# thodan/epos

Hardware: AMD Instinct MI355X
Metric: images/sec end-to-end (CNN+PnP-RANSAC), YCB-V 640x480 (higher is better)
Workload: dtype f32

## Files before the change

### epos_amd/_lib.py

```python
import ctypes
import os

from epos_amd import build as _build

c_f32p = ctypes.POINTER(ctypes.c_float)
c_f64p = ctypes.POINTER(ctypes.c_double)
c_i32p = ctypes.POINTER(ctypes.c_int32)
c_i64p = ctypes.POINTER(ctypes.c_int64)
c_u64p = ctypes.POINTER(ctypes.c_uint64)
vp = ctypes.c_void_p


class EposError(RuntimeError):
  pass


class PointwiseArgs(ctypes.Structure):
  _fields_ = [
      ('A', vp), ('lda', ctypes.c_int64),
      ('Wp', vp), ('bias', vp),
      ('R', vp), ('ldr', ctypes.c_int64),
      ('C', vp), ('ldc', ctypes.c_int64),
      ('M', ctypes.c_int32), ('N', ctypes.c_int32), ('K', ctypes.c_int32),
      ('relu', ctypes.c_int32), ('relu_in', ctypes.c_int32),
      ('sub', ctypes.c_int32),
      ('Ho', ctypes.c_int32), ('Wo', ctypes.c_int32),
      ('Hi', ctypes.c_int32), ('Wi', ctypes.c_int32),
      ('Ws', vp),
      ('Wh', vp), ('a_amax', vp), ('a_amax2', vp),
      ('a_gain', ctypes.c_float), ('a_bias', ctypes.c_float),
      ('a_presplit', ctypes.c_int32),
      ('c_amax', vp),
      ('col_sums', vp), ('col_ld', ctypes.c_int64),
      ('c_stream', ctypes.c_int32), ('reserved0', ctypes.c_int32),
  ]


class DepthwiseArgs(ctypes.Structure):
  _fields_ = [
      ('X', vp), ('ldx', ctypes.c_int64),
      ('w9c', vp), ('bias', vp),
      ('Y', vp), ('ldy', ctypes.c_int64),
      ('B', ctypes.c_int32), ('Hi', ctypes.c_int32), ('Wi', ctypes.c_int32),
      ('Ho', ctypes.c_int32), ('Wo', ctypes.c_int32), ('C', ctypes.c_int32),
      ('stride', ctypes.c_int32), ('rate', ctypes.c_int32),
      ('relu_in', ctypes.c_int32), ('relu_out', ctypes.c_int32),
      ('y_h2', ctypes.c_int32), ('x_amax', vp), ('x_amax2', vp),
      ('gain', ctypes.c_float), ('bias0', ctypes.c_float),
  ]


class SepConvArgs(ctypes.Structure):
  _fields_ = [('dw', DepthwiseArgs), ('pw', PointwiseArgs)]


class Conv3x3Args(ctypes.Structure):
  _fields_ = [
      ('X', vp), ('ldx', ctypes.c_int64),
      ('Wp', vp), ('bias', vp),
      ('Y', vp), ('ldy', ctypes.c_int64),
      ('B', ctypes.c_int32), ('H', ctypes.c_int32), ('W', ctypes.c_int32),
      ('Cin', ctypes.c_int32), ('Cout', ctypes.c_int32),
      ('stride', ctypes.c_int32), ('rate', ctypes.c_int32),
      ('relu', ctypes.c_int32),
      ('Ws', vp),
      ('Wh', vp), ('x_amax', vp), ('y_amax', vp),
  ]


class Im2colArgs(ctypes.Structure):
  _fields_ = [
      ('X', vp), ('ldx', ctypes.c_int64),
      ('col', vp), ('ldcol', ctypes.c_int64),
      ('B', ctypes.c_int32), ('Hi', ctypes.c_int32), ('Wi', ctypes.c_int32),
      ('Ho', ctypes.c_int32), ('Wo', ctypes.c_int32), ('C', ctypes.c_int32),
      ('stride', ctypes.c_int32), ('rate', ctypes.c_int32),
      ('pad', ctypes.c_int32), ('preprocess', ctypes.c_int32),
      ('amax_clear', vp), ('amax_words', ctypes.c_int64),
  ]


PREPROCESS_NONE, PREPROCESS_UNIT_RANGE, PREPROCESS_SUB_MEAN = 0, 1, 2


class Im2colKArgs(ctypes.Structure):
  _fields_ = [
      ('X', vp), ('ldx', ctypes.c_int64),
      ('col', vp), ('ldcol', ctypes.c_int64),
      ('B', ctypes.c_int32), ('Hi', ctypes.c_int32), ('Wi', ctypes.c_int32),
      ('Ho', ctypes.c_int32), ('Wo', ctypes.c_int32), ('C', ctypes.c_int32),
      ('k', ctypes.c_int32), ('stride', ctypes.c_int32), ('rate', ctypes.c_int32),
      ('pad', ctypes.c_int32), ('preprocess', ctypes.c_int32),
      ('mean_rgb', ctypes.c_float * 3),
      ('amax_clear', vp), ('amax_words', ctypes.c_int64),
  ]


class PointwiseBf16Args(ctypes.Structure):
  _fields_ = [
      ('A', vp), ('lda', ctypes.c_int64),
      ('Wp', vp), ('bias', vp),
      ('R', vp), ('ldr', ctypes.c_int64),
      ('C', vp), ('ldc', ctypes.c_int64),
      ('M', ctypes.c_int32), ('N', ctypes.c_int32), ('K', ctypes.c_int32),
      ('relu', ctypes.c_int32), ('sub', ctypes.c_int32),
      ('Ho', ctypes.c_int32), ('Wo', ctypes.c_int32),
      ('Hi', ctypes.c_int32), ('Wi', ctypes.c_int32),
      ('c_f32', ctypes.c_int32), ('c_stream', ctypes.c_int32),
  ]


class DepthwiseBf16Args(ctypes.Structure):
  _fields_ = [
      ('X', vp), ('ldx', ctypes.c_int64),
      ('w9c', vp), ('bias', vp),
      ('Y', vp), ('ldy', ctypes.c_int64),
      ('B', ctypes.c_int32), ('Hi', ctypes.c_int32), ('Wi', ctypes.c_int32),
      ('Ho', ctypes.c_int32), ('Wo', ctypes.c_int32), ('C', ctypes.c_int32),
      ('stride', ctypes.c_int32), ('rate', ctypes.c_int32),
      ('relu_in', ctypes.c_int32), ('relu_out', ctypes.c_int32),
  ]


class Im2colBf16Args(ctypes.Structure):
  _fields_ = [
      ('X', vp), ('ldx', ctypes.c_int64),
      ('x_bf16', ctypes.c_int32), ('reserved0', ctypes.c_int32),
      ('col', vp), ('ldcol', ctypes.c_int64),
      ('B', ctypes.c_int32), ('Hi', ctypes.c_int32), ('Wi', ctypes.c_int32),
      ('Ho', ctypes.c_int32), ('Wo', ctypes.c_int32), ('C', ctypes.c_int32),
      ('k', ctypes.c_int32), ('stride', ctypes.c_int32), ('rate', ctypes.c_int32),
      ('pad', ctypes.c_int32), ('preprocess', ctypes.c_int32),
# ... 59 lines not shown
              ('K', ctypes.c_int32), ('N', ctypes.c_int32)]


class PointwiseWgradArgs(ctypes.Structure):
  _fields_ = [('A', vp), ('lda', ctypes.c_int64), ('G', vp), ('ldg', ctypes.c_int64),
              ('M', ctypes.c_int64), ('K', ctypes.c_int32), ('N', ctypes.c_int32),
              ('a_presplit', ctypes.c_int32), ('reserved0', ctypes.c_int32),
              ('a_amax', vp), ('a_amax2', vp),
              ('a_gain', ctypes.c_float), ('a_bias', ctypes.c_float),
              ('S', vp), ('g', vp), ('workspace', vp)]


class PointwiseDgradArgs(ctypes.Structure):
  _fields_ = [('G', vp), ('ldg', ctypes.c_int64), ('W', vp), ('gamma', vp),
              ('moving_variance', vp), ('eps', ctypes.c_double),
              ('mask', vp), ('ldm', ctypes.c_int64),
              ('mask_h2', ctypes.c_int32), ('reserved0', ctypes.c_int32),
              ('M', ctypes.c_int64), ('K', ctypes.c_int32), ('N', ctypes.c_int32),
              ('D', vp), ('ldd', ctypes.c_int64), ('workspace', vp)]


class DepthwiseWgradArgs(ctypes.Structure):
  _fields_ = [('X', vp), ('ldx', ctypes.c_int64), ('D', vp), ('ldd', ctypes.c_int64),
              ('B', ctypes.c_int32), ('H', ctypes.c_int32), ('W', ctypes.c_int32),
              ('C', ctypes.c_int32), ('stride', ctypes.c_int32), ('rate', ctypes.c_int32),
              ('T', vp), ('t', vp), ('workspace', vp)]


class AsppJoinDw(ctypes.Structure):
  _fields_ = [('D', vp), ('ldd', ctypes.c_int64), ('w9c', vp), ('rate', ctypes.c_int32),
              ('reserved0', ctypes.c_int32)]


class AsppJoinPlain(ctypes.Structure):
  _fields_ = [('E', vp), ('lde', ctypes.c_int64)]


class AsppJoinArgs(ctypes.Structure):
  _fields_ = [('B', ctypes.c_int32), ('H', ctypes.c_int32), ('W', ctypes.c_int32),
              ('C', ctypes.c_int32), ('n_dw', ctypes.c_int32), ('n_plain', ctypes.c_int32),
              ('dw', AsppJoinDw * 4), ('plain', AsppJoinPlain * 2),
              ('Pool', vp), ('ldp', ctypes.c_int64), ('pool_div', ctypes.c_int64),
              ('Y', vp), ('ldy', ctypes.c_int64), ('dX', vp), ('ldx', ctypes.c_int64),
              ('partition', ctypes.c_int32), ('reserved0', ctypes.c_int32)]


ASPP_JOIN_PARTITIONS = {'shipped': 0, 'pixel': 1, 'slice32': 2, 'slice64': 3, 'slice32x2': 4,
                        'slice32x4': 5}


class FitParams(ctypes.Structure):
  _fields_ = [
      ('threshold', ctypes.c_double),
      ('neighborhood_ball_radius', ctypes.c_double),
      ('spatial_coherence_weight', ctypes.c_double),
      ('scaling_from_millimeters', ctypes.c_double),
      ('max_tanimoto_similarity', ctypes.c_double),
      ('conf', ctypes.c_double),
      ('proposal_engine_conf', ctypes.c_double),
      ('min_coverage', ctypes.c_double),
      ('min_triangle_area', ctypes.c_double),
      ('max_iters', ctypes.c_int32),
      ('min_point_number', ctypes.c_int32),
      ('max_model_number', ctypes.c_int32),
      ('max_model_number_for_optimization', ctypes.c_int32),
      ('use_prosac', ctypes.c_int32),
      ('lo_iters', ctypes.c_int32),
      ('gc_sweeps', ctypes.c_int32),
      ('pearl_iters', ctypes.c_int32),
  ]


class PnpRansacParams(ctypes.Structure):
  _fields_ = [
      ('iterations_count', ctypes.c_int32),
      ('min_point_number', ctypes.c_int32),
      ('reprojection_error', ctypes.c_double),
      ('confidence', ctypes.c_double),
  ]


SYMBOLS = {
    'epos_abi_version': (ctypes.c_int, []),
    'epos_last_error': (ctypes.c_char_p, []),
    'epos_device_count': (ctypes.c_int, []),
    'epos_clock_probe': (ctypes.c_int, [ctypes.c_void_p, ctypes.c_int, ctypes.c_void_p]),
    'epos_pack_pointwise_weights': (ctypes.c_int64,
                                    [vp, ctypes.c_int, ctypes.c_int, vp]),
    'epos_pack_pointwise_weights_split': (ctypes.c_int64,
                                          [vp, ctypes.c_int, ctypes.c_int, vp]),
    'epos_pack_pointwise_weights_h2': (ctypes.c_int64,
                                       [vp, ctypes.c_int, ctypes.c_int, vp]),
    'epos_absmax_f32': (ctypes.c_int, [vp, ctypes.c_int64, ctypes.c_int64,
                                       ctypes.c_int64, vp, vp]),
    'epos_amax_clear': (ctypes.c_int, [vp, ctypes.c_int64, vp]),
    'epos_pointwise_conv_f32': (ctypes.c_int,
                                [ctypes.POINTER(PointwiseArgs), vp]),
    'epos_pointwise_conv_grouped_f32': (ctypes.c_int, [
        ctypes.POINTER(PointwiseArgs), ctypes.c_int, vp]),
    'epos_heads_gemm_f32': (ctypes.c_int, [
        ctypes.POINTER(PointwiseArgs), ctypes.c_int, vp]),
    'epos_heads_gemm_plan': (ctypes.c_int, [
        ctypes.POINTER(PointwiseArgs), ctypes.c_int, ctypes.c_int, c_i32p]),
    'epos_conv3x3_f32': (ctypes.c_int, [ctypes.POINTER(Conv3x3Args), ctypes.c_void_p]),
    'epos_depthwise3x3_f32': (ctypes.c_int,
                              [ctypes.POINTER(DepthwiseArgs), vp]),
    'epos_separable_conv_f32': (ctypes.c_int, [ctypes.POINTER(SepConvArgs), vp]),
    'epos_set_h2_narrow_tile_limit': (ctypes.c_int, [ctypes.c_int]),
    'epos_im2col3x3_f32': (ctypes.c_int, [ctypes.POINTER(Im2colArgs), vp]),
    'epos_im2col_f32': (ctypes.c_int, [ctypes.POINTER(Im2colKArgs), vp]),
    'epos_global_avg_pool_partial_f32': (ctypes.c_int, [
        vp, ctypes.c_int64, vp, ctypes.c_int, ctypes.c_int, ctypes.c_int, ctypes.c_int, vp]),
    'epos_global_avg_pool_f32': (ctypes.c_int, [
        vp, ctypes.c_int64, vp, ctypes.c_int, ctypes.c_int, ctypes.c_int, vp]),
    'epos_resize_bilinear_f32': (ctypes.c_int, [
        vp, ctypes.c_int64, vp, ctypes.c_int64, ctypes.c_int, ctypes.c_int,
        ctypes.c_int, ctypes.c_int, ctypes.c_int, ctypes.c_int, vp]),
    'epos_maxpool3x3_s2_f32': (ctypes.c_int, [
        vp, ctypes.c_int64, vp, ctypes.c_int64, ctypes.c_int, ctypes.c_int,
        ctypes.c_int, ctypes.c_int, vp]),
    'epos_subsample_f32': (ctypes.c_int, [
        vp, ctypes.c_int64, vp, ctypes.c_int64, ctypes.c_int, ctypes.c_int,
        ctypes.c_int, ctypes.c_int, ctypes.c_int, vp]),
    'epos_add_relu_f32': (ctypes.c_int, [vp, vp, vp, ctypes.c_int64, vp]),
    'epos_softmax_groups_f32': (ctypes.c_int,
                                [vp, ctypes.c_int64, ctypes.c_int, vp]),
    'epos_u8_to_f32': (ctypes.c_int, [vp, vp, ctypes.c_int64, vp]),
    'epos_scatter_blocks_f32': (ctypes.c_int, [vp, vp, vp, ctypes.c_int64, ctypes.c_int, vp]),
    'epos_argmax_i64': (ctypes.c_int, [
        vp, ctypes.c_int64, vp, ctypes.c_int64, ctypes.c_int, vp]),
    'epos_softmax_slots_f32': (ctypes.c_int, [
        vp, vp, ctypes.c_int, ctypes.c_int, ctypes.c_int, ctypes.c_int, vp]),
    'epos_corr_count': (ctypes.c_int, [
        vp, vp, vp, ctypes.c_int, ctypes.c_int, ctypes.c_int, ctypes.c_int,
        ctypes.c_int, ctypes.c_float, ctypes.c_float, vp, vp, vp, vp, vp]),
    'epos_corr_fill': (ctypes.c_int, [
        vp, vp, vp, vp, vp, vp, ctypes.c_int, ctypes.c_int, ctypes.c_int,
        ctypes.c_int, ctypes.c_int, ctypes.c_int, ctypes.c_double, vp, vp, vp,
        vp, ctypes.c_int64, ctypes.POINTER(CorrOut), vp, vp]),
    'epos_corr_slot_bases': (ctypes.c_int, [vp, ctypes.c_int, vp, vp]),
    'epos_corr_order_tile_rows': (ctypes.c_int, []),
    'epos_corr_order_workspace_bytes': (ctypes.c_int64, [ctypes.c_int, ctypes.c_int64]),
    'epos_corr_order_by_conf': (ctypes.c_int, [
        vp, vp, vp, vp, vp, ctypes.c_int, ctypes.c_int64, ctypes.c_int, ctypes.c_int64,
        ctypes.c_int, vp, vp, vp, vp, vp, vp, vp, vp]),
    'epos_project_to_mesh_f64': (ctypes.c_int, [
        ctypes.c_void_p, ctypes.c_int64, ctypes.c_void_p, ctypes.c_int64,
        ctypes.c_void_p, ctypes.c_int64, ctypes.c_void_p, ctypes.c_void_p,
        ctypes.c_void_p]),
    'epos_project_rows_to_mesh_f64': (ctypes.c_int, [
        vp, vp, vp, ctypes.c_int, ctypes.c_int64, vp, ctypes.c_int, vp, vp, vp, vp, vp]),
    'epos_fragmentation_fps': (ctypes.c_int, [
        vp, ctypes.c_int64, ctypes.c_int, vp, vp, vp, vp, vp]),
    'epos_fit_params_default': (None, [ctypes.POINTER(FitParams)]),
    'epos_find6d_poses': (ctypes.c_int, [
        vp, vp, ctypes.c_int64, vp, ctypes.POINTER(FitParams), ctypes.c_uint64,
        vp, vp, vp, ctypes.c_int32]),
    'epos_fit_workspace_bytes': (ctypes.c_int64, [
        ctypes.c_int, ctypes.c_int64, ctypes.POINTER(FitParams),
        ctypes.c_int32]),
    'epos_find6d_poses_device': (ctypes.c_int, [
        vp, vp, vp, ctypes.c_int, ctypes.c_int64, vp, vp, vp,
        ctypes.POINTER(FitParams), ctypes.c_int32, vp, vp, vp, vp, vp, vp]),
    'epos_find6d_poses_device_ordered': (ctypes.c_int, [
        vp, vp, vp, ctypes.c_int, ctypes.c_int64, vp, vp, vp,
        ctypes.POINTER(FitParams), ctypes.c_int32, vp, vp, vp, vp, vp, vp, vp, vp]),
# ... 188 lines not shown
```

### epos_amd/csrc/common.h

```cpp
#pragma once
#include <hip/hip_runtime.h>
#include <stdint.h>
#include <stdio.h>

#include "../../include/epos_hip.h"

namespace epos {

void set_error(const char* fmt, ...);

inline int check_hip(hipError_t e, const char* what) {
  if (e == hipSuccess) return EPOS_OK;
  set_error("%s: %s", what, hipGetErrorString(e));
  return EPOS_E_HIP_BASE - static_cast<int>(e);
}

inline int launch_status(const char* kernel) {
  return check_hip(hipGetLastError(), kernel);
}

inline int64_t round_up(int64_t x, int64_t m) { return (x + m - 1) / m * m; }
inline int64_t ceil_div(int64_t x, int64_t m) { return (x + m - 1) / m; }
inline unsigned blocks_for(int64_t total, int threads) {
  return static_cast<unsigned>(ceil_div(total, threads));
}
inline bool al16(const void* p) { return (reinterpret_cast<uintptr_t>(p) & 15) == 0; }

__device__ __forceinline__ float4 relu4(float4 v) {
  return make_float4(fmaxf(v.x, 0.f), fmaxf(v.y, 0.f), fmaxf(v.z, 0.f),
                     fmaxf(v.w, 0.f));
}

constexpr int DW_PRIO = 3;
#define EPOS_SET_PRIO(p) do { if ((p) > 0) __builtin_amdgcn_s_setprio(p); } while (0)

#define EPOS_REQUIRE(cond, msg)                  \
  do {                                           \
    if (!(cond)) {                               \
      ::epos::set_error("%s: %s", __func__, msg); \
      return EPOS_E_INVALID;                     \
    }                                            \
  } while (0)

#define EPOS_REQUIRE_FN(fn, cond, msg)           \
  do {                                           \
    if (!(cond)) {                               \
      ::epos::set_error("%s: %s", fn, msg);      \
      return EPOS_E_INVALID;                     \
    }                                            \
  } while (0)

}
```

### epos_amd/csrc/glue.hip

```cpp
#include "nhwc.h"

namespace epos {
namespace {

template <class SP, class DP>
__global__ __launch_bounds__(256) void resize_bilinear_kernel(
    const typename SP::elem* X, int64_t ldx, typename DP::elem* Y, int64_t ldy, int Hi, int Wi,
    int Ho, int Wo, int cn, float sy, float sx, int64_t total) {
  static_assert(SP::n == DP::n, "one thread reads the channels it writes");
  const int64_t id = static_cast<int64_t>(blockIdx.x) * blockDim.x + threadIdx.x;
  if (id >= total) return;
  const Pixel p = decode_pixel<DP::n>(id, cn, Ho, Wo);
  const BilinearSrc<typename SP::elem> src = {X, ldx, Hi, Wi, sy, sx};
  float o[DP::n];
  bilinear_sample<SP>(src, p.b, p.yo, p.xo, p.c, o);
  DP::store(Y + pixel_offset(p, Ho, Wo, ldy), o);
}

template <class P>
__global__ __launch_bounds__(256) void maxpool3x3_s2_kernel(
    const typename P::elem* X, int64_t ldx, typename P::elem* Y, int64_t ldy, int Hi, int Wi,
    int Ho, int Wo, int cn, int pad_y, int pad_x, int64_t total) {
  const int64_t id = static_cast<int64_t>(blockIdx.x) * blockDim.x + threadIdx.x;
  if (id >= total) return;
  const Pixel p = decode_pixel<P::n>(id, cn, Ho, Wo);
  const typename P::elem* xb = X + static_cast<int64_t>(p.b) * Hi * Wi * ldx + p.c;
  float m[P::n];
#pragma unroll
  for (int e = 0; e < P::n; ++e) m[e] = -INFINITY;
#pragma unroll
  for (int ky = 0; ky < 3; ++ky) {
    const int yi = p.yo * 2 - pad_y + ky;
    if (yi < 0 || yi >= Hi) continue;
#pragma unroll
    for (int kx = 0; kx < 3; ++kx) {
      const int xi = p.xo * 2 - pad_x + kx;
      if (xi < 0 || xi >= Wi) continue;
      float v[P::n];
      P::load(xb + (static_cast<int64_t>(yi) * Wi + xi) * ldx, v);
#pragma unroll
      for (int e = 0; e < P::n; ++e) m[e] = fmaxf(m[e], v[e]);
    }
  }
  P::store(Y + pixel_offset(p, Ho, Wo, ldy), m);
}

template <class P>
__global__ __launch_bounds__(256) void subsample_kernel(
    const typename P::elem* X, int64_t ldx, typename P::elem* Y, int64_t ldy, int Hi, int Wi,
    int Ho, int Wo, int cn, int factor, int64_t total) {
  const int64_t id = static_cast<int64_t>(blockIdx.x) * blockDim.x + threadIdx.x;
  if (id >= total) return;
  const Pixel p = decode_pixel<P::n>(id, cn, Ho, Wo);
  using vec = typename P::vec;
  *reinterpret_cast<vec*>(Y + pixel_offset(p, Ho, Wo, ldy)) = *reinterpret_cast<const vec*>(
      X + ((static_cast<int64_t>(p.b) * Hi + p.yo * factor) * Wi + p.xo * factor) * ldx + p.c);
}

template <class P>
__global__ __launch_bounds__(256) void add_relu_kernel(const typename P::elem* A,
                                                       const typename P::elem* B,
                                                       typename P::elem* Y, int64_t packs) {
  const int64_t i = static_cast<int64_t>(blockIdx.x) * blockDim.x + threadIdx.x;
  if (i >= packs) return;
  float a[P::n], b[P::n];
  P::load(A + P::n * i, a);
  P::load(B + P::n * i, b);
#pragma unroll
  for (int e = 0; e < P::n; ++e) a[e] = fmaxf(a[e] + b[e], 0.f);
  P::store(Y + P::n * i, a);
}

int check_maps(const char* fn, const void* X, int64_t ldx, const void* Y, int64_t ldy, int B,
               int Hi, int Wi, int C, int N, const void* need_al0 = nullptr,
               const void* need_al1 = nullptr) {
  const char* msg = nullptr;
  if (!X || !Y) msg = "null pointer";
  else if (C % N || ldx % N || ldy % N) msg = "C, ldx, ldy must be multiples of 4 (bf16: 8)";
  else if (!al16(need_al0) || !al16(need_al1)) msg = "bf16 tensors must be 16-byte aligned";
  else if (B < 1 || Hi < 1 || Wi < 1 || C < 1) msg = "empty map";
  else if (ldx < C || ldy < C) msg = "ldx, ldy >= C";
  if (!msg) return EPOS_OK;
  set_error("%s: %s", fn, msg);
  return EPOS_E_INVALID;
}

struct Same { int out, pad; };
Same same_3x3_s2(int in) {
  const int out = (in + 1) / 2, t = (out - 1) * 2 + 3 - in;
  return {out, t > 0 ? t / 2 : 0};
}

template <class SP, class DP>
int resize(const typename SP::elem* X, int64_t ldx, typename DP::elem* Y, int64_t ldy, int B,
           int Hi, int Wi, int Ho, int Wo, int C, void* stream) {
  const int cn = C / DP::n;
  const int64_t total = static_cast<int64_t>(B) * Ho * Wo * cn;
  hipLaunchKernelGGL((resize_bilinear_kernel<SP, DP>), dim3(blocks_for(total, 256)), dim3(256),
                     0, static_cast<hipStream_t>(stream), X, ldx, Y, ldy, Hi, Wi, Ho, Wo, cn,
                     align_corners_scale(Hi, Ho), align_corners_scale(Wi, Wo), total);
  return launch_status("resize_bilinear_kernel");
}

template <class P>
int maxpool(const typename P::elem* X, int64_t ldx, typename P::elem* Y, int64_t ldy, int B,
            int Hi, int Wi, int C, void* stream) {
  const Same y = same_3x3_s2(Hi), x = same_3x3_s2(Wi);
  const int cn = C / P::n;
  const int64_t total = static_cast<int64_t>(B) * y.out * x.out * cn;
  hipLaunchKernelGGL(maxpool3x3_s2_kernel<P>, dim3(blocks_for(total, 256)), dim3(256), 0,
                     static_cast<hipStream_t>(stream), X, ldx, Y, ldy, Hi, Wi, y.out, x.out, cn,
                     y.pad, x.pad, total);
  return launch_status("maxpool3x3_s2_kernel");
}

template <class P>
int subsample(const typename P::elem* X, int64_t ldx, typename P::elem* Y, int64_t ldy, int B,
              int Hi, int Wi, int C, int factor, void* stream) {
  const int Ho = (Hi - 1) / factor + 1, Wo = (Wi - 1) / factor + 1;
  const int cn = C / P::n;
  const int64_t total = static_cast<int64_t>(B) * Ho * Wo * cn;
  hipLaunchKernelGGL(subsample_kernel<P>, dim3(blocks_for(total, 256)), dim3(256), 0,
                     static_cast<hipStream_t>(stream), X, ldx, Y, ldy, Hi, Wi, Ho, Wo, cn,
                     factor, total);
  return launch_status("subsample_kernel");
}

template <class P>
int add_relu(const char* fn, const typename P::elem* A, const typename P::elem* B,
             typename P::elem* Y, int64_t n, bool need_al, void* stream) {
  const char* msg = nullptr;
  if (!A || !B || !Y) msg = "null pointer";
  else if (n < 0 || n % P::n) msg = "n must be a multiple of 4 (bf16: 8)";
  else if (need_al && !(al16(A) && al16(B) && al16(Y))) msg = "16-byte aligned";
  if (msg) {
    set_error("%s: %s", fn, msg);
    return EPOS_E_INVALID;
  }
  if (n == 0) return EPOS_OK;
  hipLaunchKernelGGL(add_relu_kernel<P>, dim3(blocks_for(n / P::n, 256)), dim3(256), 0,
                     static_cast<hipStream_t>(stream), A, B, Y, n / P::n);
  return launch_status("add_relu_kernel");
}

using F32 = F32Pack<4>;

}
}

using namespace epos;

extern "C" int epos_resize_bilinear_f32(const float* X, int64_t ldx, float* Y, int64_t ldy, int B,
                                        int Hi, int Wi, int Ho, int Wo, int C, void* stream) {
  EPOS_REQUIRE(Ho >= 1 && Wo >= 1, "empty map");
  if (int rc = check_maps(__func__, X, ldx, Y, ldy, B, Hi, Wi, C, 4)) return rc;
  return resize<F32, F32>(X, ldx, Y, ldy, B, Hi, Wi, Ho, Wo, C, stream);
}

extern "C" int epos_resize_bilinear_bf16(const void* X, int64_t ldx, int x_f32, uint16_t* Y,
                                         int64_t ldy, int B, int Hi, int Wi, int Ho, int Wo,
                                         int C, void* stream) {
  EPOS_REQUIRE(Ho >= 1 && Wo >= 1, "empty map");
  if (int rc = check_maps(__func__, X, ldx, Y, ldy, B, Hi, Wi, C, 8, Y, x_f32 ? nullptr : X))
    return rc;
  if (x_f32)
    return resize<F32ScalarPack, Bf16Pack>(static_cast<const float*>(X), ldx, Y, ldy, B, Hi, Wi,
                                           Ho, Wo, C, stream);
  return resize<Bf16Pack, Bf16Pack>(static_cast<const uint16_t*>(X), ldx, Y, ldy, B, Hi, Wi, Ho,
                                    Wo, C, stream);
}

extern "C" int epos_maxpool3x3_s2_f32(const float* X, int64_t ldx, float* Y, int64_t ldy, int B,
                                      int Hi, int Wi, int C, void* stream) {
  if (int rc = check_maps(__func__, X, ldx, Y, ldy, B, Hi, Wi, C, 4)) return rc;
  return maxpool<F32>(X, ldx, Y, ldy, B, Hi, Wi, C, stream);
}

extern "C" int epos_maxpool3x3_s2_bf16(const uint16_t* X, int64_t ldx, uint16_t* Y,
                                       int64_t ldy, int B, int Hi, int Wi, int C, void* stream) {
  if (int rc = check_maps(__func__, X, ldx, Y, ldy, B, Hi, Wi, C, 8, X, Y)) return rc;
  return maxpool<Bf16Pack>(X, ldx, Y, ldy, B, Hi, Wi, C, stream);
}

extern "C" int epos_subsample_f32(const float* X, int64_t ldx, float* Y, int64_t ldy, int B,
                                  int Hi, int Wi, int C, int factor, void* stream) {
  EPOS_REQUIRE(factor >= 1, "factor >= 1");
  if (int rc = check_maps(__func__, X, ldx, Y, ldy, B, Hi, Wi, C, 4)) return rc;
  return subsample<F32>(X, ldx, Y, ldy, B, Hi, Wi, C, factor, stream);
}

extern "C" int epos_subsample_bf16(const uint16_t* X, int64_t ldx, uint16_t* Y, int64_t ldy,
                                   int B, int Hi, int Wi, int C, int factor, void* stream) {
  EPOS_REQUIRE(factor >= 1, "factor >= 1");
  if (int rc = check_maps(__func__, X, ldx, Y, ldy, B, Hi, Wi, C, 8, X, Y)) return rc;
  return subsample<Bf16Pack>(X, ldx, Y, ldy, B, Hi, Wi, C, factor, stream);
}

extern "C" int epos_add_relu_f32(const float* A, const float* B, float* Y, int64_t n,
                                 void* stream) {
  return add_relu<F32>(__func__, A, B, Y, n, false, stream);
}

extern "C" int epos_add_relu_bf16(const uint16_t* A, const uint16_t* B, uint16_t* Y, int64_t n,
                                  void* stream) {
  return add_relu<Bf16Pack>(__func__, A, B, Y, n, true, stream);
}
```

### epos_amd/csrc/heads_gemm_h2.hip

```cpp
#include "h2_scale.h"
#include "pointwise_gemm.h"

namespace epos {
namespace {

typedef _Float16 hd_f16x8 __attribute__((ext_vector_type(8)));
typedef unsigned hd_u32x4 __attribute__((ext_vector_type(4)));

constexpr int HD_BM = 128, HD_BN = 64, HD_BK = 16;
constexpr int HD_K = 256;
constexpr int HD_NKS = HD_K / HD_BK;
constexpr int HD_NS = 8;
constexpr int HD_LA = HD_NS - 1;
constexpr int HD_STAGE = 4 * 1024;
constexpr int HD_RING = HD_NS * HD_STAGE;
constexpr int HD_OPS = 2 * 4 * 1024;
constexpr int HD_EPR = HD_BN + 4;
constexpr int HD_EPI = 4 * 32 * HD_EPR * 4;
constexpr int HD_LDS = HD_RING + HD_OPS + HD_EPI;
constexpr int HD_S_MIN = 8;
constexpr unsigned HD_OOB = 0x80000000u;
static_assert(HD_NKS % HD_NS == 0, "stage of a K step = its index mod HD_NS");
static_assert(HD_LA - 2 + 2 + HD_S_MIN <= 63, "vmcnt is a 6-bit counter");

// ... 151 lines not shown
    const int par = (tt - t0) & 1;
    f32x16 acc[2], corr[2];
#pragma unroll
    for (int j = 0; j < 2; ++j)
#pragma unroll
      for (int r = 0; r < 16; ++r) { acc[j][r] = 0.f; corr[j][r] = 0.f; }

    auto step = [&](auto ks_tag) {
      constexpr int ks = decltype(ks_tag)::value;
      constexpr int younger = (HD_LA - 2) + (ks >= 10 ? 2 : 0);
      static_assert(HD_LA == 7, "the counts above are written for 7 steps ahead");
      if constexpr (ks <= 5) {
        if (first) hd_wait_vm_lgkm0<younger>();
        else hd_wait_vm_lgkm0<younger + HD_S_MIN>();
      } else {
        hd_wait_vm_lgkm0<younger>();
      }
      __builtin_amdgcn_s_barrier();
      constexpr int s1 = (ks + 1) % HD_NS;
      hd_u32x4 nb[2][2];
#pragma unroll
      for (int cb = 0; cb < 2; ++cb)
#pragma unroll
        for (int pc = 0; pc < 2; ++pc)
          nb[cb][pc] = *reinterpret_cast<const hd_u32x4*>(smem + s1 * (HD_STAGE / 4) + b_off +
                                                          (cb * 2 + pc) * 256);
      __builtin_amdgcn_sched_barrier(0);
      hd_mfma(ah[ks], bp[0][1], corr[0]);
      __builtin_amdgcn_sched_barrier(0);
      {
        constexpr int q = ks + HD_LA;
        constexpr int slot = q % HD_NS;
        if constexpr (q < HD_NKS) issue_w(cur, q, slot);
        else issue_w(nxt, q - HD_NKS, slot);
      }
      __builtin_amdgcn_sched_barrier(0);
      hd_mfma(ah[ks], bp[1][1], corr[1]);
      if constexpr (ks + HD_LA == HD_NKS) {
        __builtin_amdgcn_sched_barrier(0);
        issue_ops(nxt, par ^ 1);
        __builtin_amdgcn_sched_barrier(0);
      }
      hd_mfma(am[ks], bp[0][0], corr[0]);
      hd_mfma(am[ks], bp[1][0], corr[1]);
      hd_mfma(ah[ks], bp[0][0], acc[0]);
      hd_mfma(ah[ks], bp[1][0], acc[1]);
#pragma unroll
      for (int cb = 0; cb < 2; ++cb) { bp[cb][0] = nb[cb][0]; bp[cb][1] = nb[cb][1]; }
    };
    hd_static_for(std::make_integer_sequence<int, HD_NKS>{}, step);

#pragma unroll
    for (int j = 0; j < 2; ++j)
#pragma unroll
      for (int r = 0; r < 16; ++r)
        ws[((r & 3) + 8 * (r >> 2) + 4 * h) * HD_EPR + j * 32 + l31] =
            __builtin_fmaf(corr[j][r], 0x1p-11f, acc[j][r]);
    __builtin_amdgcn_fence(__ATOMIC_RELEASE, "wavefront");
    const float* ops = smem + (HD_RING + par * 4096) / 4 + wave * 256;
    const float4 cn4 = *reinterpret_cast<const float4*>(ops + c4 * 4);
    const float4 b4 = *reinterpret_cast<const float4*>(ops + 64 + c4 * 4);
    float4 v[8];
#pragma unroll
    for (int i = 0; i < 8; ++i) {
      v[i] = *reinterpret_cast<const float4*>(ws + (r0 + 4 * i) * HD_EPR + c4 * 4);
      v[i].x = v[i].x * cn4.x * inv_a + b4.x;
      v[i].y = v[i].y * cn4.y * inv_a + b4.y;
      v[i].z = v[i].z * cn4.z * inv_a + b4.z;
      v[i].w = v[i].w * cn4.w * inv_a + b4.w;
    }
    const EposPointwiseArgs& q = gp->p[cur.pi];
    const int rows = M - m0 < HD_BM ? M - m0 : HD_BM;
    const int64_t ldc = q.ldc;
    const __amdgpu_buffer_rsrc_t rsrc = __builtin_amdgcn_make_buffer_rsrc(
        q.C + static_cast<int64_t>(m0) * ldc, 0, static_cast<int>(rows * ldc * 4), 0x00020000);
    const int n = cur.n0 + c4 * 4;
    const unsigned row0 = static_cast<unsigned>(wave * 32 + r0);
    const bool vec = (ldc & 3) == 0 && (cur.N & 3) == 0 &&
                     (reinterpret_cast<uintptr_t>(q.C) & 15) == 0;
    auto opaque = [](unsigned x) { asm volatile("" : "+v"(x)); return x; };
    if (vec) {
      const unsigned oob = n < cur.N ? 0u : HD_OOB;
      const unsigned nb4 = static_cast<unsigned>(n) * 4u;
#pragma unroll
      for (int i = 0; i < 8; ++i) {
        const int off = static_cast<int>(
            opaque(((row0 + 4 * i) * static_cast<unsigned>(ldc) * 4u + nb4) | oob));
        if (q.c_stream)
          __builtin_amdgcn_raw_buffer_store_b128(__builtin_bit_cast(hd_u32x4, v[i]), rsrc, off, 0, 2);
        else
          __builtin_amdgcn_raw_buffer_store_b128(__builtin_bit_cast(hd_u32x4, v[i]), rsrc, off, 0, 0);
      }
    } else {
#pragma unroll
      for (int i = 0; i < 8; ++i) {
        const float e4[4] = {v[i].x, v[i].y, v[i].z, v[i].w};
#pragma unroll
        for (int e = 0; e < 4; ++e) {
          const unsigned oob = n + e < cur.N ? 0u : HD_OOB;
          const int off = static_cast<int>(opaque(
              (((row0 + 4 * i) * static_cast<unsigned>(ldc) + static_cast<unsigned>(n + e)) * 4u) |
              oob));
          __builtin_amdgcn_raw_buffer_store_b32(__float_as_uint(e4[e]), rsrc, off, 0, 0);
        }
      }
    }
    cur = nxt;
    nxt = hd_tile(gp, tt + 2 < t1 ? tt + 2 : t1 - 1);
  }
  asm volatile("s_waitcnt vmcnt(0)" ::: "memory");
}

int choose_range(int nt, int panels, int cus) {
  const int slots = cus > 8 ? cus * 2 / 8 : 1;
  const int pmax = (panels + 7) / 8;
  int best = nt < 4 ? nt : 4;
  int64_t best_cost = -1;
  for (int r = 4; r <= 32; ++r) {
    const int rr = r < nt ? r : nt;
    const int64_t nr = (nt + rr - 1) / rr;
    const int64_t rounds = (pmax * nr + slots - 1) / slots;
    const int64_t cost = rounds * (rr + 1);
    if (best_cost < 0 || cost < best_cost) { best_cost = cost; best = rr; }
    if (rr == nt) break;
  }
  return best;
}

int device_cus() {
  static int cus[16] = {};
  int dev = 0;
  if (hipGetDevice(&dev) != hipSuccess || dev < 0 || dev >= 16) return 256;
  int n = __atomic_load_n(&cus[dev], __ATOMIC_RELAXED);
  if (n > 0) return n;
  if (hipDeviceGetAttribute(&n, hipDeviceAttributeMultiprocessorCount, dev) != hipSuccess || n <= 0)
    n = 256;
  __atomic_store_n(&cus[dev], n, __ATOMIC_RELAXED);
  return n;
}

}

bool heads_eligible(const EposPointwiseArgs* args, int count) {
  if (count < 1 || count > MAX_GROUP) return false;
  const EposPointwiseArgs& a0 = args[0];
  if (!a0.a_amax) return false;
  for (int i = 0; i < count; ++i) {
    const EposPointwiseArgs& a = args[i];
    if (a.A != a0.A || a.lda != a0.lda || a.M != a0.M || a.K != HD_K || a.sub != 1 ||
        a.R || a.relu || a.relu_in || a.a_presplit || a.c_amax || a.col_sums || !a.Wh ||
        a.a_amax != a0.a_amax || a.a_amax2 != a0.a_amax2 || a.a_gain != a0.a_gain ||
        a.a_bias != a0.a_bias || a.N < 1 || a.M < 1 || a.ldc < a.N ||
        a.ldc > (1LL << 20) ||
        (reinterpret_cast<uintptr_t>(a.Wh) & 15) != 0 ||
        (reinterpret_cast<uintptr_t>(a.bias) & 3) != 0)
      return false;
  }
  return true;
}

namespace {

bool heads_fill(const EposPointwiseArgs* args, int count, int cus, HeadsArgs& g, int& blocks) {
  if (!h2_eligible(args, count) || !heads_eligible(args, count)) return false;
  g.count = count;
  int nt = 0;
  for (int i = 0; i < count; ++i) {
    g.p[i] = args[i];
    g.tile0[i] = nt;
    nt += static_cast<int>(ceil_div(args[i].N, HD_BN));
  }
  for (int i = count; i <= MAX_GROUP; ++i) g.tile0[i] = nt;
  g.nt = nt;
  g.panels = static_cast<int>(ceil_div(args[0].M, HD_BM));
// ... 47 lines not shown
```

### epos_amd/csrc/layers.hip

```cpp
#include <stdlib.h>

#include "h2_scale.h"
#include "nhwc.h"

namespace epos {
namespace {

typedef unsigned dw_u32x4 __attribute__((ext_vector_type(4)));
__device__ __forceinline__ void st4_h2(float* p, float4 v, float s) {
  dw_u32x4 o;
  unsigned h0, h1, m0, m1;
  h2_split_pair(v.x, v.y, s, h0, m0);
  h2_split_pair(v.z, v.w, s, h1, m1);
  o[0] = h0; o[1] = h1; o[2] = m0; o[3] = m1;
  *reinterpret_cast<dw_u32x4*>(p) = o;
}
__device__ __forceinline__ void st4_any(float* p, float4 v, bool h2, float s) {
  if (h2) st4_h2(p, v, s); else st4(p, v);
}
__device__ __forceinline__ float4 fma4(float4 a, float4 b, float4 c) {
  return make_float4(fmaf(a.x, b.x, c.x), fmaf(a.y, b.y, c.y),
                     fmaf(a.z, b.z, c.z), fmaf(a.w, b.w, c.w));
}

__global__ __launch_bounds__(256) void depthwise3x3_kernel(EposDepthwiseArgs p,
                                                           int c4n,
                                                           int64_t total) {
  EPOS_SET_PRIO(DW_PRIO);
  int64_t id = static_cast<int64_t>(blockIdx.x) * blockDim.x + threadIdx.x;
  const bool h2 = p.y_h2 != 0;
  float hs = 1.f;
  unsigned am_raw, am_raw2;
  {
    const unsigned* s1 = h2 ? p.x_amax : reinterpret_cast<const unsigned*>(p.bias);
    const unsigned* s2 = (h2 && p.x_amax2) ? p.x_amax2 : s1;
    const int li = h2 ? static_cast<int>(threadIdx.x & 63) : 0;
    am_raw = s1[li];
    am_raw2 = s2[li];
  }
  const bool live = id < total;
  if (__builtin_amdgcn_ballot_w64(live) == 0) return;
  id = live ? id : total - 1;
  const Pixel o = decode_pixel<4>(id, c4n, p.Ho, p.Wo);
  const int pad = p.rate;
  float4 acc = ld4(p.bias + o.c);
  const float* xb = p.X + static_cast<int64_t>(o.b) * p.Hi * p.Wi * p.ldx + o.c;
#pragma unroll
  for (int ky = 0; ky < 3; ++ky) {
    const int yi = o.yo * p.stride - pad + ky * p.rate;
    if (yi < 0 || yi >= p.Hi) continue;
#pragma unroll
    for (int kx = 0; kx < 3; ++kx) {
      const int xi = o.xo * p.stride - pad + kx * p.rate;
      if (xi < 0 || xi >= p.Wi) continue;
      float4 v = ld4(xb + (static_cast<int64_t>(yi) * p.Wi + xi) * p.ldx);
      if (p.relu_in) v = relu4(v);
      acc = fma4(v, ld4(p.w9c + (ky * 3 + kx) * p.C + o.c), acc);
    }
  }
  if (p.relu_out) acc = relu4(acc);
  if (h2) {
    float hinv;
    h2_scale_finish(am_raw, am_raw2, p.gain, p.bias0, hs, hinv);
  }
  if (live) st4_any(p.Y + pixel_offset(o, p.Ho, p.Wo, p.ldy), acc, h2, hs);
}

constexpr int DW_REP = 1;
constexpr int DW_MIN_BLOCKS = 4;
constexpr int DW_MIN_BLOCKS2 = 3;
struct FastDiv {
  unsigned mul, sh1, sh2, d;
};
struct DwPartition {
  int mode;
  int runs;
  int rows;
  int unit;
  int nu;
  FastDiv dwc[3];
  FastDiv dc4n, dchunk, dres, dho;
  FastDiv drate;
};
__device__ __forceinline__ unsigned fdiv(unsigned n, const FastDiv& f) {
  const unsigned t = __umulhi(f.mul, n);
  return (t + ((n - t) >> f.sh1)) >> f.sh2;
}
__device__ __forceinline__ float relu_1op(float x) {
  float r;
  asm("v_max_f32 %0, 0, %1" : "=v"(r) : "v"(x));
  return r;
}
__device__ __forceinline__ float4 relu4_1op(float4 v) {
  return make_float4(relu_1op(v.x), relu_1op(v.y), relu_1op(v.z), relu_1op(v.w));
}

template <int L, bool RELU_IN, bool RELU_OUT, int ROWS>
__global__ __launch_bounds__(256, (ROWS == 2 ? DW_MIN_BLOCKS2 : DW_MIN_BLOCKS)) void depthwise3x3_s1_kernel(
    EposDepthwiseArgs p, int c4n, int nres, int nchunk, int nrows, DwPartition part) {
  constexpr int NR = ROWS + 2;
  EPOS_SET_PRIO(DW_PRIO);
  {
    uint64_t a0 = reinterpret_cast<uint64_t>(p.X), a1 = reinterpret_cast<uint64_t>(p.w9c),
             a2 = reinterpret_cast<uint64_t>(p.bias), a3 = reinterpret_cast<uint64_t>(p.Y),
             a4 = reinterpret_cast<uint64_t>(p.x_amax), a5 = reinterpret_cast<uint64_t>(p.x_amax2),
             l0 = static_cast<uint64_t>(p.ldx), l1 = static_cast<uint64_t>(p.ldy);
    int i0 = p.B, i1 = p.Hi, i2 = p.Wi, i3 = p.Ho, i4 = p.Wo, i5 = p.C, i6 = p.rate, i7 = p.y_h2;
    float f0 = p.gain, f1 = p.bias0;
    const unsigned bd = blockDim.x;
    asm volatile("" : : "s"(bd));
    asm volatile("" : : "s"(a0), "s"(a1), "s"(a2), "s"(a3), "s"(a4), "s"(a5), "s"(l0), "s"(l1),
                 "s"(i0), "s"(i1), "s"(i2), "s"(i3), "s"(i4), "s"(i5), "s"(i6), "s"(i7), "s"(f0),
                 "s"(f1), "s"(c4n), "s"(nres), "s"(nchunk), "s"(nrows));
    asm volatile("" : : "s"(part.mode), "s"(part.runs), "s"(part.rows), "s"(part.dwc[0].mul),
                 "s"(part.dwc[0].sh1), "s"(part.dwc[0].sh2), "s"(part.dwc[0].d),
                 "s"(part.dwc[1].mul), "s"(part.dwc[1].sh1), "s"(part.dwc[1].sh2), "s"(part.dwc[1].d),
                 "s"(part.dwc[2].mul), "s"(part.dwc[2].sh1), "s"(part.dwc[2].sh2), "s"(part.unit), "s"(part.nu),
                 "s"(part.dc4n.mul), "s"(part.dc4n.sh1), "s"(part.dc4n.sh2), "s"(part.dchunk.mul),
                 "s"(part.dchunk.sh1), "s"(part.dchunk.sh2), "s"(part.dres.mul), "s"(part.dres.sh1),
                 "s"(part.dres.sh2), "s"(part.dho.mul), "s"(part.dho.sh1), "s"(part.dho.sh2),
                 "s"(part.drate.mul), "s"(part.drate.sh1), "s"(part.drate.sh2));
  }
  const bool h2 = p.y_h2 != 0;
  float hs = 1.f;
  unsigned am_raw, am_raw2;
  {
    const unsigned* s1 = h2 ? p.x_amax : reinterpret_cast<const unsigned*>(p.bias);
    const unsigned* s2 = (h2 && p.x_amax2) ? p.x_amax2 : s1;
    const int li = h2 ? static_cast<int>(threadIdx.x & 63) : 0;
    am_raw = s1[li];
    am_raw2 = s2[li];
  }
  static_assert(DW_REP == 1, "the scale reduction sits inside the (one) run of a thread");
  auto dw_scale_finish = [&] {
    if (h2) {
      float hinv;
      unsigned r1 = am_raw, r2 = am_raw2;
      asm volatile("" : "+v"(r1), "+v"(r2));
      h2_scale_finish(r1, r2, p.gain, p.bias0, hs, hinv);
    }
  };
  const int xcd = blockIdx.x & 7;
  const unsigned local = (blockIdx.x >> 3) * blockDim.x + threadIdx.x;
  int c, chunk, res, ys, b;
  bool live = true;
  if (part.mode == 0) {
    const int c_lo = (xcd * part.nu / 8) * part.unit;
    int c_hi = ((xcd + 1) * part.nu / 8) * part.unit;
    c_hi = c_hi < c4n ? c_hi : c4n;
    const int wc = c_hi - c_lo;
    live = wc > 0 && local < static_cast<unsigned>(part.runs) * wc;
    const FastDiv& dw = wc == static_cast<int>(part.dwc[0].d) ? part.dwc[0]
                      : wc == static_cast<int>(part.dwc[1].d) ? part.dwc[1] : part.dwc[2];
    unsigned rest = fdiv(local, dw);
    c = (c_lo + static_cast<int>(local - rest * wc)) * 4;
    unsigned q = fdiv(rest, part.dchunk);
    chunk = static_cast<int>(rest - q * nchunk); rest = q;
    q = fdiv(rest, part.dres);
    res = static_cast<int>(rest - q * nres); rest = q;
    q = fdiv(rest, part.dho);
    ys = static_cast<int>(rest - q * nrows);
    b = static_cast<int>(q);
  } else {
    const int r_lo = static_cast<int>(static_cast<int64_t>(xcd) * part.rows / 8);
    const int nrow = static_cast<int>(static_cast<int64_t>(xcd + 1) * part.rows / 8) - r_lo;
    live = local < static_cast<unsigned>(nrow) * nres * nchunk * c4n;
    unsigned rest = fdiv(local, part.dc4n);
    c = static_cast<int>(local - rest * c4n) * 4;
    unsigned q = fdiv(rest, part.dchunk);
    chunk = static_cast<int>(rest - q * nchunk); rest = q;
    q = fdiv(rest, part.dres);
    res = static_cast<int>(rest - q * nres); rest = q;
    const unsigned row = r_lo + rest;
    q = fdiv(row, part.dho);
    ys = static_cast<int>(row - q * nrows);
    b = static_cast<int>(q);
  }
  const int r = p.rate;
  int y = ys;
  if (ROWS == 2) {
    const unsigned g = fdiv(static_cast<unsigned>(ys), part.drate);
    y = static_cast<int>(2 * r * g + (ys - g * r));
  }
  live = live && res + chunk * (DW_REP * L) * r < p.Wo && y < p.Ho;
  if (__builtin_amdgcn_ballot_w64(live) == 0) return;
  if (!live) {
    c = part.mode == 0 ? (xcd * part.nu / 8) * part.unit * 4 : 0;
    chunk = 0; res = 0; y = 0; b = 0;
  }
  const bool row1 = ROWS == 2 && y + r < p.Ho;
  float4 w[9];
#pragma unroll
  for (int i = 0; i < 9; ++i) w[i] = ld4(p.w9c + i * p.C + c);
  const float4 bias = ld4(p.bias + c);
  const float* xb = p.X + static_cast<int64_t>(b) * p.Hi * p.Wi * p.ldx + c;
  float* yb = p.Y + ((static_cast<int64_t>(b) * p.Ho + y) * p.Wo) * p.ldy + c;
  const int ldx = static_cast<int>(p.ldx), ldy = static_cast<int>(p.ldy);
  const int rowpitch = p.Wi * ldx;
  const unsigned yrow1 = static_cast<unsigned>(r * p.Wo * ldy);
#pragma unroll 1
  for (int rep = 0; rep < DW_REP; ++rep) {
  const int x0 = res + (chunk * DW_REP + rep) * L * r;
  if (x0 >= p.Wo) break;
  const bool interior = y - r >= 0 && y + (ROWS == 2 ? 2 : 1) * r < p.Hi && x0 - r >= 0 &&
                        x0 + L * r < p.Wi && (ROWS == 1 || row1);
  float4 col[L + 2][NR];
  if (__builtin_amdgcn_ballot_w64(!interior) == 0) {
    const unsigned o00 = (y - r) * rowpitch + (x0 - r) * ldx;
    const unsigned rstep = r * rowpitch, cstep = r * ldx;
#pragma unroll
    for (int i = 0; i < L + 2; ++i)
#pragma unroll
      for (int ky = 0; ky < NR; ++ky) col[i][ky] = ld4(xb + (o00 + ky * rstep + i * cstep));
    __builtin_amdgcn_sched_barrier(0);
    dw_scale_finish();
    __builtin_amdgcn_sched_barrier(0);
    if (RELU_IN) {
#pragma unroll
      for (int i = 0; i < L + 2; ++i)
#pragma unroll
        for (int ky = 0; ky < NR; ++ky) col[i][ky] = relu4_1op(col[i][ky]);
    }
#pragma unroll
    for (int rr = 0; rr < ROWS; ++rr) {
#pragma unroll
      for (int j = 0; j < L; ++j) {
        float4 acc = bias;
#pragma unroll
        for (int ky = 0; ky < 3; ++ky) {
          acc = fma4(col[j][ky + rr], w[ky * 3 + 0], acc);
          acc = fma4(col[j + 1][ky + rr], w[ky * 3 + 1], acc);
          acc = fma4(col[j + 2][ky + rr], w[ky * 3 + 2], acc);
        }
        if (RELU_OUT) acc = relu4_1op(acc);
        st4_any(yb + (static_cast<unsigned>((x0 + j * r) * ldy) + (rr ? yrow1 : 0u)), acc, h2, hs);
      }
    }
    continue;
  }
  unsigned rowoff[NR];
  bool rowok[NR];
#pragma unroll
  for (int ky = 0; ky < NR; ++ky) {
    const int yi = y + (ky - 1) * r;
    rowok[ky] = yi >= 0 && yi < p.Hi;
    rowoff[ky] = (rowok[ky] ? yi : 0) * rowpitch;
  }
#pragma unroll
  for (int i = 0; i < L + 2; ++i) {
    const int xi = x0 + (i - 1) * r;
    const bool xok = xi >= 0 && xi < p.Wi;
    const unsigned off = (xok ? xi : 0) * ldx;
#pragma unroll
    for (int ky = 0; ky < NR; ++ky) col[i][ky] = ld4(xb + (rowoff[ky] + off));
  }
  __builtin_amdgcn_sched_barrier(0);
  dw_scale_finish();
  __builtin_amdgcn_sched_barrier(0);
#pragma unroll
  for (int i = 0; i < L + 2; ++i) {
    const int xi = x0 + (i - 1) * r;
    const bool xok = xi >= 0 && xi < p.Wi;
#pragma unroll
    for (int ky = 0; ky < NR; ++ky) {
      float4 v = col[i][ky];
      if (!(xok && rowok[ky])) v = make_float4(0.f, 0.f, 0.f, 0.f);
      col[i][ky] = RELU_IN ? relu4_1op(v) : v;
    }
  }
#pragma unroll
  for (int rr = 0; rr < ROWS; ++rr) {
    if (rr == 1 && !row1) break;
#pragma unroll
    for (int j = 0; j < L; ++j) {
      const int x = x0 + j * r;
      float4 acc = bias;
#pragma unroll
      for (int ky = 0; ky < 3; ++ky) {
        acc = fma4(col[j][ky + rr], w[ky * 3 + 0], acc);
        acc = fma4(col[j + 1][ky + rr], w[ky * 3 + 1], acc);
        acc = fma4(col[j + 2][ky + rr], w[ky * 3 + 2], acc);
      }
      if (RELU_OUT) acc = relu4_1op(acc);
      if (x < p.Wo && live) st4_any(yb + (static_cast<unsigned>(x * ldy) + (rr ? yrow1 : 0u)), acc, h2, hs);
    }
  }
  }
}

__global__ __launch_bounds__(256) void im2col3x3_kernel(EposIm2colArgs p,
                                                        int64_t total) {
  const int64_t id = static_cast<int64_t>(blockIdx.x) * blockDim.x + threadIdx.x;
  if (p.amax_clear && id < p.amax_words) p.amax_clear[id] = 0u;
  if (id >= total) return;
  const int col = static_cast<int>(id % p.ldcol);
  int64_t pix = id / p.ldcol;
  float v = 0.f;
  if (col < 9 * p.C) {
    const int tap = col / p.C, c = col - tap * p.C;
    const int ky = tap / 3, kx = tap - ky * 3;
    const int xo = static_cast<int>(pix % p.Wo);
    const int64_t t = pix / p.Wo;
    const int yo = static_cast<int>(t % p.Ho);
    const int b = static_cast<int>(t / p.Ho);
    const int yi = yo * p.stride - p.pad + ky * p.rate;
    const int xi = xo * p.stride - p.pad + kx * p.rate;
    if (yi >= 0 && yi < p.Hi && xi >= 0 && xi < p.Wi) {
      v = p.X[((static_cast<int64_t>(b) * p.Hi + yi) * p.Wi + xi) * p.ldx + c];
      if (p.preprocess) v = (2.0f / 255.0f) * v - 1.0f;
    }
  }
  p.col[pix * p.ldcol + col] = v;
}

__global__ __launch_bounds__(256) void im2col_k_kernel(EposIm2colKArgs p, int q) {
  const int r = blockIdx.x * blockDim.x + threadIdx.x;
  if (p.amax_clear) {
    const int64_t lin = (static_cast<int64_t>(blockIdx.y) * gridDim.x + blockIdx.x) *
                        blockDim.x + threadIdx.x;
    if (lin < p.amax_words) p.amax_clear[lin] = 0u;
  }
  if (r >= p.Wo * q) return;
  const int xo = r / q;
  const int col0 = (r - xo * q) * 4;
  const int kkc = p.k * p.k * p.C;
  const int tap0 = col0 / p.C;
  const int c0 = col0 - tap0 * p.C;
  const int ky0 = tap0 / p.k;
  const int kx0 = tap0 - ky0 * p.k;
  const int x0 = xo * p.stride - p.pad;
  const float m0 = p.mean_rgb[0], m1 = p.mean_rgb[1], m2 = p.mean_rgb[2];
  const int rows = p.B * p.Ho;
  for (int row = blockIdx.y; row < rows; row += gridDim.y) {
    const int b = row / p.Ho, yo = row - b * p.Ho;
    const int y0 = yo * p.stride - p.pad;
    const float* xb = p.X + static_cast<int64_t>(b) * p.Hi * p.Wi * p.ldx;
    int c = c0, ky = ky0, kx = kx0;
    float v[4];
#pragma unroll
    for (int j = 0; j < 4; ++j) {
      float e = 0.f;
      const int yi = y0 + ky * p.rate, xi = x0 + kx * p.rate;
      if (col0 + j < kkc && yi >= 0 && yi < p.Hi && xi >= 0 && xi < p.Wi) {
        e = xb[(static_cast<int64_t>(yi) * p.Wi + xi) * p.ldx + c];
        if (p.preprocess == EPOS_PREPROCESS_UNIT_RANGE) {
          e = (2.0f / 255.0f) * e - 1.0f;
        } else if (p.preprocess == EPOS_PREPROCESS_SUB_MEAN) {
          e = e - (c == 0 ? m0 : c == 1 ? m1 : c == 2 ? m2 : 0.f);
        }
      }
      v[j] = e;
      if (++c == p.C) {
        c = 0;
        if (++kx == p.k) { kx = 0; ++ky; }
      }
    }
    const int64_t m = static_cast<int64_t>(row) * p.Wo + xo;
    st4(p.col + m * p.ldcol + col0, make_float4(v[0], v[1], v[2], v[3]));
  }
}

__global__ __launch_bounds__(1024) void global_avg_pool_kernel(
    const float* X, int64_t ldx, float* Y, int HW, int C) {
  __shared__ float4 part[64][16];
  const int b = blockIdx.y;
  const int c = blockIdx.x * 64 + (threadIdx.x & 15) * 4;
  const int phase = threadIdx.x >> 4;
  float4 s = make_float4(0.f, 0.f, 0.f, 0.f);
  if (c < C) {
    const float* xb = X + static_cast<int64_t>(b) * HW * ldx + c;
    int r = phase;
    for (; r + 7 * 64 < HW; r += 8 * 64) {
      float4 v[8];
#pragma unroll
      for (int u = 0; u < 8; ++u) v[u] = ld4(xb + static_cast<int64_t>(r + u * 64) * ldx);
#pragma unroll
      for (int u = 0; u < 8; ++u) { s.x += v[u].x; s.y += v[u].y; s.z += v[u].z; s.w += v[u].w; }
    }
    for (; r < HW; r += 64) {
      const float4 v = ld4(xb + static_cast<int64_t>(r) * ldx);
      s.x += v.x; s.y += v.y; s.z += v.z; s.w += v.w;
    }
  }
  part[phase][threadIdx.x & 15] = s;
  __syncthreads();
  if (phase == 0 && c < C) {
    float4 t = part[0][threadIdx.x];
    for (int i = 1; i < 64; ++i) {
      const float4 v = part[i][threadIdx.x];
      t.x += v.x; t.y += v.y; t.z += v.z; t.w += v.w;
    }
    const float n = static_cast<float>(HW);
    st4(Y + static_cast<int64_t>(b) * C + c,
        make_float4(t.x / n, t.y / n, t.z / n, t.w / n));
  }
}

__global__ __launch_bounds__(256) void argmax_kernel(const float* X, int64_t ldx,
                                                     int64_t* labels, int64_t P,
                                                     int C) {
  const int64_t i = static_cast<int64_t>(blockIdx.x) * blockDim.x + threadIdx.x;
  if (i >= P) return;
  const float* x = X + i * ldx;
  float best = x[0];
  int arg = 0;
  for (int c = 1; c < C; ++c) {
    const float v = x[c];
    if (v > best) { best = v; arg = c; }
  }
  labels[i] = arg;
}

__global__ __launch_bounds__(256) void scatter_blocks_kernel(float* __restrict__ dst,
                                                             const int64_t* __restrict__ offsets,
                                                             const float* __restrict__ src,
                                                             int64_t total, int width) {
  const int64_t i = static_cast<int64_t>(blockIdx.x) * blockDim.x + threadIdx.x;
  if (i >= total) return;
  const int64_t b = i / width;
  dst[offsets[b] + (i - b * width)] = src[i];
}

__global__ __launch_bounds__(256) void u8_to_f32_kernel(const uint8_t* __restrict__ X,
                                                        float* __restrict__ Y, int64_t n) {
  const int64_t i = (static_cast<int64_t>(blockIdx.x) * blockDim.x + threadIdx.x) * 16;
  if (i >= n) return;
  if (i + 16 <= n) {
    const uint4 v = *reinterpret_cast<const uint4*>(X + i);
    const unsigned w[4] = {v.x, v.y, v.z, v.w};
#pragma unroll
    for (int q = 0; q < 4; ++q)
      reinterpret_cast<float4*>(Y + i)[q] = make_float4(
          static_cast<float>(w[q] & 0xffu), static_cast<float>((w[q] >> 8) & 0xffu),
          static_cast<float>((w[q] >> 16) & 0xffu), static_cast<float>(w[q] >> 24));
  } else {
    for (int64_t j = i; j < n; ++j) Y[j] = static_cast<float>(X[j]);
  }
}

}
}

using namespace epos;


extern "C" int epos_depthwise3x3_f32(const EposDepthwiseArgs* a, void* stream) {
  EPOS_REQUIRE(a && a->X && a->w9c && a->bias && a->Y, "null pointer");
  EPOS_REQUIRE(a->C % 4 == 0 && a->ldx % 4 == 0 && a->ldy % 4 == 0,
               "C, ldx, ldy must be multiples of 4");
  EPOS_REQUIRE(a->stride == 1 || (a->stride == 2 && a->rate == 1),
               "stride 2 requires rate 1");
  EPOS_REQUIRE(!a->y_h2 || a->x_amax, "y_h2 needs the absmax slot of X (x_amax)");
  const int c4n = a->C / 4;
  hipStream_t st = static_cast<hipStream_t>(stream);
  if (a->stride == 1 && a->Hi == a->Ho && a->Wi == a->Wo) {
    constexpr int L = 4;
    static const int threads = [] {
      const char* e = getenv("EPOS_DW_THREADS");
      return e ? atoi(e) : 256;
    }();
    const int nres = a->rate < a->Wo ? a->rate : a->Wo;
    const int per_res = static_cast<int>(ceil_div(a->Wo, a->rate));
    const int nchunk = static_cast<int>(ceil_div(per_res, L * DW_REP));
    static const int rows_env = [] {
      const char* e = getenv("EPOS_DW_ROWS");
      return e ? atoi(e) : 2;
    }();
    const int64_t threads2 = static_cast<int64_t>(a->B) * ceil_div(a->Ho, 2) *
                             ceil_div(a->Wo, L) * c4n;
    const int ROWS = (rows_env == 1 || (rows_env != 22 && threads2 < 256 * 256)) ? 1 : 2;
    const int nrows = ROWS == 2 ? static_cast<int>(ceil_div(a->Ho, 2 * a->rate)) * a->rate : a->Ho;
    const int64_t runs = static_cast<int64_t>(a->B) * nrows * nres * nchunk;
    if (runs == 0) return EPOS_OK;
    EPOS_REQUIRE(runs * c4n < (1LL << 31) &&
                 static_cast<int64_t>(a->Hi) * a->Wi * a->ldx < (1LL << 29) &&
                 static_cast<int64_t>(a->Ho) * a->Wo * a->ldy < (1LL << 29),
                 "tensor too large for 32-bit offsets within one image");
    static const int force_mode = [] {
      const char* e = getenv("EPOS_DW_MODE");
      return e ? atoi(e) : -1;
    }();
    auto fast_div = [](unsigned d) {
      FastDiv f; f.d = d;
      unsigned l = 0;
      while ((1ull << l) < d) ++l;
      f.mul = static_cast<unsigned>(((1ull << 32) * ((1ull << l) - d)) / d + 1);
      f.sh1 = l > 0 ? 1 : 0;
      f.sh2 = l > 0 ? l - 1 : 0;
      return f;
    };
    DwPartition part;
    part.mode = (c4n >= 128 || (c4n >= 64 && c4n % 8 == 0)) ? 0 : 1;
    if (force_mode >= 0) part.mode = force_mode;
    if (c4n < 8) part.mode = 1;
    part.runs = static_cast<int>(runs);
    part.rows = a->B * nrows;
    const bool lines = a->ldx % 32 == 0 && a->ldy % 32 == 0 &&
                       (reinterpret_cast<uintptr_t>(a->X) & 127) == 0 &&
                       (reinterpret_cast<uintptr_t>(a->Y) & 127) == 0 && c4n >= 64;
    part.unit = lines ? 8 : 1;
    part.nu = static_cast<int>(ceil_div(c4n, part.unit));
    int widths[3] = {0, 0, 0}, nwid = 0, wmax = 0;
    for (int x = 0; x < 8; ++x) {
      const int lo = (x * part.nu / 8) * part.unit;
      int hi = ((x + 1) * part.nu / 8) * part.unit;
      hi = hi < c4n ? hi : c4n;
      const int wdt = hi - lo;
      if (wdt <= 0) continue;
      wmax = wdt > wmax ? wdt : wmax;
      bool seen = false;
      for (int i = 0; i < nwid; ++i) seen = seen || widths[i] == wdt;
      if (!seen && nwid < 3) widths[nwid++] = wdt;
    }
    for (int i = 0; i < 3; ++i) part.dwc[i] = fast_div(widths[i] > 0 ? widths[i] : 1);
    part.dc4n = fast_div(c4n);
    part.dchunk = fast_div(nchunk);
    part.dres = fast_div(nres);
    part.dho = fast_div(nrows);
    part.drate = fast_div(a->rate);
    int64_t per_xcd;
    if (part.mode == 0) per_xcd = runs * (wmax > 0 ? wmax : 1);
    else per_xcd = ceil_div(part.rows, 8) * nres * nchunk * c4n;
    const unsigned grid = 8 * blocks_for(per_xcd, threads);
    const int v = (a->relu_in ? 2 : 0) | (a->relu_out ? 1 : 0);
    static const unsigned lds_pad = [] {
      const char* e = getenv("EPOS_DW_LDS_KB");
      return e ? static_cast<unsigned>(atoi(e)) * 1024u : 0u;
    }();
#define EPOS_DW_LAUNCH(RI, RO, RW)                                                          \
    hipLaunchKernelGGL((depthwise3x3_s1_kernel<L, RI, RO, RW>), dim3(grid), dim3(threads),   \
                       lds_pad, st, *a, c4n, nres, nchunk, nrows, part)
    if (ROWS == 2) {
      if (v == 0) EPOS_DW_LAUNCH(false, false, 2);
      else if (v == 1) EPOS_DW_LAUNCH(false, true, 2);
      else if (v == 2) EPOS_DW_LAUNCH(true, false, 2);
      else EPOS_DW_LAUNCH(true, true, 2);
    } else {
      if (v == 0) EPOS_DW_LAUNCH(false, false, 1);
      else if (v == 1) EPOS_DW_LAUNCH(false, true, 1);
      else if (v == 2) EPOS_DW_LAUNCH(true, false, 1);
      else EPOS_DW_LAUNCH(true, true, 1);
    }
#undef EPOS_DW_LAUNCH
    return launch_status("depthwise3x3_s1_kernel");
  }
  const int64_t total = static_cast<int64_t>(a->B) * a->Ho * a->Wo * c4n;
  if (total == 0) return EPOS_OK;
  hipLaunchKernelGGL(depthwise3x3_kernel, dim3(blocks_for(total, 256)), dim3(256),
                     0, st, *a, c4n, total);
  return launch_status("depthwise3x3_kernel");
}

extern "C" int epos_im2col3x3_f32(const EposIm2colArgs* a, void* stream) {
  EPOS_REQUIRE(a && a->X && a->col, "null pointer");
  EPOS_REQUIRE(a->ldcol >= 9 * a->C, "ldcol too small");
  const int64_t total = static_cast<int64_t>(a->B) * a->Ho * a->Wo * a->ldcol;
  EPOS_REQUIRE(!a->amax_clear || (a->amax_words >= 0 && a->amax_words <= total),
               "amax_words exceeds the launch's thread count");
  if (total == 0) return EPOS_OK;
  hipLaunchKernelGGL(im2col3x3_kernel, dim3(blocks_for(total, 256)), dim3(256), 0,
                     static_cast<hipStream_t>(stream), *a, total);
  return launch_status("im2col3x3_kernel");
}

extern "C" int epos_im2col_f32(const EposIm2colKArgs* a, void* stream) {
  EPOS_REQUIRE(a && a->X && a->col, "null pointer");
  EPOS_REQUIRE(a->k >= 1 && a->stride >= 1 && a->rate >= 1 && a->pad >= 0 && a->C >= 1,
               "bad k / stride / rate / pad / C");
  EPOS_REQUIRE(a->preprocess >= EPOS_PREPROCESS_NONE &&
               a->preprocess <= EPOS_PREPROCESS_SUB_MEAN, "bad preprocess mode");
  EPOS_REQUIRE(a->ldx >= a->C, "ldx < C");
  EPOS_REQUIRE(a->ldcol >= static_cast<int64_t>(a->k) * a->k * a->C, "ldcol too small");
  EPOS_REQUIRE(a->ldcol % 4 == 0 && reinterpret_cast<uintptr_t>(a->col) % 16 == 0,
               "col needs ldcol % 4 == 0 and 16-byte alignment");
  EPOS_REQUIRE(a->B >= 0 && a->Ho >= 0 && a->Wo >= 0 && a->Hi >= 1 && a->Wi >= 1,
               "bad shape");
  EPOS_REQUIRE(static_cast<int64_t>(a->Wo) * (a->ldcol / 4) < (1ll << 31) &&
               static_cast<int64_t>(a->B) * a->Ho < (1ll << 31), "shape too large");
  const int q = static_cast<int>(a->ldcol / 4);
  const int rows = a->B * a->Ho;
  const int64_t per_row = static_cast<int64_t>(a->Wo) * q;
  if (rows == 0 || per_row == 0) {
    EPOS_REQUIRE(!a->amax_clear || a->amax_words == 0,
                 "amax_words exceeds the launch's thread count");
    return EPOS_OK;
  }
  const dim3 grid(static_cast<unsigned>(blocks_for(per_row, 256)),
                  static_cast<unsigned>(rows < 65535 ? rows : 65535));
  EPOS_REQUIRE(!a->amax_clear || (a->amax_words >= 0 && a->amax_words <= per_row * grid.y),
               "amax_words exceeds the launch's thread count");
  hipLaunchKernelGGL(im2col_k_kernel, grid, dim3(256), 0, static_cast<hipStream_t>(stream), *a,
                     q);
  return launch_status("im2col_k_kernel");
}

extern "C" int epos_global_avg_pool_f32(const float* X, int64_t ldx, float* Y,
                                        int B, int HW, int C, void* stream) {
  EPOS_REQUIRE(X && Y, "null pointer");
  EPOS_REQUIRE(C % 4 == 0 && ldx % 4 == 0 && HW > 0, "C, ldx multiples of 4");
  EPOS_REQUIRE(B > 0 && C > 0 && ldx >= C, "B, C > 0; ldx >= C");
  hipLaunchKernelGGL(global_avg_pool_kernel,
                     dim3(static_cast<unsigned>(ceil_div(C, 64)), B), dim3(1024),
                     0, static_cast<hipStream_t>(stream), X, ldx, Y, HW, C);
  return launch_status("global_avg_pool_kernel");
}

namespace epos { namespace {
__global__ __launch_bounds__(256) void pool_partial_kernel(const float* P, int64_t ldp,
                                                           float* Y, int blocks, int C, int hw) {
  __shared__ float4 red[16][16];
  const int b = blockIdx.y;
  const int q = threadIdx.x & 15, r = threadIdx.x >> 4;
  const int c = (blockIdx.x * 16 + q) * 4;
  float4 t = make_float4(0.f, 0.f, 0.f, 0.f);
  if (c < C) {
    const float* pb = P + static_cast<int64_t>(b) * blocks * ldp + c;
#pragma unroll 4
    for (int i = r; i < blocks; i += 16) {
      const float4 v = ld4(pb + static_cast<int64_t>(i) * ldp);
      t.x += v.x; t.y += v.y; t.z += v.z; t.w += v.w;
    }
  }
  red[r][q] = t;
  __syncthreads();
  if (r != 0 || c >= C) return;
  for (int i = 1; i < 16; ++i) {
    const float4 v = red[i][q];
    t.x += v.x; t.y += v.y; t.z += v.z; t.w += v.w;
  }
  const float n = static_cast<float>(hw);
  st4(Y + static_cast<int64_t>(b) * C + c, make_float4(t.x / n, t.y / n, t.z / n, t.w / n));
}
} }

extern "C" int epos_global_avg_pool_partial_f32(const float* P, int64_t ldp, float* Y,
                                                int32_t B, int32_t blocks, int32_t C,
                                                int32_t hw, void* stream) {
  EPOS_REQUIRE(P && Y, "null pointer");
  EPOS_REQUIRE(C % 4 == 0 && ldp % 4 == 0 && ldp >= C && blocks > 0 && hw > 0 && B > 0,
               "C, ldp multiples of 4; blocks, hw, B > 0");
  hipLaunchKernelGGL(epos::pool_partial_kernel,
                     dim3(static_cast<unsigned>(epos::ceil_div(C, 64)), B), dim3(256), 0,
                     static_cast<hipStream_t>(stream), P, ldp, Y, blocks, C, hw);
  return epos::launch_status("pool_partial_kernel");
}

extern "C" int epos_argmax_i64(const float* X, int64_t ldx, int64_t* labels,
                               int64_t P, int C, void* stream) {
  EPOS_REQUIRE(X && labels, "null pointer");
  EPOS_REQUIRE(P >= 0 && C >= 1 && ldx >= C, "P >= 0; C >= 1; ldx >= C");
  if (P == 0) return EPOS_OK;
  hipLaunchKernelGGL(argmax_kernel, dim3(blocks_for(P, 256)), dim3(256), 0,
                     static_cast<hipStream_t>(stream), X, ldx, labels, P, C);
  return launch_status("argmax_kernel");
}

extern "C" int epos_scatter_blocks_f32(float* dst, const int64_t* offsets, const float* src,
                                       int64_t n_blocks, int width, void* stream) {
  EPOS_REQUIRE(n_blocks >= 0 && width > 0, "bad sizes");
  if (n_blocks == 0) return EPOS_OK;
  EPOS_REQUIRE(dst && offsets && src, "null pointer");
  const int64_t total = n_blocks * width;
  hipLaunchKernelGGL(scatter_blocks_kernel, dim3(blocks_for(total, 256)), dim3(256), 0,
                     static_cast<hipStream_t>(stream), dst, offsets, src, total, width);
  return launch_status("scatter_blocks_kernel");
}

extern "C" int epos_u8_to_f32(const uint8_t* X, float* Y, int64_t n, void* stream) {
  EPOS_REQUIRE(X && Y, "null pointer");
  EPOS_REQUIRE(reinterpret_cast<uintptr_t>(X) % 16 == 0 &&
               reinterpret_cast<uintptr_t>(Y) % 16 == 0, "16-byte aligned buffers");
  if (n == 0) return EPOS_OK;
  hipLaunchKernelGGL(u8_to_f32_kernel, dim3(blocks_for((n + 15) / 16, 256)), dim3(256), 0,
                     static_cast<hipStream_t>(stream), X, Y, n);
  return launch_status("u8_to_f32_kernel");
}
```

### epos_amd/csrc/pointwise_gemm.h

```cpp
#pragma once
#include <stdlib.h>

#include <mutex>
#include <type_traits>

#include "common.h"

namespace epos {

struct Fp32MfmaRef {
  int (*dma)(const EposPointwiseArgs* args, int count, hipStream_t s, const int* conv_cin,
             const int* conv_rate);
  int (*staged)(const EposPointwiseArgs* args, int count, hipStream_t s);
};
Fp32MfmaRef& fp32_mfma_ref();
int launch_grouped_split(const EposPointwiseArgs* args, int count, hipStream_t s,
                         const int* conv_cin = nullptr, const int* conv_rate = nullptr);
bool split_eligible(const EposPointwiseArgs* args, int count);
int launch_grouped_h2(const EposPointwiseArgs* args, int count, hipStream_t s,
                      const int* conv_cin = nullptr, const int* conv_rate = nullptr);
bool h2_eligible(const EposPointwiseArgs* args, int count);
bool heads_eligible(const EposPointwiseArgs* args, int count);
bool heads_takes(const EposPointwiseArgs* args, int count);
int heads_plan(const EposPointwiseArgs* args, int count, int cus, int32_t* plan);
// ... 55 lines not shown
  const uint32_t hi = __builtin_amdgcn_readfirstlane(static_cast<uint32_t>(b >> 32));
  return reinterpret_cast<const float*>((static_cast<uint64_t>(hi) << 32) | lo);
}
__device__ __forceinline__ void glds16_s(unsigned voff, const float* sbase,
                                         unsigned lds_dst) {
  unsigned keep;
  asm volatile(
      "s_mov_b32 %0, m0\n\ts_mov_b32 m0, %2\n\ts_nop 0\n\t"
      "global_load_lds_dwordx4 %1, %3\n\ts_mov_b32 m0, %0"
      : "=&s"(keep) : "v"(voff), "s"(lds_dst), "s"(sbase) : "memory");
}

__device__ __forceinline__ void glds16_v_m0(const float* gsrc, unsigned lds_dst) {
  asm volatile("s_mov_b32 m0, %1\n\ts_nop 0\n\tglobal_load_lds_dwordx4 %0, off"
               : : "v"(gsrc), "s"(lds_dst) : "memory", "m0");
}
__device__ __forceinline__ void glds16_s_m0(unsigned voff, const float* sbase,
                                            unsigned lds_dst) {
  asm volatile("s_mov_b32 m0, %1\n\ts_nop 0\n\tglobal_load_lds_dwordx4 %0, %2"
               : : "v"(voff), "s"(lds_dst), "s"(sbase) : "memory", "m0");
}
template <int OFF>
__device__ __forceinline__ void glds16_v_off(const float* gsrc) {
  asm volatile("global_load_lds_dwordx4 %0, off offset:%1" : : "v"(gsrc), "n"(OFF) : "memory");
}
template <int OFF>
__device__ __forceinline__ void glds16_s_off(unsigned voff, const float* sbase) {
  asm volatile("global_load_lds_dwordx4 %0, %1 offset:%2"
               : : "v"(voff), "s"(sbase), "n"(OFF) : "memory");
}
__device__ __forceinline__ void amax_publish(unsigned* slot, float m, int lane, int salt) {
#pragma unroll
  for (int o = 32; o > 0; o >>= 1) m = fmaxf(m, __shfl_xor(m, o, 64));
  if (lane == 0)
    __hip_atomic_fetch_max(slot + (salt & (EPOS_AMAX_WORDS - 1)), __float_as_uint(m),
                           __ATOMIC_RELAXED, __HIP_MEMORY_SCOPE_AGENT);
}

constexpr int EP_ROW = 68;

__device__ __forceinline__ bool vec_epilogue_ok(const EposPointwiseArgs& p, bool has_res) {
  bool ok = (p.ldc & 3) == 0 && (p.N & 3) == 0 &&
            (reinterpret_cast<uintptr_t>(p.C) & 15) == 0;
  if (has_res)
    ok = ok && (p.ldr & 3) == 0 && (reinterpret_cast<uintptr_t>(p.R) & 15) == 0;
  return ok;
}

template <int TM, int TN, bool HAS_RES, int EPR = EP_ROW>
__device__ __forceinline__ void vec_epilogue(float* ws, const f32x16* acc,
                                             const EposPointwiseArgs& p, int m0w,
                                             int n0w, int lane) {
  const int l31 = lane & 31, h = lane >> 5;
  const int M = p.M, N = p.N;
  constexpr int C4 = TN * 8;
  constexpr int RPI = 64 / C4;
  constexpr int NI = TM * 32 / RPI;
  const int c4 = lane % C4, r0 = lane / C4;
  const int n = n0w + c4 * 4;
  float4 rv[HAS_RES ? NI : 1];
  if (HAS_RES) {
    const int ncl = n < N ? n : 0;
#pragma unroll
    for (int i = 0; i < NI; ++i) {
      int m = m0w + r0 + i * RPI;
      m = m < M ? m : M - 1;
      rv[i] = *reinterpret_cast<const float4*>(p.R + static_cast<int64_t>(m) * p.ldr + ncl);
    }
  }
#pragma unroll
  for (int j = 0; j < TN; ++j) {
    const int nb = n0w + j * 32 + l31;
    const float bias = p.bias ? p.bias[nb < N ? nb : N - 1] : 0.f;
#pragma unroll
    for (int i = 0; i < TM; ++i)
#pragma unroll
      for (int r = 0; r < 16; ++r)
        ws[(i * 32 + (r & 3) + 8 * (r >> 2) + 4 * h) * EPR + j * 32 + l31] =
            acc[i * TN + j][r] + bias;
  }
  __builtin_amdgcn_fence(__ATOMIC_RELEASE, "wavefront");
  const bool relu = p.relu != 0;
  float amax = 0.f;
#pragma unroll
  for (int i = 0; i < NI; ++i) {
    const int row = r0 + i * RPI;
    const int m = m0w + row;
    float4 v = *reinterpret_cast<const float4*>(ws + row * EPR + c4 * 4);
    if (HAS_RES) {
      v.x += rv[i].x; v.y += rv[i].y; v.z += rv[i].z; v.w += rv[i].w;
    }
    if (relu) v = relu4(v);
    if (m < M && n < N) {
      *reinterpret_cast<float4*>(p.C + static_cast<int64_t>(m) * p.ldc + n) = v;
      amax = fmaxf(fmaxf(amax, fmaxf(fabsf(v.x), fabsf(v.y))), fmaxf(fabsf(v.z), fabsf(v.w)));
    }
  }
  if (p.c_amax) amax_publish(p.c_amax, amax, lane, static_cast<int>(blockIdx.x) * 4 + (m0w >> 5));
}

}
}
```

### epos_amd/csrc/pointwise_gemm.hip

```cpp
#include "pointwise_gemm.h"

namespace epos {

Fp32MfmaRef& fp32_mfma_ref() {
  static Fp32MfmaRef hooks = {nullptr, nullptr};
  return hooks;
}

namespace {

int no_fp32_mfma(const char* what) {
  set_error("%s: this problem brings neither fp16-pair (Wh + a bound for A) nor bf16 x 6 (Ws) "
            "weights, and this build of libepos_hip.so carries no fp32-MFMA kernel (they are "
            "test-only since round 6: libepos_hip_ref.so, `python -m epos_amd.build --ref`, "
            "EPOS_HIP_LIB=<that file>)", what);
  return EPOS_E_INVALID;
}

constexpr int GEMV_SLICES = 16;

__global__ __launch_bounds__(64 * GEMV_SLICES) void pointwise_gemv_f32(EposPointwiseArgs p,
                                                                       int npad) {
  __shared__ float part[GEMV_SLICES][64];
  const int t = threadIdx.x;
// ... 12 lines not shown
      wv[u] = *reinterpret_cast<const float4*>(
          p.Wp + (static_cast<int64_t>(q + u * GEMV_SLICES) * npad + n) * 4);
    }
#pragma unroll
    for (int u = 0; u < 8; ++u) {
      if (p.relu_in) av[u] = relu4(av[u]);
      acc = fmaf(av[u].x, wv[u].x, acc);
      acc = fmaf(av[u].y, wv[u].y, acc);
      acc = fmaf(av[u].z, wv[u].z, acc);
      acc = fmaf(av[u].w, wv[u].w, acc);
    }
  }
  for (; q < kq; q += GEMV_SLICES) {
    float4 av = *reinterpret_cast<const float4*>(a + q * 4);
    if (p.relu_in) av = relu4(av);
    const float4 wv = *reinterpret_cast<const float4*>(
        p.Wp + (static_cast<int64_t>(q) * npad + n) * 4);
    acc = fmaf(av.x, wv.x, acc);
    acc = fmaf(av.y, wv.y, acc);
    acc = fmaf(av.z, wv.z, acc);
    acc = fmaf(av.w, wv.w, acc);
  }
  part[ks][t & 63] = acc;
  __syncthreads();
  if (ks == 0 && n < p.N) {
    float v = part[0][t];
#pragma unroll
    for (int i = 1; i < GEMV_SLICES; ++i) v += part[i][t];
    if (p.bias) v += p.bias[n];
    if (p.R) v += p.R[static_cast<int64_t>(m) * p.ldr + n];
    if (p.relu) v = fmaxf(v, 0.f);
    p.C[static_cast<int64_t>(m) * p.ldc + n] = v;
  }
}

int validate(const EposPointwiseArgs* a) {
  EPOS_REQUIRE(a->A && a->Wp && a->C, "null pointer");
  EPOS_REQUIRE(a->M > 0 && a->N > 0 && a->K > 0, "empty problem");
  EPOS_REQUIRE(a->K % 4 == 0 && a->lda % 4 == 0, "K and lda must be multiples of 4");
  EPOS_REQUIRE((reinterpret_cast<uintptr_t>(a->A) & 15) == 0, "A must be 16-byte aligned");
  EPOS_REQUIRE(a->sub >= 1, "sub must be >= 1");
  EPOS_REQUIRE(!a->a_presplit || (a->Wh && a->a_amax && a->relu_in == 0 && a->M > 8 &&
                                  a->sub == 1),
               "a_presplit needs Wh, a_amax, relu_in == 0, sub == 1 and M > 8");
  if (a->c_amax) {
    bool ok = a->relu_in == 0 && a->M > 8 && (a->N & 3) == 0 && (a->ldc & 3) == 0 &&
              (reinterpret_cast<uintptr_t>(a->C) & 15) == 0;
    if (a->R) ok = ok && (a->ldr & 3) == 0 && (reinterpret_cast<uintptr_t>(a->R) & 15) == 0;
    EPOS_REQUIRE(ok, "c_amax needs N, ldc (ldr) multiples of 4, 16-byte aligned C (R), "
                     "relu_in == 0 and M > 8");
  }
  return EPOS_OK;
}

}
}

extern "C" int64_t epos_pack_pointwise_weights(const float* w_kn, int K, int N,
                                               float* dst) {
  using namespace epos;
  const int64_t kg = ceil_div(K, BK) * (BK / 4);
  const int64_t npad = round_up(N, BN);
  const int64_t total = kg * npad * 4;
  if (!dst) return total;
  for (int64_t q = 0; q < kg; ++q)
    for (int64_t n = 0; n < npad; ++n)
      for (int e = 0; e < 4; ++e) {
        const int64_t k = q * 4 + e;
        dst[(q * npad + n) * 4 + e] =
            (k < K && n < N) ? w_kn[k * static_cast<int64_t>(N) + n] : 0.f;
      }
  return total;
}

static int grouped_impl(const EposPointwiseArgs* args, int count, void* stream);

extern "C" int epos_pointwise_conv_grouped_f32(const EposPointwiseArgs* args,
                                               int count, void* stream) {
  using namespace epos;
  EPOS_REQUIRE(args && count >= 1 && count <= MAX_GROUP, "1..8 problems per group");
  for (int i = 0; i < count; ++i) {
    const EposPointwiseArgs& a = args[i];
    EPOS_REQUIRE(a.reserved0 == 0, "EposPointwiseArgs.reserved0 must be 0 (ABI 7)");
    if (a.col_sums)
      EPOS_REQUIRE(!a.R && a.N % 4 == 0 && a.col_ld % 4 == 0 && a.col_ld >= a.N &&
                       (reinterpret_cast<uintptr_t>(a.col_sums) & 15) == 0 &&
                       (a.ldc & 3) == 0 && (reinterpret_cast<uintptr_t>(a.C) & 15) == 0 &&
                       h2_eligible(args, count),
                   "col_sums needs the fp16-pair kernel (Wh, a bound for A), no residual, "
                   "N, ldc, col_ld multiples of 4 and 16-byte aligned C / col_sums");
  }
  return grouped_impl(args, count, stream);
}

extern "C" int epos_heads_gemm_f32(const EposPointwiseArgs* args, int count, void* stream) {
  using namespace epos;
  EPOS_REQUIRE(args && count >= 1 && count <= MAX_GROUP, "1..8 problems per group");
  if (!heads_takes(args, count))
    return epos_pointwise_conv_grouped_f32(args, count, stream);
  for (int i = 0; i < count; ++i) {
    EPOS_REQUIRE(args[i].reserved0 == 0, "EposPointwiseArgs.reserved0 must be 0 (ABI 7)");
    const int rc = validate(&args[i]);
    if (rc) return rc;
  }
  hipStream_t s = static_cast<hipStream_t>(stream);
  const float* z = h2_zero_chunk(s);
  EPOS_REQUIRE(z, "cannot allocate the zero chunk (first fp16-pair launch on this device "
                  "during a stream capture? launch once before capturing)");
  return launch_heads_h2(args, count, z, s);
}

extern "C" int epos_heads_gemm_plan(const EposPointwiseArgs* args, int count, int cus,
                                    int32_t* plan) {
  using namespace epos;
  EPOS_REQUIRE(args && count >= 1 && count <= MAX_GROUP, "1..8 problems per group");
  EPOS_REQUIRE(cus >= 0, "cus: 0 (the current device) or a positive count");
  return heads_plan(args, count, cus, plan);
}

static int grouped_impl(const EposPointwiseArgs* args, int count, void* stream) {
  using namespace epos;
  hipStream_t s = static_cast<hipStream_t>(stream);
  for (int i = 0; i < count; ++i) {
    const int rc = validate(&args[i]);
    if (rc) return rc;
    EPOS_REQUIRE((args[i].relu_in != 0) == (args[0].relu_in != 0) &&
                 (args[i].R != nullptr) == (args[0].R != nullptr),
                 "problems of one group must agree on relu_in / residual");
  }
  if (count == 1 && args[0].M <= 8 && args[0].sub == 1) {
    const int npad = static_cast<int>(round_up(args[0].N, BN));
    hipLaunchKernelGGL(pointwise_gemv_f32, dim3(npad / 64, args[0].M),
                       dim3(64 * GEMV_SLICES), 0, s, args[0], npad);
    return launch_status("pointwise_gemv_f32");
  }
  if (h2_eligible(args, count)) return launch_grouped_h2(args, count, s);
  for (int i = 0; i < count; ++i)
    EPOS_REQUIRE(!args[i].a_presplit,
                 "a pre-split A operand needs the fp16-pair kernel (every problem of the "
                 "group with Wh; EPOS_GEMM_H2 / EPOS_GEMM_SPLIT not 0)");
  if (split_eligible(args, count)) return launch_grouped_split(args, count, s);
  const Fp32MfmaRef& ref = fp32_mfma_ref();
  static const int use_dma = [] {
    const char* e = getenv("EPOS_GEMM_DMA");
    return e ? atoi(e) : -1;
  }();
  if (args[0].relu_in == 0 && use_dma != 0 && ref.dma)
    return ref.dma(args, count, s, nullptr, nullptr);
  if (ref.staged) return ref.staged(args, count, s);
  for (int i = 0; i < count; ++i)
    if (args[i].M <= 8) {
      set_error("epos_pointwise_conv_grouped_f32: problem %d of %d has M <= 8 rows (M = %d, "
                "sub = %d): such a problem is served by the GEMV only, as a single problem "
                "with sub == 1 -- not inside a group and not with a stride-2 gather, whatever "
                "weights it brings", i, count, args[i].M, args[i].sub);
      return EPOS_E_INVALID;
    }
  if (args[0].relu_in != 0) {
    set_error("epos_pointwise_conv_grouped_f32: relu_in != 0 with M > 8 (M = %d): the "
              "pre-activation ReLU is served by the GEMV only (one problem, M <= 8, sub == 1), "
              "whatever weights the problem brings", args[0].M);
    return EPOS_E_INVALID;
  }
  return no_fp32_mfma("epos_pointwise_conv_grouped_f32");
}

extern "C" int epos_conv3x3_f32(const EposConv3x3Args* a, void* stream) {
  using namespace epos;
  EPOS_REQUIRE(a && a->X && a->Wp && a->Y, "null pointer");
  EPOS_REQUIRE(a->Cin > 0 && a->Cin % BK == 0, "Cin must be a multiple of 32");
  EPOS_REQUIRE(a->ldx % 4 == 0 && a->ldx >= a->Cin, "ldx: multiple of 4, >= Cin");
  EPOS_REQUIRE((reinterpret_cast<uintptr_t>(a->X) & 15) == 0, "X must be 16-byte aligned");
  EPOS_REQUIRE(a->B > 0 && a->H > 0 && a->W > 0 && a->Cout > 0, "empty problem");
  EPOS_REQUIRE((a->stride == 1 || a->stride == 2) && a->rate >= 1, "stride 1|2, rate >= 1");
  const int ho = (a->H - 1) / a->stride + 1, wo = (a->W - 1) / a->stride + 1;
  EPOS_REQUIRE(static_cast<int64_t>(a->B) * a->H * a->W < (1LL << 31), "too many pixels");
  EposPointwiseArgs p = {};
  p.A = a->X; p.lda = a->ldx;
  p.Wp = a->Wp; p.bias = a->bias;
  p.R = nullptr; p.ldr = 0;
  p.C = a->Y; p.ldc = a->ldy;
  p.M = a->B * ho * wo; p.N = a->Cout; p.K = 9 * a->Cin;
  p.relu = a->relu; p.relu_in = 0; p.sub = a->stride;
  p.Ho = ho; p.Wo = wo; p.Hi = a->H; p.Wi = a->W;
  p.Ws = a->Ws;
  p.Wh = a->Wh; p.a_amax = a->x_amax; p.c_amax = a->y_amax;
  {
    const int rc = validate(&p);
    if (rc) return rc;
  }
  const int cin = a->Cin, rate = a->rate;
  if (a->Wh && h2_eligible(&p, 1))
    return launch_grouped_h2(&p, 1, static_cast<hipStream_t>(stream), &cin, &rate);
  if (a->Ws && split_eligible(&p, 1))
    return launch_grouped_split(&p, 1, static_cast<hipStream_t>(stream), &cin, &rate);
  if (fp32_mfma_ref().dma)
    return fp32_mfma_ref().dma(&p, 1, static_cast<hipStream_t>(stream), &cin, &rate);
  return no_fp32_mfma("epos_conv3x3_f32");
}

extern "C" int epos_separable_conv_f32(const EposSepConvArgs* a, void* stream) {
  using namespace epos;
  EPOS_REQUIRE(a && a->dw.X && a->dw.w9c && a->dw.bias && a->dw.Y, "null pointer");
  const EposDepthwiseArgs& d = a->dw;
  const EposPointwiseArgs& p = a->pw;
  EPOS_REQUIRE(p.A == d.Y && p.lda == d.ldy && p.K == d.C,
               "the pointwise conv must read the depthwise output");
  EPOS_REQUIRE(static_cast<int64_t>(p.M) == static_cast<int64_t>(d.B) * d.Ho * d.Wo,
               "pw.M must be the number of depthwise output pixels");
  EPOS_REQUIRE((d.y_h2 != 0) == (p.a_presplit != 0),
               "dw.y_h2 and pw.a_presplit describe the same intermediate");
  const int rc = validate(&p);
  if (rc) return rc;
  const int rd = epos_depthwise3x3_f32(&d, stream);
  if (rd) return rd;
  return epos_pointwise_conv_f32(&p, stream);
}

extern "C" int epos_pointwise_conv_f32(const EposPointwiseArgs* a, void* stream) {
  return epos_pointwise_conv_grouped_f32(a, 1, stream);
}
```

### epos_amd/csrc/pointwise_gemm_h2.hip

```cpp
#include <string.h>

#include <mutex>
#include <utility>

#include "h2_scale.h"
#include "pointwise_gemm.h"

namespace epos {
namespace {

typedef _Float16 f16x8 __attribute__((ext_vector_type(8)));
typedef unsigned u32x4 __attribute__((ext_vector_type(4)));
typedef float h2_f32x4 __attribute__((ext_vector_type(4)));

#ifdef EPOS_GEMM_TRACE
__device__ uint64_t* g_h2_trace = nullptr;
#define H2_STAMP(i) do { if (g_h2_trace && t == 0) g_h2_trace[8 * static_cast<uint64_t>(blockIdx.x) + (i)] = wall_clock64(); } while (0)
#else
#define H2_STAMP(i) do { } while (0)
#endif
constexpr int RING_DEVICES = 16;
constexpr int H2_BM = 128, H2_BN = 128, H2_BK = 16;
constexpr int H2_W_BYTES = H2_BK * H2_BN * 4;
constexpr int H2_A_BYTES = H2_BM * H2_BK * 4;
// ... 51 lines not shown
                                                 const EposPointwiseArgs& p, int m0w, int n0w,
                                                 int lane) {
  const int l31 = lane & 31, h = lane >> 5;
  const int M = p.M, N = p.N;
  constexpr int EPR = H2Geo<NB>::EP_ROW;
  constexpr int C4 = NB * 8;
  constexpr int RPI = 64 / C4;
  constexpr int NI = 32 / RPI;
  const int c4 = lane & (C4 - 1);
  int r0 = lane / C4;
  asm volatile("" : "+v"(r0));
  const int n = n0w + c4 * 4;
  float4 rv[HAS_RES ? NI : 1];
  const int ncl = n < N ? n : 0;
  auto request_res = [&](int i_lo, int i_hi) {
#pragma unroll
    for (int i = i_lo; i < i_hi; ++i) {
      int m = m0w + r0 + i * RPI;
      m = m < M ? m : M - 1;
      rv[i] = *reinterpret_cast<const float4*>(p.R + static_cast<int64_t>(m) * p.ldr + ncl);
    }
  };
  if (HAS_RES) request_res(0, NI / 2);
#pragma unroll
  for (int j = 0; j < NB; ++j) {
    if (HAS_RES && j == NB / 2) request_res(NI / 2, NI);
    const float bias = bias4 ? bias4[j] : 0.f;
    const float c = cn[j];
#pragma unroll
    for (int r = 0; r < 16; r += 2) {
      const h2_f32x2 a2 = {acc[j][r], acc[j][r + 1]}, c2 = {corr[j][r], corr[j][r + 1]};
      const h2_f32x2 k2 = {0x1p-11f, 0x1p-11f}, cc = {c, c}, ia = {inv_a, inv_a}, b2 = {bias, bias};
      const h2_f32x2 sum = __builtin_elementwise_fma(c2, k2, a2);
      h2_f32x2 sv = (sum * cc) * ia;
      if (bias4) sv = sv + b2;
      ws[((r & 3) + 8 * (r >> 2) + 4 * h) * EPR + j * 32 + l31] = sv[0];
      ws[(((r + 1) & 3) + 8 * ((r + 1) >> 2) + 4 * h) * EPR + j * 32 + l31] = sv[1];
    }
  }
  __builtin_amdgcn_fence(__ATOMIC_RELEASE, "wavefront");
#ifdef EPOS_GEMM_TRACE
  if (g_h2_trace && threadIdx.x == 0) g_h2_trace[8 * static_cast<uint64_t>(blockIdx.x) + 6] = wall_clock64();
#endif
  const bool relu = p.relu != 0;
  float amax = 0.f;
  float4 bv = make_float4(0.f, 0.f, 0.f, 0.f);
  if (!bias4 && p.bias) {
    const float* bsrc = p.bias + (n < N ? n : 0);
    bv = *reinterpret_cast<const float4*>(bsrc);
  }
  float4 v[NI];
#pragma unroll
  for (int i = 0; i < NI; ++i)
    v[i] = *reinterpret_cast<const float4*>(ws + (r0 + i * RPI) * EPR + c4 * 4);
#pragma unroll
  for (int i = 0; i < NI; ++i) {
    if (!bias4) { v[i].x += bv.x; v[i].y += bv.y; v[i].z += bv.z; v[i].w += bv.w; }
    if (HAS_RES) {
      v[i].x += rv[i].x; v[i].y += rv[i].y; v[i].z += rv[i].z; v[i].w += rv[i].w;
    }
  }
  if (relu) {
#pragma unroll
    for (int i = 0; i < NI; ++i) v[i] = relu4(v[i]);
  }
  if (!HAS_RES && p.col_sums) {
    float4 cs = make_float4(0.f, 0.f, 0.f, 0.f);
#pragma unroll
    for (int i = 0; i < NI; ++i) {
      if (m0w + r0 + i * RPI < M) { cs.x += v[i].x; cs.y += v[i].y; cs.z += v[i].z; cs.w += v[i].w; }
    }
    if constexpr (NB == 2) {
      cs.x += __shfl_xor(cs.x, 16, 64); cs.y += __shfl_xor(cs.y, 16, 64);
      cs.z += __shfl_xor(cs.z, 16, 64); cs.w += __shfl_xor(cs.w, 16, 64);
    }
    cs.x += __shfl_xor(cs.x, 32, 64); cs.y += __shfl_xor(cs.y, 32, 64);
    cs.z += __shfl_xor(cs.z, 32, 64); cs.w += __shfl_xor(cs.w, 32, 64);
    if (lane < C4 && n < N && m0w < M)
      *reinterpret_cast<float4*>(p.col_sums + static_cast<int64_t>(m0w >> 5) * p.col_ld + n) = cs;
  }
  float* crow = p.C + (static_cast<int64_t>(m0w + r0) * p.ldc + n);
  const int64_t cstep = static_cast<int64_t>(RPI) * p.ldc;
  const bool nok = n < N;
  const bool nt = p.c_stream != 0;
#pragma unroll
  for (int i = 0; i < NI; ++i) {
    const int m = m0w + r0 + i * RPI;
    if (m < M && nok) {
      if (nt) {
        const h2_f32x4 nv = {v[i].x, v[i].y, v[i].z, v[i].w};
        __builtin_nontemporal_store(nv, reinterpret_cast<h2_f32x4*>(crow));
      }
      else *reinterpret_cast<float4*>(crow) = v[i];
      amax = fmaxf(fmaxf(amax, fmaxf(fabsf(v[i].x), fabsf(v[i].y))),
                   fmaxf(fabsf(v[i].z), fabsf(v[i].w)));
    }
    crow += cstep;
  }
#ifdef EPOS_GEMM_TRACE
  if (g_h2_trace && threadIdx.x == 0) g_h2_trace[8 * static_cast<uint64_t>(blockIdx.x) + 7] = wall_clock64();
#endif
  return amax;
}

template <bool HAS_RES, bool SINGLE, bool CONV, bool PRESPLIT, int NB = 4>
__global__ __launch_bounds__(256, 2)
void pointwise_gemm_h2_f32(GroupedArgs ga_) {
  static_assert(NB == 4 || NB == 2, "tile = 128 x 128 or 128 x 64");
  using Geo = H2Geo<NB>;
  constexpr int NW = 4;
  constexpr int NST = H2_NST;
  constexpr int BM = H2_BM;
  constexpr int NP = Geo::NP;
  constexpr int NA = Geo::NA;
  constexpr int LA = NST - 1;
  static_assert((LA - 1) * NP <= 63, "vmcnt is a 6-bit counter");
  extern __shared__ __attribute__((aligned(16))) float smem[];
  const int t = threadIdx.x;
  const int lane = t & 63;
  const int wave = t >> 6;
  const int wave_u = __builtin_amdgcn_readfirstlane(wave);
  const int wrow = wave;
  const int l31 = lane & 31, h = lane >> 5;

  (void)ga_;
  H2_STAMP(0);
  const GroupedArgs* __restrict__ gp =
      (const GroupedArgs*)__builtin_amdgcn_kernarg_segment_ptr();
  if constexpr (SINGLE) {
    const EposPointwiseArgs& q = gp->p[0];
    uint64_t a0 = reinterpret_cast<uint64_t>(q.A), a1 = reinterpret_cast<uint64_t>(q.Wh),
             a2 = reinterpret_cast<uint64_t>(q.C), a3 = reinterpret_cast<uint64_t>(q.R),
             a4 = reinterpret_cast<uint64_t>(q.bias), a5 = reinterpret_cast<uint64_t>(q.a_amax),
             a6 = reinterpret_cast<uint64_t>(q.a_amax2), a7 = reinterpret_cast<uint64_t>(q.c_amax),
             a8 = reinterpret_cast<uint64_t>(gp->zero_chunk), l0 = static_cast<uint64_t>(q.lda),
             l1 = static_cast<uint64_t>(q.ldc), l2 = static_cast<uint64_t>(q.ldr);
    int i0 = q.M, i1 = q.N, i2 = q.K, i3 = q.relu, i4 = q.sub, i5 = gp->tiles_n[0],
        i6 = gp->tile_start[MAX_GROUP], i7 = q.Ho, i8 = q.Wo, i9 = q.Hi, i10 = q.Wi,
        i11 = q.c_stream;
    uint64_t a9 = reinterpret_cast<uint64_t>(q.col_sums), l3 = static_cast<uint64_t>(q.col_ld);
    unsigned u0 = gp->tn_mul[0], u1 = gp->tn_sh1[0], u2 = gp->tn_sh2[0];
    float f0 = q.a_gain, f1 = q.a_bias;
    asm volatile("" : : "s"(a0), "s"(a1), "s"(a2), "s"(a3), "s"(a4), "s"(a5), "s"(a6), "s"(a7),
                 "s"(a8), "s"(l0), "s"(l1), "s"(l2));
    asm volatile("" : : "s"(i0), "s"(i1), "s"(i2), "s"(i3), "s"(i4), "s"(i5), "s"(i6), "s"(u0),
                 "s"(u1), "s"(u2), "s"(f0), "s"(f1));
    asm volatile("" : : "s"(i7), "s"(i8), "s"(i9), "s"(i10), "s"(i11), "s"(a9), "s"(l3));
  }
  int bid;
  {
    const int total = gp->tile_start[MAX_GROUP];
    const int raw = blockIdx.x, x = raw & 7, idx = raw >> 3;
    const int q = total >> 3, r = total & 7;
    bid = (x < r ? x * (q + 1) : r * (q + 1) + (x - r) * q) + idx;
  }
  int pi = 0;
  if (!SINGLE) {
#pragma unroll
    for (int i = 1; i < MAX_GROUP; ++i)
      if (i < gp->count && bid >= gp->tile_start[i]) pi = i;
    bid -= gp->tile_start[pi];
  }
  const EposPointwiseArgs p = gp->p[pi];
  const int tiles_n = gp->tiles_n[pi];
  const float* zero_chunk = uniform_ptr(gp->zero_chunk);
  const int M = p.M, N = p.N, K = p.K;
  int tile_m, tile_n;
  if (tiles_n <= 8) {
    const H2Div dv = {gp->tn_mul[pi], gp->tn_sh1[pi], gp->tn_sh2[pi]};
    tile_m = static_cast<int>(h2_div(static_cast<unsigned>(bid), dv));
    tile_n = bid - tile_m * tiles_n;
  } else {
    const int tiles_m = (M + BM - 1) / BM;
    const int per_band = tiles_m * 8;
    const int band = bid / per_band;
    const int rem = bid - band * per_band;
    const int left = tiles_n - band * 8;
    const int bw = left < 8 ? left : 8;
    tile_m = rem / bw;
    tile_n = band * 8 + (rem - tile_m * bw);
  }
// ... 819 lines not shown
```

### epos_amd/csrc/runtime.hip

```cpp
#include <stdarg.h>
#include <string.h>

#include "common.h"

namespace epos {
namespace {
thread_local char g_error[512] = "";
}

void set_error(const char* fmt, ...) {
  va_list ap;
  va_start(ap, fmt);
  vsnprintf(g_error, sizeof(g_error), fmt, ap);
  va_end(ap);
}

namespace {
__global__ void clock_probe_kernel(int64_t* out, int ticks) {
  const unsigned long long w0 = wall_clock64(), c0 = clock64();
  unsigned long long w = w0;
  while (w - w0 < static_cast<unsigned long long>(ticks)) {
    __builtin_amdgcn_s_sleep(8);
    w = wall_clock64();
  }
  const unsigned long long c1 = clock64();
  out[0] = static_cast<int64_t>(c1 - c0);
  out[1] = static_cast<int64_t>(w - w0);
}
}
}

extern "C" int epos_clock_probe(int64_t* out2, int microseconds, void* stream) {
  EPOS_REQUIRE(out2 && microseconds > 0 && microseconds <= 100000, "bad arguments");
  hipLaunchKernelGGL(epos::clock_probe_kernel, dim3(1), dim3(64), 0,
                     static_cast<hipStream_t>(stream), out2, microseconds * 100);
  return epos::launch_status("clock_probe_kernel");
}

extern "C" int epos_abi_version(void) { return EPOS_ABI_VERSION; }

extern "C" const char* epos_last_error(void) { return epos::g_error; }

extern "C" int epos_device_count(void) {
  int n = 0;
  hipError_t e = hipGetDeviceCount(&n);
  if (e != hipSuccess) {
    epos::set_error("hipGetDeviceCount: %s", hipGetErrorString(e));
    (void)hipGetLastError();
    return 0;
  }
  return n;
}
```

### epos_amd/csrc/softmax.hip

```cpp
#include "common.h"
#include "wave.h"

namespace epos {
namespace {

typedef float sm_f32x4 __attribute__((ext_vector_type(4)));
template <bool STREAM>
__device__ __forceinline__ float4 ld4(const float* p) {
  const sm_f32x4* q = reinterpret_cast<const sm_f32x4*>(p);
  const sm_f32x4 v = STREAM ? __builtin_nontemporal_load(q) : *q;
  return make_float4(v[0], v[1], v[2], v[3]);
}
template <bool STREAM>
__device__ __forceinline__ void st4(float* p, float4 v) {
  const sm_f32x4 o = {v.x, v.y, v.z, v.w};
  if (STREAM) __builtin_nontemporal_store(o, reinterpret_cast<sm_f32x4*>(p));
  else *reinterpret_cast<sm_f32x4*>(p) = o;
}

template <int LANES>
__device__ __forceinline__ float4 softmax_vec4(float4 v) {
  const float m = wave_max<LANES>(fmaxf(fmaxf(v.x, v.y), fmaxf(v.z, v.w)));
  v.x = expf(v.x - m); v.y = expf(v.y - m); v.z = expf(v.z - m); v.w = expf(v.w - m);
  const float s = wave_sum<LANES>((v.x + v.y) + (v.z + v.w));
  return make_float4(v.x / s, v.y / s, v.z / s, v.w / s);
}

template <int N, typename Op>
__device__ __forceinline__ float in_lane(const float* v, Op op) {
  if constexpr (N == 1) return v[0];
  else return op(in_lane<N / 2>(v, op), in_lane<N / 2>(v + N / 2, op));
}

template <int NV>
__device__ __forceinline__ void softmax_strided(float* x, int G, int lane) {
  float v[NV];
#pragma unroll
  for (int k = 0; k < NV; ++k) v[k] = lane + 64 * k < G ? x[lane + 64 * k] : -INFINITY;
  const float m = wave_max(in_lane<NV>(v, [](float a, float b) { return fmaxf(a, b); }));
#pragma unroll
  for (int k = 0; k < NV; ++k) v[k] = lane + 64 * k < G ? expf(v[k] - m) : 0.f;
  const float s = wave_sum(in_lane<NV>(v, [](float a, float b) { return a + b; }));
#pragma unroll
  for (int k = 0; k < NV; ++k)
    if (lane + 64 * k < G) x[lane + 64 * k] = v[k] / s;
}

struct DenseRows {
  static constexpr bool STREAM = true;
  typedef int64_t Index;
  Index n;
  __device__ __forceinline__ float* at(float* X, int64_t r, int G) const { return X + r * G; }
};
struct SlotRows {
  static constexpr bool STREAM = false;
  typedef int Index;
  Index n;
  const EposCorrSlot* __restrict__ slots;
  int O;
  __device__ __forceinline__ float* at(float* X, int p, int F) const {
    const int img = slots[blockIdx.y].image, obj = slots[blockIdx.y].obj_id;
    return X + ((static_cast<int64_t>(img) * n + p) * O + (obj - 1)) * F;
  }
};

template <int VEC, int NV, typename Rows>
__global__ __launch_bounds__(256) void softmax_kernel(float* X, Rows rows, int G) {
  constexpr int ROWS_PER_WAVE = VEC ? 64 / VEC : 1;
  const int lane = threadIdx.x & 63;
  typedef typename Rows::Index Index;
  const Index r = (static_cast<Index>(blockIdx.x) * 4 + (threadIdx.x >> 6)) * ROWS_PER_WAVE +
                  (VEC ? lane / VEC : 0);
  const bool on = r < rows.n;
  if (ROWS_PER_WAVE == 1 && !on) return;
  if constexpr (VEC != 0) {
    float* x = rows.at(X, on ? r : 0, 4 * VEC) + (lane & (VEC - 1)) * 4;
    const float4 y = softmax_vec4<VEC>(ld4<Rows::STREAM>(x));
    if (on) st4<Rows::STREAM>(x, y);
  } else {
    softmax_strided<NV>(rows.at(X, r, G), G, lane);
  }
}

template <int VEC, int NV, typename Rows>
int launch_form(float* X, const Rows& rows, unsigned grid_y, int G, void* stream,
                const char* name) {
  const unsigned grid_x = static_cast<unsigned>(ceil_div(rows.n, VEC == 16 ? 16 : 4));
  hipLaunchKernelGGL((softmax_kernel<VEC, NV, Rows>), dim3(grid_x, grid_y), dim3(256), 0,
                     static_cast<hipStream_t>(stream), X, rows, G);
  return launch_status(name);
}

template <typename Rows>
int softmax_launch(float* X, const Rows& rows, unsigned grid_y, int G, void* stream) {
#define EPOS_SM_LAUNCH(VEC, NV)                                                          \
  launch_form<VEC, NV>(X, rows, grid_y, G, stream,                                       \
                       std::is_same<Rows, DenseRows>::value                              \
                           ? "softmax_kernel<" #VEC ", " #NV ", DenseRows>"              \
                           : "softmax_kernel<" #VEC ", " #NV ", SlotRows>")
  const bool aligned = (reinterpret_cast<uintptr_t>(X) & 15) == 0;
  if (G > 64) return G == 256 && aligned ? EPOS_SM_LAUNCH(64, 0) : EPOS_SM_LAUNCH(0, 4);
  return G == 64 && aligned ? EPOS_SM_LAUNCH(16, 0) : EPOS_SM_LAUNCH(0, 1);
#undef EPOS_SM_LAUNCH
}

}
}

using namespace epos;

extern "C" int epos_softmax_groups_f32(float* X, int64_t n_groups, int G,
                                       void* stream) {
  EPOS_REQUIRE(X, "null pointer");
  EPOS_REQUIRE(G >= 1 && G <= 256, "G must be in [1, 256]");
  if (n_groups == 0) return EPOS_OK;
  return softmax_launch(X, DenseRows{n_groups}, 1, G, stream);
}

extern "C" int epos_softmax_slots_f32(float* X, const EposCorrSlot* slots, int S,
                                      int P, int O, int F, void* stream) {
  EPOS_REQUIRE(X && slots, "null pointer");
  EPOS_REQUIRE(F >= 1 && F <= 256, "F must be in [1, 256]");
  if (S == 0 || P == 0) return EPOS_OK;
  return softmax_launch(X, SlotRows{P, slots, O}, S, F, stream);
}
```

### epos_amd/net.py

```python
import ctypes
import os

import numpy as np
import torch

from epos_amd import _call as C
from epos_amd import _lib
from epos_amd import weights as W
from epos_amd._call import ptr as _ptr
from epos_amd.net_modes import Bf16Mode, Fp32Mode

XCEPTION_BN_EPS = 1e-3
HEAD_BN_EPS = 1e-5
RESNET_BN_EPS = 1e-5
MODES = {'fp32': Fp32Mode, 'bf16': Bf16Mode}
PRECISIONS = tuple(MODES)
PREPROCESS = {None: _lib.PREPROCESS_NONE, 'unit_range': _lib.PREPROCESS_UNIT_RANGE,
              'sub_mean': _lib.PREPROCESS_SUB_MEAN}
PREPROCESS_EXPR = {'unit_range': 'preprocess(input)', 'sub_mean': 'submean(input)'}


def scale_dimension(dim, scale):
  return int((float(dim) - 1.0) * scale + 1.0)


_CAPTURE_STREAMS = {}


def _capture_stream(dev):
  side = torch.cuda.current_stream(dev)
  if side != torch.cuda.default_stream(dev):
    return side
  key = str(dev)
  if key not in _CAPTURE_STREAMS:
    _CAPTURE_STREAMS[key] = torch.cuda.Stream(dev)
  return _CAPTURE_STREAMS[key]


class EposNet(object):

  def __init__(self, checkpoint, batch, height, width, num_objs, num_frags=64,
               model_variant='xception_65', encoder_output_stride=8,
               decoder_output_stride=4, atrous_rates=(12, 24, 36),
               multi_grid=None, device='cuda:0', dry_run=False, precision='fp32',
               decoder_hw=None):
    if precision not in PRECISIONS:
      raise ValueError('precision must be one of %s (got %r).' % (PRECISIONS, precision))
    self.precision = precision
    self.variant = W.variant(model_variant)
    self.model_variant = model_variant
    if encoder_output_stride != 8 or decoder_output_stride != 4:
      raise ValueError('Only encoder OS 8 / decoder OS 4 (common.py:127-135).')
    if not 1 <= num_frags <= 256:
      raise ValueError('num_frags must be in [1, 256] (got %d).' % num_frags)
    self.dry_run = bool(dry_run)
    if not self.dry_run and not torch.cuda.is_available():
      raise _lib.EposError('EposNet needs a HIP device (no CPU fallback).')
    self.lib = None if self.dry_run else _lib.load()
    self.dev = torch.device('meta' if self.dry_run else device)
    self.B, self.H, self.W = batch, height, width
    self.num_objs, self.num_frags = num_objs, num_frags
    self.atrous_rates = tuple(atrous_rates)
    self.multi_grid = list(multi_grid) if multi_grid else [1, 1, 1]
    self.decoder_hw = tuple(decoder_hw) if decoder_hw is not None else None
    self.ckpt = checkpoint
    self._keep = []
    self.ops = []
    self.post_ops = []
    self.flops = 0
    self.op_flops = {}
    self.op_kind = {}
    self.op_bytes = {}
    self.op_io = {}
    self._dw_reads = {}
    self._glue_bytes = 0
    self._graph = None
    self._graph_sparse = None
    self._graph_logits = None
    self._graph_alt, self.alt_skip = None, None
    self.trace_layers, self.trace_outputs = [], {}
    self._exprs = {}
    self.pad_rows = os.environ.get('EPOS_PAD_ROWS', '1') != '0'
    self._lds = {}
    self._col_ids = set()
    self._images_u8 = None
    self.pool_folded = False
    self._n_trunk_ops = 0
    self._obj_head_op, self._obj_head_flops = None, 0
    self._sparse_packs = None
    self._layer_consts = {}
# ... 5 lines not shown
    self._aspp_pw, self._aspp_dw = W.aspp_layers(self.atrous_rates)
    self._aspp = {}
    self.mode = MODES[precision](self)
    self.act_dtype = self.mode.dtype
    self._build_plan()

  use_h2 = property(lambda self: self.mode.use_h2)
  h2_layers = property(lambda self: self.mode.h2_layers)
  h2_refused = property(lambda self: self.mode.h2_refused)
  presplit_layers = property(lambda self: self.mode.presplit_layers)
  _n_slots = property(lambda self: self.mode._n_slots)
  _amax_table = property(lambda self: self.mode._amax_table)

  def _empty(self, *shape, dtype=torch.float32):
    t = torch.empty(*shape, dtype=dtype, device=self.dev)
    self._keep.append(t)
    return t

  def _act(self, b, h, w, c):
    line = self.mode.line
    ld = (c + line - 1) // line * line if (self.pad_rows and c >= 256) else c
    t = self._empty(b, h, w, ld, dtype=self.act_dtype)
    self._lds[id(t)] = ld
    return t

  def _abuf(self, *shape):
    return self._empty(*shape, dtype=self.act_dtype)

  def _ld(self, buf):
    return self._lds.get(id(buf), buf.shape[-1])

  def _dev(self, arr):
    t = torch.from_numpy(np.ascontiguousarray(arr)).to(self.dev)
    self._keep.append(t)
    return t

  def _set_expr(self, buf, expr, off=0, width=None):
    width = buf.shape[-1] if width is None else width
    ent = [e for e in self._exprs.get(id(buf), []) if e[0] != off]
    ent.append((off, width, expr))
    self._exprs[id(buf)] = sorted(ent)

  def _expr_of(self, buf, off=0, width=None):
    width = buf.shape[-1] if width is None else width
    ent = self._exprs[id(buf)]
    for o, w, e in ent:
      if o == off and w == width:
        return e
    parts, at = [], off
    for o, w, e in ent:
      if o == at and at < off + width:
        parts.append(e)
        at += w
    assert at == off + width and parts, ('no expression for the slice', off, width, ent)
    return 'concat(%s)' % ','.join(parts)

  @staticmethod
  def _relu_expr(e):
    return e if e.startswith('relu(') else 'relu(%s)' % e

  def _trace_layer(self, scope, op, kernel, stride, rate, padding, cin, cout, bn_eps,
                   bias, expr_in, out_hw):
    self.trace_layers.append({
        'scope': scope, 'op': op, 'kernel': [kernel, kernel], 'stride': stride,
        'rate': rate, 'padding': padding, 'cin': cin, 'cout': cout, 'bn_eps': bn_eps,
        'bias': bias, 'input': expr_in, 'out_hw': [int(out_hw[0]), int(out_hw[1])]})

  def _conv_params(self, scope, eps):
    w = self.ckpt[scope + '/weights']
    w = w.reshape(-1, w.shape[3])
    if eps is None:
      return w, np.ones(w.shape[1], np.float32), self.ckpt[scope + '/biases']
    scale, bias = W.fold_bn(self.ckpt, scope, eps, 'conv')
    return w, scale, bias

  def _dw_params(self, scope, eps):
    w = self.ckpt[scope + '/depthwise_weights']
    scale, bias = W.fold_bn(self.ckpt, scope, eps, 'dw')
    w9c = (w[:, :, :, 0].reshape(9, -1) * scale[None, :]).astype(np.float32)
    gain = float(np.abs(w9c.astype(np.float64)).sum(0).max())
    bias0 = float(np.abs(np.asarray(bias, np.float64)).max())
    return self._dev(w9c), self._dev(bias), gain, bias0

  def _fn(self, name):
    return None if self.lib is None else getattr(self.lib, name)

  @staticmethod
  def _call(name, fn, args):
    args = tuple(ctypes.byref(a) if isinstance(a, ctypes.Structure) else a for a in args)

    def run(stream):
      _lib.check(fn(*args, stream), name)
    return run

  def _launch(self, name, fn, args, kind='other', flops=0, nbytes=0):
    self.ops.append((name, self._call(name, fn, args)))
    self.op_bytes[name] = nbytes
    self.flops += flops
    self.op_flops[name] = flops
    self.op_kind[name] = kind

  def _conv1x1(self, name, eps, a, a_off, lda, m, k, c, c_off, ldc, relu, res=None,
               res_off=0, ldr=0, sub=1, ho=0, wo=0, hi=0, wi=0, group=None, track_out=True):
    conv = self._conv_params(name, eps)
    n = conv[0].shape[1]
    hw = (ho, wo) if sub > 1 else (c.shape[1:3] if c.dim() == 4 else (1, 1))
    self._trace_layer(name, 'conv2d', 1, sub, 1, 'SAME', k, n, eps, eps is None,
                      self._expr_of(a, a_off, k), hw)
    eout = 'L:' + name
    if res is not None:
      eout = 'add(%s)' % ','.join(sorted([eout, self._expr_of(res, res_off, n)]))
    self._set_expr(c, self._relu_expr(eout) if relu else eout, c_off, n)
    self.mode.pointwise(name, a, a_off, lda, m, k, conv, c, c_off, ldc, relu, res, res_off,
                        ldr, sub, ho, wo, hi, wi, group, track_out)

  def _depthwise(self, name, x, ldx, hi, wi, c, stride, rate, eps, relu_in, relu_out):
    B = self.B
    ho, wo = (hi - 1) // stride + 1, (wi - 1) // stride + 1
    w9c, bias, gain, bias0 = self._dw_params(name, eps)
    y = self._act(B, ho, wo, c)
    if name in W.DEPTHWISE_BACKWARD_LAYERS or name in W.DEPTHWISE_CHAIN_LAYERS or \
        name in self._aspp_dw:
      assert stride == 1 and not relu_in and relu_out, name
      self._dw_operands[name] = {'x': x, 'ldx': ldx, 'b': B, 'h': hi, 'w': wi, 'c': c,
                                 'rate': rate, 'w9c': w9c, 'bias': bias, 'eps': eps}
    ein = self._expr_of(x, 0, c)
    if relu_in:
      ein = self._relu_expr(ein)
    if stride > 1:
      ein = 'pad(%s,%d,%d)' % (ein, rate, rate)
    self._trace_layer(name, 'depthwise_conv2d', 3, stride, rate,
                      'SAME' if stride == 1 else 'VALID', c, c, eps, False, ein, (ho, wo))
    self._set_expr(y, self._relu_expr('L:' + name) if relu_out else 'L:' + name, 0, c)
    e = y.element_size()
    self._dw_reads[id(y)] = e * B * hi * wi * c + 40 * c
    self.mode.depthwise(name, x, y, gain, bias0, 2 * 9 * B * ho * wo * c,
                        e * (B * hi * wi * c + B * ho * wo * c) + 40 * c,
                        X=_ptr(x), ldx=ldx, w9c=_ptr(w9c), bias=_ptr(bias), Y=_ptr(y),
                        ldy=self._ld(y), B=B, Hi=hi, Wi=wi, Ho=ho, Wo=wo, C=c, stride=stride,
                        rate=rate, relu_in=int(relu_in), relu_out=int(relu_out))
    return y, ho, wo

  def _dense_conv(self, name, x, hi, wi, cin, stride, eps, rate=1, preprocess=None):
    conv = self._conv_params(name, eps)
    kk = self.ckpt[name + '/weights'].shape[0]
    cout = conv[0].shape[1]
    ho, wo = (hi - 1) // stride + 1, (wi - 1) // stride + 1
    pad = rate * (kk - 1) // 2
    ein = self._expr_of(x, 0, cin)
    if preprocess:
      assert ein == 'input'
      ein = PREPROCESS_EXPR[preprocess]
    if stride > 1:
      ein = 'pad(%s,%d,%d)' % (ein, pad, rate * (kk - 1) - pad)
    self._trace_layer(name, 'conv2d', kk, stride, rate, 'SAME' if stride == 1 else 'VALID',
                      cin, cout, eps, False, ein, (ho, wo))
    y = self._abuf(self.B, ho, wo, cout)
    self.mode.dense_conv(name, x, y, hi, wi, cin, ho, wo, kk, stride, rate, pad,
                         PREPROCESS[preprocess], conv)
    self._set_expr(y, 'relu(L:%s)' % name)
    return y, ho, wo, cout

  def _bottleneck(self, scope, x, hi, wi, cin, depth, db, stride, rate,
                  keep_conv3=False):
    eps = RESNET_BN_EPS
    B = self.B
# ... 150 lines not shown
      x, h, w, c, low_level = self._backbone_resnet()
    self.encoder = x
    eh, ew, ec = h, w, c

    nb = 2 + len(self.atrous_rates)
    cat = self._abuf(B, eh, ew, 256 * nb)
    ldcat = 256 * nb
    m_enc = B * eh * ew
    pooled = self._empty(B, ec)
    self.pool_folded = mode.mean('image_pooling/mean', x, pooled, eh * ew, ec)
    self._set_expr(pooled, 'mean(%s)' % self._expr_of(x, 0, ec))
    pool_feat = self._empty(B, 256)
    self._conv1x1('image_pooling', HEAD_BN_EPS, pooled, 0, ec, B, ec, pool_feat, 0, 256,
                  relu=True)
    mode.resize('image_pooling/resize', pool_feat, 256, cat, ldcat, 1, 1, eh, ew, 256)
    self._set_expr(cat, 'resize(%s,%dx%d)' % (self._expr_of(pool_feat), eh, ew), 0, 256)
    grp = []
    self._conv1x1('aspp0', HEAD_BN_EPS, x, 0, ec, m_enc, ec, cat, 256, ldcat, relu=True,
                  group=grp)
    for i, r in enumerate(self.atrous_rates, 1):
      d, _, _ = self._depthwise('aspp%d_depthwise' % i, x, ec, eh, ew, ec, 1, r,
                                HEAD_BN_EPS, False, True)
      self._conv1x1('aspp%d_pointwise' % i, HEAD_BN_EPS, d, 0, self._ld(d), m_enc, ec, cat,
                    256 * (i + 1), ldcat, relu=True, group=grp)
    mode.flush(grp)
    mode.join_absmax('image_pooling/absmax', pool_feat, 256, B, 256, cat)
    proj = self._abuf(B, eh, ew, 256)
    self._conv1x1('concat_projection', HEAD_BN_EPS, cat, 0, ldcat, m_enc, ldcat, proj, 0,
                  256, relu=True)
    self.aspp_concat, self.concat_projection = cat, proj
    self._aspp = {'encoder': x, 'eh': eh, 'ew': ew, 'ec': ec, 'pooled': pooled,
                  'pool_feat': pool_feat, 'aspp_concat': cat,
                  'encoder_relu': self._expr_of(x, 0, ec).startswith('relu(')}

    ll, lh, lw, lc = low_level
    dh = scale_dimension(H, 1.0 / 4)
    dw_ = scale_dimension(Wd, 1.0 / 4)
    assert (lh, lw) == (dh, dw_), ((lh, lw), (dh, dw_))
    if self.decoder_hw is not None:
      dh, dw_ = self.decoder_hw
    dcat = self._abuf(B, dh, dw_, 304)
    ldd = self._ld(dcat)
    mode.resize('decoder/resize', proj, 256, dcat, ldd, eh, ew, dh, dw_, 256)
    self._set_expr(dcat, self._expr_of(proj) if (eh, ew) == (dh, dw_) else
                   'resize(%s,%dx%d)' % (self._expr_of(proj), dh, dw_), 0, 256)
    m_dec = B * dh * dw_
    if (lh, lw) == (dh, dw_):
      self._conv1x1('decoder/feature_projection0', HEAD_BN_EPS, ll, 0, lc, m_dec, lc, dcat,
                    256, ldd, relu=True)
    else:
      low = self._abuf(B, lh, lw, 48)
      self._conv1x1('decoder/feature_projection0', HEAD_BN_EPS, ll, 0, lc, B * lh * lw, lc,
                    low, 0, 48, relu=True)
      mode.resize('decoder/resize_low_level', low, 48, dcat[..., 256:], ldd, lh, lw, dh, dw_,
                  48)
      self._set_expr(dcat, 'resize(%s,%dx%d)' % (self._expr_of(low), dh, dw_), 256, 48)
      mode.same_bound(dcat, low)
    mode.concat_bound(dcat, proj)
    self.decoder_concat = dcat[..., :304]
    self._chain = {'decoder_concat': dcat, 'ld_concat': ldd, 'concat_projection': proj,
                   'aspp_concat': cat, 'ld_aspp': ldcat, 'low_level': ll, 'low_level_c': lc,
                   'low_level_hw': (lh, lw), 'encoder_hw': (eh, ew), 'decoder_hw': (dh, dw_)}
    x, c = dcat, 304
    for j in range(2):
      scope = 'decoder/decoder_conv%d' % j
      d, _, _ = self._depthwise(scope + '_depthwise', x, self._ld(x), dh, dw_, c, 1, 1,
                                HEAD_BN_EPS, False, True)
      y = self._abuf(B, dh, dw_, 256)
      self._conv1x1(scope + '_pointwise', HEAD_BN_EPS, d, 0, self._ld(d), m_dec, c, y, 0,
                    256, relu=True)
      x, c = y, 256
    self.decoder_out = x
    self.out_h, self.out_w = dh, dw_

    self.logits = {}
    grp = []
    self._n_trunk_ops = len(self.ops)
    for name, ch in sorted(W.outputs_to_num_channels(
        self.num_objs, self.num_frags).items()):
      buf = self._empty(B, dh, dw_, ch)
      self._conv1x1('logits/' + name, None, x, 0, 256, m_dec, 256, buf, 0, ch, relu=False,
                    group=grp, track_out=False)
      self.logits[name] = buf
    if os.environ.get('EPOS_HEAD_NT_STORES', '1') == '1':
      for g in grp:
        g[1].c_stream = 1
    oname, oargs, oflops = [g for g in grp if g[0].endswith(W.PRED_OBJ_CONF)][0][:3]
    self.heads_group = None
    mode.flush(grp, heads=os.environ.get('EPOS_HEADS_KERNEL', '1') == '1')
    self._obj_head_op = (oname, mode.obj_head(oname, oargs))
    self._obj_head_flops = oflops
    self._decoder_x = x

    obj = self.logits[W.PRED_OBJ_CONF]
    frag = self.logits[W.PRED_FRAG_CONF]
    self.obj_label = self._empty(B, dh, dw_, dtype=torch.int64)
    O, F = self.num_objs, self.num_frags
    softmax = self._fn('epos_softmax_groups_f32')
    self.post_ops = [
        ('softmax_obj', self._call('softmax_obj', softmax, (_ptr(obj), m_dec, O + 1))),
        ('softmax_frag', self._call('softmax_frag', softmax, (_ptr(frag), m_dec * O, F))),
        ('argmax', self._call('argmax', self._fn('epos_argmax_i64'),
                              (_ptr(obj), O + 1, _ptr(self.obj_label), m_dec, O + 1)))]
    eo = self._expr_of(self.logits[W.PRED_OBJ_CONF])
    ef = self._expr_of(self.logits[W.PRED_FRAG_CONF])
    el = self._expr_of(self.logits[W.PRED_FRAG_LOC])
    self.trace_outputs = {
        W.PRED_OBJ_CONF: {'expr': 'softmax(%s)' % eo, 'shape': [B, dh, dw_, O + 1]},
        W.PRED_OBJ_LABEL: {'expr': 'argmax(softmax(%s))' % eo, 'shape': [B, dh, dw_]},
        W.PRED_FRAG_CONF: {'expr': 'softmax(reshape(%s,%s))' % (ef, [O, F]),
                           'shape': [B, dh, dw_, O, F]},
        W.PRED_FRAG_LOC: {'expr': 'reshape(%s,%s)' % (el, [O, F, 3]),
                          'shape': [B, dh, dw_, O, F, 3]}}
    mode.finish()

  def algorithmic_bytes(self, dense_heads=True):
    total = self._glue_bytes
    for a_bytes, rest, a_id in self.op_io.values():
      total += self._dw_reads.get(a_id, a_bytes) + rest
    if not dense_heads:
      total -= 4 * self.B * self.out_h * self.out_w * (4 * self.num_objs * self.num_frags)
    return total

  def _stream(self):
    return C.stream_handle(self.dev)[1]

  def sync_current(self):
    torch.cuda.current_stream(self.dev).synchronize()

  def run_plan(self, with_post=True, sparse=False, skip_kinds=()):
    s = self._stream()
    if not sparse:
      for name, fn in self.ops:
        if self.op_kind.get(name) not in skip_kinds:
          fn(s)
      if with_post and 'post' not in skip_kinds:
        for name, fn in self.post_ops:
          fn(s)
      return
    for name, fn in self.ops[:self._n_trunk_ops]:
      fn(s)
    self._obj_head_op[1](s)
    for name, fn in self.post_ops:
      if name != 'softmax_frag':
        fn(s)

  def _build_sparse_packs(self):
    O, F = self.num_objs, self.num_frags
    wc, bc = self._conv_params('logits/' + W.PRED_FRAG_CONF, None)[::2]
    wl, bl = self._conv_params('logits/' + W.PRED_FRAG_LOC, None)[::2]
    self._sparse_packs = [
        (self.mode.sparse_weights(wc[:, o * F:(o + 1) * F], bc[o * F:(o + 1) * F]),
         self.mode.sparse_weights(wl[:, o * 3 * F:(o + 1) * 3 * F],
                                  bl[o * 3 * F:(o + 1) * 3 * F]))
        for o in range(O)]

  def run_sparse_heads(self, slots, slots_dev):
    if self._sparse_packs is None:
      self._build_sparse_packs()
    O, F = self.num_objs, self.num_frags
    P = self.out_h * self.out_w
    x = self._decoder_x
    s = self._stream()
    flops = 0
    for kind, buf in enumerate((self.logits[W.PRED_FRAG_CONF], self.logits[W.PRED_FRAG_LOC])):
      n = F if kind == 0 else 3 * F
      ldc = O * n
      probs = [self.mode.sparse_problem(self._sparse_packs[obj_id - 1][kind], x, im * P * 256,
                                        buf, im * P * ldc + (obj_id - 1) * n, ldc, P, n)
               for im, obj_id in slots]
      flops += 2 * P * n * 256 * len(slots)
      for i in range(0, len(probs), 8):
        self.mode.sparse_launch(probs[i:i + 8], s)
    if slots:
      _lib.check(self.lib.epos_softmax_slots_f32(_ptr(self.logits[W.PRED_FRAG_CONF]),
                                                 _ptr(slots_dev), len(slots), P, O, F, s),
                 'softmax_slots')
    return flops

  def _need_fp32_plan(self, what, device=True):
    if self.precision != 'fp32':
      raise NotImplementedError('%s: precision=%r nets are not supported' % (
          what, self.precision))
    if device and self.lib is None:
# ... 129 lines not shown
            'encoder_relu': r['encoder_relu'], 'pooled': r['pooled'],
            'pool_feat': r['pool_feat'], 'aspp_concat': r['aspp_concat'],
            'rates': self.atrous_rates,
            'pointwise': {s: self._pointwise_record(s, None, eps)
                          for s, eps in self._aspp_pw.items()},
            'depthwise': {s: dict(self._dw_operands[s]) for s in self._aspp_dw}}

  def aspp_constants(self, scope):
    if scope not in self._aspp_pw and scope not in self._aspp_dw:
      raise ValueError('%r is not an ASPP layer (%s)' % (
          scope, ', '.join(list(self._aspp_pw) + list(self._aspp_dw))))
    kept = self._pw_consts if scope in self._aspp_pw else self._dw_consts
    if scope not in kept:
      first = 'weights' if scope in self._aspp_pw else 'depthwise_weights'
      kept[scope] = tuple(
          torch.from_numpy(np.ascontiguousarray(self.ckpt[scope + '/' + v], np.float32)).to(self.dev)
          for v in (first, 'BatchNorm/gamma', 'BatchNorm/moving_mean',
                    'BatchNorm/moving_variance'))
    return kept[scope]

  def chain_operands(self):
    self._need_fp32_plan('chain_operands', device=False)
    r = self._chain
    ll, (lh, lw) = r['low_level'], r['low_level_hw']
    return {'decoder_concat': r['decoder_concat'][..., :304],
            'concat_projection': r['concat_projection'], 'aspp_concat': r['aspp_concat'],
            'low_level': ll.view(self.B, lh, lw, -1)[..., :r['low_level_c']],
            'low_level_hw': (lh, lw), 'encoder_hw': r['encoder_hw'],
            'decoder_hw': r['decoder_hw']}

  def depthwise_operand(self, name=W.DECODER_CONV1_DEPTHWISE):
    return self._depthwise_record('depthwise_operand', name, W.DEPTHWISE_BACKWARD_LAYERS)

  def crossed_depthwise_operand(self, name=W.DECODER_CONV0_DEPTHWISE):
    return self._depthwise_record('crossed_depthwise_operand', name, W.DEPTHWISE_CHAIN_LAYERS)

  def _depthwise_record(self, what, name, table):
    self._need_fp32_plan(what, device=False)
    if name not in table or name not in self._dw_operands:
      raise ValueError('%r is not a depthwise layer the backward pass crosses (%s)' % (
          name, ', '.join(table)))
    return dict(self._dw_operands[name])

  def depthwise_constants(self, name=W.DECODER_CONV1_DEPTHWISE):
    return self._depthwise_consts(name, W.DEPTHWISE_BACKWARD_LAYERS)

  def crossed_depthwise_constants(self, name=W.DECODER_CONV0_DEPTHWISE):
    return self._depthwise_consts(name, W.DEPTHWISE_CHAIN_LAYERS)

  def _depthwise_consts(self, name, table):
    if name not in table:
      raise ValueError('%r is not a depthwise layer the backward pass crosses (%s)' % (
          name, ', '.join(table)))
    if name not in self._dw_consts:
      self._dw_consts[name] = tuple(
          torch.from_numpy(np.ascontiguousarray(self.ckpt[name + '/' + v], np.float32)).to(self.dev)
          for v in ('depthwise_weights', 'BatchNorm/gamma', 'BatchNorm/moving_mean',
                    'BatchNorm/moving_variance'))
    return self._dw_consts[name]

  def layer_constants(self, name=W.DECODER_CONV1_POINTWISE):
    if name not in self._layer_consts:
      self._layer_consts[name] = tuple(
          torch.from_numpy(np.ascontiguousarray(self.ckpt[name + '/BatchNorm/' + v],
                                                np.float32)).to(self.dev)
          for v in ('moving_mean', 'moving_variance'))
    return self._layer_consts[name]

  def set_images(self, images):
    t = torch.as_tensor(images)
    if t.dtype == torch.uint8:
      n = self.B * self.H * self.W * 3
      t = t.reshape(-1)
      if t.numel() != n:
        raise ValueError('images: expected %d values, got %d' % (n, t.numel()))
      if not t.is_cuda and t.is_pinned() and t.is_contiguous() and t.data_ptr() % 16 == 0 and \
          os.environ.get('EPOS_UPLOAD', 'zerocopy') == 'zerocopy':
        src = t
      else:
        if self._images_u8 is None:
          self._images_u8 = torch.empty(n, dtype=torch.uint8, device=self.dev)
        self._images_u8.copy_(t, non_blocking=True)
        src = self._images_u8
      _lib.check(self.lib.epos_u8_to_f32(_ptr(src), _ptr(self.images), n, self._stream()),
                 'u8_to_f32')
      return
    if t.dtype != torch.float32:
      if t.is_cuda:
        raise TypeError('device images must be float32 or uint8, got %s' % t.dtype)
      t = t.float()
    self.images.copy_(t.reshape(self.B, self.H, self.W, 3), non_blocking=True)

  def capture_graph(self, sparse=False):
    torch.cuda.synchronize(self.dev)
    side = _capture_stream(self.dev)
    with torch.cuda.stream(side):
      self.run_plan(sparse=sparse)
    torch.cuda.synchronize(self.dev)
    g = torch.cuda.CUDAGraph()
    with torch.cuda.graph(g, stream=side):
      self.run_plan(sparse=sparse)
    if sparse:
      self._graph_sparse = g
    else:
      self._graph = g
    return g

  def capture_alt(self, skip_kinds):
    if skip_kinds is None:
      self._graph_alt, self.alt_skip = None, None
      return
    torch.cuda.synchronize(self.dev)
    g = torch.cuda.CUDAGraph()
    with torch.cuda.graph(g, stream=_capture_stream(self.dev)):
      self.run_plan(skip_kinds=tuple(skip_kinds))
    self._graph_alt, self.alt_skip = g, tuple(skip_kinds)

  def forward(self, images=None, use_graph=False, sparse=False):
    if images is not None:
      self.set_images(images)
    if use_graph:
      if sparse:
        if self._graph_sparse is None:
          self.capture_graph(sparse=True)
        self._graph_sparse.replay()
      elif self._graph_alt is not None:
        self._graph_alt.replay()
      else:
        if self._graph is None:
          self.capture_graph()
        self._graph.replay()
    else:
      self.run_plan(sparse=sparse)
    return self.outputs()

  def forward_logits(self, images=None, use_graph=False):
    if images is not None:
      self.set_images(images)
    if use_graph:
      if self._graph_logits is None:
        torch.cuda.synchronize(self.dev)
        side = _capture_stream(self.dev)
        with torch.cuda.stream(side):
          self.run_plan(with_post=False)
        torch.cuda.synchronize(self.dev)
        g = torch.cuda.CUDAGraph()
        with torch.cuda.graph(g, stream=side):
          self.run_plan(with_post=False)
        self._graph_logits = g
      self._graph_logits.replay()
    else:
      self.run_plan(with_post=False)
    out = self.outputs()
    del out[W.PRED_OBJ_LABEL]
    return out

  def outputs(self):
    B, h, w = self.B, self.out_h, self.out_w
    O, F = self.num_objs, self.num_frags
    return {
        W.PRED_OBJ_CONF: self.logits[W.PRED_OBJ_CONF],
        W.PRED_OBJ_LABEL: self.obj_label,
        W.PRED_FRAG_CONF: self.logits[W.PRED_FRAG_CONF].view(B, h, w, O, F),
        W.PRED_FRAG_LOC: self.logits[W.PRED_FRAG_LOC].view(B, h, w, O, F, 3),
    }

  def time_ops(self, iters=3, warm=0):
    out = []
# ... 15 lines not shown
```

### epos_amd/net_modes.py

```python
import ctypes
import os

import numpy as np
import torch

from epos_amd import _lib
from epos_amd._call import ptr as _ptr
from epos_amd import weights as W


def _fold(w_kn, scale, kmult):
  k, n = w_kn.shape
  w = w_kn.astype(np.float32) * scale[None, :].astype(np.float32)
  kpad = -(-k // kmult) * kmult
  if kpad != k:
    w = np.concatenate([w, np.zeros((kpad - k, n), np.float32)], 0)
  return np.ascontiguousarray(w)


def _pack(fn, w, dtype):
  src = w.ctypes.data_as(ctypes.c_void_p)
  total = fn(src, w.shape[0], w.shape[1], None)
  if total <= 0:
    return None
  dst = np.empty(total, dtype)
  fn(src, w.shape[0], w.shape[1], dst.ctypes.data_as(ctypes.c_void_p))
  return dst


def _bias(bias, n, mult):
  b = np.zeros(-(-n // mult) * mult, np.float32)
  b[:n] = bias
  return b


class Fp32Mode(object):

  dtype, line = torch.float32, 32
  MAX_SLOTS = 512

  def __init__(self, net):
    self.net = net
    fn = net._fn
    self.gemm = fn('epos_pointwise_conv_grouped_f32')
    self.gemm1 = fn('epos_pointwise_conv_f32')
    self.heads = fn('epos_heads_gemm_f32')
    self.dw = fn('epos_depthwise3x3_f32')
    self.conv3x3 = fn('epos_conv3x3_f32')
    self.im2col3x3 = fn('epos_im2col3x3_f32')
    self.im2col_k = fn('epos_im2col_f32')
    self.absmax = fn('epos_absmax_f32')
    self.amax_clear = fn('epos_amax_clear')
    self.avg_pool = fn('epos_global_avg_pool_f32')
    self.avg_pool_partial = fn('epos_global_avg_pool_partial_f32')
    self.resize_fn = fn('epos_resize_bilinear_f32')
    self.subsample = fn('epos_subsample_f32')
    self.add_relu = fn('epos_add_relu_f32')
    self.maxpool = fn('epos_maxpool3x3_s2_f32')
    self.pack_plain = fn('epos_pack_pointwise_weights')
    self.pack_split = fn('epos_pack_pointwise_weights_split')
    self.pack_h2 = fn('epos_pack_pointwise_weights_h2')
    self._amax_table = torch.zeros(self.MAX_SLOTS * _lib.AMAX_WORDS, dtype=torch.int32,
                                   device=net.dev)
    self._slot_count = ctypes.c_int64(0)
    self._bounds = {}
    self.use_h2 = (os.environ.get('EPOS_GEMM_H2', '1') != '0' and
                   os.environ.get('EPOS_GEMM_SPLIT', '1') != '0')
    self.use_presplit = self.use_h2 and os.environ.get('EPOS_H2_PRESPLIT', '1') == '1'
    self._dw_h2 = {}
    self.h2_layers, self.h2_refused, self.presplit_layers = [], [], []
    self.packs = {}
    self.layer_operands = {}
    self.pack_device = fn('epos_pack_weights_device_f32')
    self._last_pw = None
    self._first_im2col = None

  @property
  def _n_slots(self):
    return self._slot_count.value

  def _new_slot(self):
    i = self._slot_count.value
    if i >= self.MAX_SLOTS:
      raise _lib.EposError('absmax slot table exhausted')
    self._slot_count.value = i + 1
    return i

  def _slot_ptr(self, i):
    return _ptr(self._amax_table, i * _lib.AMAX_WORDS) if i is not None else None

  def _set_bound(self, buf, slot, slot2=None, gain=0.0, bias=0.0):
    self._bounds[id(buf)] = (slot, slot2, float(gain), float(bias))

  def _out_slot(self, buf, n, ldc, off=0):
    if n % 4 or ldc % 4 or off % 4:
      return None
    b = self._bounds.get(id(buf))
    if b is not None and b[1] is None and b[2] == 0.0:
      return b[0]
    slot = self._new_slot()
    self._set_bound(buf, slot)
    return slot

  def same_bound(self, dst, src):
    b = self._bounds.get(id(src))
    if b is not None:
      self._bounds[id(dst)] = b

  def concat_bound(self, cat, left):
    lb, cb = self._bounds.get(id(left)), self._bounds.get(id(cat))
    if lb is not None and cb is not None:
      self._set_bound(cat, cb[0], lb[0])
    else:
      self._bounds.pop(id(cat), None)

  def track_absmax(self, name, y, ld, rows, n):
    slot = self._new_slot()
    self._set_bound(y, slot)
    self.net._launch(name, self.absmax, (_ptr(y), ld, rows, n, self._slot_ptr(slot)))

  def join_absmax(self, name, x, ld, rows, n, into):
    b = self._bounds.get(id(into))
    if b is not None:
      self.net._launch(name, self.absmax, (_ptr(x), ld, rows, n, self._slot_ptr(b[0])))

  def _weights(self, name, conv, h2):
    w_kn, scale, bias = conv
    k, n = w_kn.shape
    kpad = -(-k // 4) * 4
    net = self.net
    if net.dry_run:
      wp, bp, ws, wh = net._empty(1), net._empty(1), net._empty(1), None
      if h2:
        wh = net._empty(1)
    else:
      w = _fold(w_kn, scale, 4)
      wh = _pack(self.pack_h2, w, np.uint8) if h2 else None
      wh = net._dev(wh) if wh is not None else None
      wp, bp = net._dev(_pack(self.pack_plain, w, np.float32)), net._dev(_bias(bias, n, 128))
      ws = net._dev(_pack(self.pack_split, w, np.uint8))
    if h2 and name is not None:
      (self.h2_layers if wh is not None else self.h2_refused).append(name)
    return wp, bp, ws, wh, kpad

  def begin(self):
    self.net._launch('amax_clear', self.amax_clear, (_ptr(self._amax_table), self._slot_count))

  def pointwise(self, name, a, a_off, lda, m, k, conv, c, c_off, ldc, relu, res=None, res_off=0,
                ldr=0, sub=1, ho=0, wo=0, hi=0, wi=0, group=None, track_out=True):
    net = self.net
    ab = self._bounds.get(id(a)) if self.use_h2 else None
    wp, bp, ws, wh, kpad = self._weights(name, conv, ab is not None and m > 8)
    n = conv[0].shape[1]
    assert kpad == k or (kpad > k and lda >= kpad), (name, k, kpad, lda)
    if name in W.TRAINABLE_LAYERS:
      assert kpad == k, name
      self.packs[name] = (k, n, (wp, bp, ws, wh))
    dwa = self._dw_h2.pop(id(a), None)
    presplit = False
    if dwa is not None:
      presplit = wh is not None and sub == 1 and a_off == 0
      dwa.y_h2 = int(presplit)
      if presplit:
        self.presplit_layers.append(name)
    track = track_out and m > 8 and (res is None or ldr % 4 == 0)
    cslot = self._out_slot(c, n, ldc, c_off) if track else None
    h = wh is not None
    args = _lib.PointwiseArgs(
        A=_ptr(a, a_off), lda=lda, Wp=_ptr(wp), bias=_ptr(bp),
        R=_ptr(res, res_off) if res is not None else None, ldr=ldr,
        C=_ptr(c, c_off), ldc=ldc, M=m, N=n, K=kpad, relu=int(relu), sub=sub,
        Ho=ho, Wo=wo, Hi=hi, Wi=wi, Ws=_ptr(ws), Wh=_ptr(wh) if h else None,
        a_amax=self._slot_ptr(ab[0]) if h else None,
        a_amax2=self._slot_ptr(ab[1]) if h else None,
        a_gain=ab[2] if h else 0.0, a_bias=ab[3] if h else 0.0,
        a_presplit=int(presplit), c_amax=self._slot_ptr(cslot))
    if (name in W.TRAINABLE_LAYERS and name not in W.LOGITS_LAYERS) or \
        name in W.POINTWISE_CHAIN_LAYERS or name in net._aspp_pw:
      assert a_off == 0 and sub == 1 and res is None, name
      self.layer_operands[name] = (a, lda, m, k, n, args, ab if h else None)
    nbytes = 4 * (m * k + k * n + m * n + (m * n if res is not None else 0))
    net.op_io[name] = (4 * m * k, nbytes - 4 * m * k, id(a))
    if group is not None:
      group.append((name, args, 2 * m * n * k, nbytes))
      return
    net._launch(name, self.gemm, (args, 1), 'gemm', 2 * m * n * k, nbytes)
    self._last_pw = (c, args, h and res is None and c_off == 0 and n % 4 == 0)

  def flush(self, group, heads=False):
    for kind in sorted({g[1].a_presplit for g in group}):
      part = [g for g in group if g[1].a_presplit == kind]
      arr = (_lib.PointwiseArgs * len(part))(*[g[1] for g in part])
      fn = self.heads if heads and not kind else self.gemm
      if fn is self.heads:
        self.net.heads_group = (arr, len(part))
      self.net._launch('+'.join(g[0] for g in part), fn, (arr, len(part)), 'gemm',
                       sum(g[2] for g in part), sum(g[3] for g in part))
    del group[:]

  def depthwise(self, name, x, y, gain, bias0, flops, nbytes, **fields):
    xb = self._bounds.get(id(x))
    if xb is not None:
      self._set_bound(y, xb[0], xb[1], gain * (xb[2] if xb[2] else 1.0), gain * xb[3] + bias0)
    args = _lib.DepthwiseArgs(**fields)
    yb = self._bounds.get(id(y))
    if yb is not None and self.use_presplit:
      args.y_h2 = 1
      args.x_amax, args.x_amax2 = self._slot_ptr(yb[0]), self._slot_ptr(yb[1])
      args.gain, args.bias0 = yb[2], yb[3]
      self._dw_h2[id(y)] = args
    self.net._launch(name, self.dw, (args,), 'dw', flops, nbytes)

  def dense_conv(self, name, x, y, hi, wi, cin, ho, wo, kk, stride, rate, pad, preprocess,
                 conv):
    net, B = self.net, self.net.B
    cout = y.shape[3]
    k = kk * kk * cin
    if kk == 3 and cin % 32 == 0 and preprocess == _lib.PREPROCESS_NONE:
      xb = self._bounds.get(id(x))
      wp, bp, ws, wh, _ = self._weights(name, conv, xb is not None and xb[1] is None and
                                        xb[2] == 0.0)
      yslot = self._out_slot(y, cout, cout)
      args = _lib.Conv3x3Args(X=_ptr(x), ldx=cin, Wp=_ptr(wp), bias=_ptr(bp), Y=_ptr(y),
                              ldy=cout, B=B, H=hi, W=wi, Cin=cin, Cout=cout, stride=stride,
                              rate=rate, relu=1, Ws=_ptr(ws),
                              Wh=_ptr(wh) if wh is not None else None,
                              x_amax=self._slot_ptr(xb[0]) if wh is not None else None,
                              y_amax=self._slot_ptr(yslot))
      net._launch(name, self.conv3x3, (args,), 'gemm', 2 * B * ho * wo * cout * k,
                  4 * (B * hi * wi * cin + k * cout + B * ho * wo * cout))
      net.op_io[name] = (4 * B * hi * wi * cin, 4 * (k * cout + B * ho * wo * cout), id(x))
      return
    ldcol = -(-k // 4) * 4
    m = B * ho * wo
    col = net._empty(m, ldcol)
    net._col_ids.add(id(col))
    geom = dict(X=_ptr(x), ldx=cin, col=_ptr(col), ldcol=ldcol, B=B, Hi=hi, Wi=wi, Ho=ho, Wo=wo,
                C=cin, stride=stride, rate=rate, pad=pad, preprocess=preprocess)
    if kk == 3:
      args, fn, words = _lib.Im2colArgs(**geom), self.im2col3x3, m * ldcol
    else:
      args = _lib.Im2colKArgs(k=kk, mean_rgb=(ctypes.c_float * 3)(*W.MEAN_RGB), **geom)
      fn, words = self.im2col_k, wo * ldcol // 4 * min(B * ho, 65535)
    if self._first_im2col is None:
      self._first_im2col = (name + '/im2col', args, words)
    net._launch(name + '/im2col', fn, (args,), 'im2col')
    self.pointwise(name, col, 0, ldcol, m, k, conv, y, 0, cout, relu=True)
    net.op_io[name] = (x.element_size() * B * hi * wi * cin, net.op_io[name][1], id(x))

  def mean(self, name, x, pooled, hw, c):
    net, B = self.net, self.net.B
    lp = self._last_pw
    fold = (not net.dry_run and os.environ.get('EPOS_POOL_FOLD', '1') == '1' and
            lp is not None and lp[0] is x and lp[2] and (hw % 32 == 0 or B == 1))
    if fold:
      blocks = (hw + 31) // 32
      part = net._empty(B * blocks, c)
      lp[1].col_sums = _ptr(part)
      lp[1].col_ld = c
      net._launch(name, self.avg_pool_partial, (_ptr(part), c, _ptr(pooled), B, blocks, c, hw))
    else:
      net._launch(name, self.avg_pool, (_ptr(x), c, _ptr(pooled), B, hw, c))
    return bool(fold)

  def resize(self, name, x, ldx, y, ldy, hi, wi, ho, wo, c):
    self.net._launch(name, self.resize_fn,
                     (_ptr(x), ldx, _ptr(y), ldy, self.net.B, hi, wi, ho, wo, c))

  def obj_head(self, name, args):
    return self.net._call(name, self.gemm1, (args,))

  def sparse_weights(self, w_kn, bias):
    wp, bp, ws, wh, _ = self._weights(None, (w_kn, np.ones(w_kn.shape[1], np.float32), bias),
                                      True)
    return wp, bp, ws, wh

  def sparse_problem(self, pack, x, x_off, c, c_off, ldc, m, n):
    wp, bp, ws, wh = pack
    xb = self._bounds.get(id(x))
    if xb is None:
      wh = None
    h = wh is not None
    return _lib.PointwiseArgs(
        A=_ptr(x, x_off), lda=256, Wp=_ptr(wp), bias=_ptr(bp), R=None, ldr=0,
        C=_ptr(c, c_off), ldc=ldc, M=m, N=n, K=256, relu=0, sub=1, Ws=_ptr(ws),
        Wh=_ptr(wh) if h else None,
        a_amax=self._slot_ptr(xb[0]) if h else None,
        a_amax2=self._slot_ptr(xb[1]) if h else None,
        a_gain=xb[2] if h else 0.0, a_bias=xb[3] if h else 0.0)

  def sparse_launch(self, probs, stream):
    arr = (_lib.PointwiseArgs * len(probs))(*probs)
    _lib.check(self.gemm(arr, len(probs), stream), 'sparse heads')

  def pack_problem(self, pack, w, bias, col0, n):
    wp, bp, ws, wh = pack
    return _lib.WeightPackArgs(W=_ptr(w), ldw=w.shape[-1], col0=col0, bias=_ptr(bias),
                               plain=_ptr(wp), split=_ptr(ws),
                               h2=_ptr(wh) if wh is not None else None, bias_pad=_ptr(bp),
                               K=w.shape[-2], N=n)

  def pack_launch(self, probs, status, stream, what='set_weights'):
    arr = (_lib.WeightPackArgs * len(probs))(*probs)
    _lib.check(self.pack_device(arr, len(probs), _ptr(status), stream), what)

  def slot_words(self, i):
    if i is None:
      return None
    return self._amax_table[i * _lib.AMAX_WORDS:(i + 1) * _lib.AMAX_WORDS]

  def finish(self):
    net, fi = self.net, self._first_im2col
    words = self._n_slots * _lib.AMAX_WORDS
    if (not net.dry_run and fi is not None and len(net.ops) > 1 and
        net.ops[0][0] == 'amax_clear' and net.ops[1][0] == fi[0] and words <= fi[2] and
        os.environ.get('EPOS_AMAX_CLEAR_FOLD', '1') == '1'):
      fi[1].amax_clear = _ptr(self._amax_table)
      fi[1].amax_words = words
      del net.ops[0]
      net._n_trunk_ops -= 1


class Bf16Mode(object):

  dtype, line = torch.bfloat16, 64
  use_h2 = False
  _n_slots = 0

  def __init__(self, net):
    self.net = net
    fn = net._fn
    self.gemm = fn('epos_pointwise_conv_bf16')
    self.gemm_f32 = fn('epos_pointwise_conv_grouped_f32')
    self.dw = fn('epos_depthwise3x3_bf16')
    self.im2col = fn('epos_im2col_bf16')
    self.avg_pool = fn('epos_global_avg_pool_bf16')
    self.resize_fn = fn('epos_resize_bilinear_bf16')
    self.subsample = fn('epos_subsample_bf16')
    self.add_relu = fn('epos_add_relu_bf16')
    self.maxpool = fn('epos_maxpool3x3_s2_bf16')
    self.pack = fn('epos_pack_pointwise_weights_bf16')
    self.pack_plain = fn('epos_pack_pointwise_weights')
    self.pack_split = fn('epos_pack_pointwise_weights_split')
    self.h2_layers, self.h2_refused, self.presplit_layers = [], [], []
    self._col_users, self._col_elems = [], 0

  def _weights(self, conv):
    w_kn, scale, bias = conv
    k, n = w_kn.shape
    kpad = -(-k // 8) * 8
# ... 121 lines not shown
```

### include/epos_hip.h

```cpp
#ifndef EPOS_HIP_H_
#define EPOS_HIP_H_

#include <stdint.h>

#ifdef __cplusplus
extern "C" {
#endif

#define EPOS_OK 0
#define EPOS_E_INVALID (-1)
#define EPOS_E_CAPACITY (-2)
#define EPOS_E_NODEVICE (-3)
#define EPOS_E_INTERNAL (-4)
#define EPOS_E_HIP_BASE (-1000)

#define EPOS_ABI_VERSION 7

int epos_abi_version(void);
const char* epos_last_error(void);
int epos_device_count(void);
int epos_clock_probe(int64_t* out2, int microseconds, void* stream);


int64_t epos_pack_pointwise_weights(const float* w_kn, int K, int N, float* dst);

int64_t epos_pack_pointwise_weights_split(const float* w_kn, int K, int N, void* dst);

int64_t epos_pack_pointwise_weights_h2(const float* w_kn, int K, int N, void* dst);

#define EPOS_AMAX_WORDS 64
int epos_absmax_f32(const float* X, int64_t ldx, int64_t rows, int64_t cols,
                    uint32_t* slot, void* stream);
int epos_amax_clear(uint32_t* slots, int64_t n_slots, void* stream);

typedef struct EposPointwiseArgs {
  const float* A; int64_t lda;
  const float* Wp; const float* bias;
  const float* R; int64_t ldr;
  float* C; int64_t ldc;
  int32_t M, N, K;
  int32_t relu;
  int32_t relu_in;
  int32_t sub;
  int32_t Ho, Wo, Hi, Wi;
  const void* Ws;
  const void* Wh;
  const uint32_t* a_amax;
  const uint32_t* a_amax2;
  float a_gain, a_bias;
  int32_t a_presplit;
  uint32_t* c_amax;
  float* col_sums;
  int64_t col_ld;
  int32_t c_stream;
  int32_t reserved0;
} EposPointwiseArgs;
int epos_pointwise_conv_f32(const EposPointwiseArgs* args, void* stream);

int epos_pointwise_conv_grouped_f32(const EposPointwiseArgs* args, int count,
                                    void* stream);

int epos_heads_gemm_f32(const EposPointwiseArgs* args, int count, void* stream);
int epos_heads_gemm_plan(const EposPointwiseArgs* args, int count, int cus, int32_t* plan);


typedef struct EposConv3x3Args {
  const float* X; int64_t ldx;
  const float* Wp; const float* bias;
  float* Y; int64_t ldy;
  int32_t B, H, W, Cin, Cout;
  int32_t stride, rate;
  int32_t relu;
  const void* Ws;
  const void* Wh;
  const uint32_t* x_amax;
  uint32_t* y_amax;
} EposConv3x3Args;
int epos_conv3x3_f32(const EposConv3x3Args* args, void* stream);

typedef struct EposDepthwiseArgs {
  const float* X; int64_t ldx;
  const float* w9c; const float* bias;
  float* Y; int64_t ldy;
  int32_t B, Hi, Wi, Ho, Wo, C;
  int32_t stride, rate;
  int32_t relu_in, relu_out;
  int32_t y_h2;
  const uint32_t* x_amax;
  const uint32_t* x_amax2;
  float gain, bias0;
} EposDepthwiseArgs;
int epos_depthwise3x3_f32(const EposDepthwiseArgs* args, void* stream);

int epos_set_h2_narrow_tile_limit(int max_tiles);
typedef struct EposSepConvArgs {
  EposDepthwiseArgs dw;
  EposPointwiseArgs pw;
} EposSepConvArgs;
int epos_separable_conv_f32(const EposSepConvArgs* args, void* stream);

typedef struct EposIm2colArgs {
  const float* X; int64_t ldx;
  float* col; int64_t ldcol;
  int32_t B, Hi, Wi, Ho, Wo, C;
  int32_t stride, rate, pad;
  int32_t preprocess;
  uint32_t* amax_clear;
  int64_t amax_words;
} EposIm2colArgs;
int epos_im2col3x3_f32(const EposIm2colArgs* args, void* stream);

#define EPOS_PREPROCESS_NONE 0
#define EPOS_PREPROCESS_UNIT_RANGE 1
#define EPOS_PREPROCESS_SUB_MEAN 2
typedef struct EposIm2colKArgs {
  const float* X; int64_t ldx;
  float* col; int64_t ldcol;
  int32_t B, Hi, Wi, Ho, Wo, C;
  int32_t k, stride, rate, pad;
  int32_t preprocess;
  float mean_rgb[3];
  uint32_t* amax_clear;
  int64_t amax_words;
} EposIm2colKArgs;
int epos_im2col_f32(const EposIm2colKArgs* args, void* stream);

int epos_global_avg_pool_partial_f32(const float* P, int64_t ldp, float* Y, int32_t B,
                                     int32_t blocks, int32_t C, int32_t hw, void* stream);

int epos_global_avg_pool_f32(const float* X, int64_t ldx, float* Y, int B,
                             int HW, int C, void* stream);

int epos_resize_bilinear_f32(const float* X, int64_t ldx, float* Y, int64_t ldy,
                             int B, int Hi, int Wi, int Ho, int Wo, int C,
                             void* stream);

int epos_maxpool3x3_s2_f32(const float* X, int64_t ldx, float* Y, int64_t ldy,
                           int B, int Hi, int Wi, int C, void* stream);
int epos_subsample_f32(const float* X, int64_t ldx, float* Y, int64_t ldy, int B,
                       int Hi, int Wi, int C, int factor, void* stream);
int epos_add_relu_f32(const float* A, const float* B, float* Y, int64_t n,
                      void* stream);

int epos_scatter_blocks_f32(float* dst, const int64_t* offsets, const float* src,
                            int64_t n_blocks, int width, void* stream);

int epos_u8_to_f32(const uint8_t* X, float* Y, int64_t n, void* stream);

int epos_softmax_groups_f32(float* X, int64_t n_groups, int G, void* stream);

int epos_argmax_i64(const float* X, int64_t ldx, int64_t* labels, int64_t P,
                    int C, void* stream);

typedef struct EposCorrSlot {
  int32_t image;
  int32_t obj_id;
} EposCorrSlot;

int epos_softmax_slots_f32(float* X, const EposCorrSlot* slots, int S, int P,
                           int O, int F, void* stream);

int epos_corr_count(const float* obj_confs, const float* frag_confs,
                    const EposCorrSlot* slots , int S, int B, int P,
                    int O, int F, float min_obj_conf, float min_frag_rel_conf,
                    int32_t* px_off, int32_t* corr_off, uint64_t* frag_mask,
                    int32_t* totals, void* stream);

typedef struct EposCorrOut {
  int64_t* px_id; int64_t* frag_id;
  double* coord_2d; double* coord_3d;
  float* conf; float* conf_obj; float* conf_frag;
} EposCorrOut;
int epos_corr_fill(const float* obj_confs, const float* frag_confs,
                   const float* frag_coords, const double* frag_centers,
                   const double* frag_sizes, const EposCorrSlot* slots, int S,
                   int B, int P, int W, int O, int F, double inv_scale,
                   const int32_t* px_off, const int32_t* corr_off,
                   const uint64_t* frag_mask, const int64_t* slot_base,
                   int64_t capacity, const EposCorrOut* out, int32_t* overflow,
                   void* stream);

int epos_corr_slot_bases(const int32_t* totals, int S, int64_t* slot_base,
                         void* stream);

int epos_corr_order_tile_rows(void);
int64_t epos_corr_order_workspace_bytes(int S, int64_t capacity);
int epos_corr_order_by_conf(const float* conf, const int64_t* px_id, const double* coord_2d,
                            const double* coord_3d, const int64_t* slot_base, int S,
                            int64_t capacity, int W, int64_t max_corr, int always_sort,
                            void* work, int64_t* slot_base_out, double* coord_2d_out,
                            double* coord_3d_out, int32_t* src_row_out, int32_t* yorder,
                            int32_t* ypos, void* stream);

int epos_project_to_mesh_f64(const double* pts, int64_t n, const double* verts,
                             int64_t nv, const int32_t* faces, int64_t nf, double* out,
                             int32_t* face_idx, void* stream);

typedef struct EposMeshRec {
  int64_t tri_off;
  int64_t fid_off;
  int64_t box_off[4];
  int32_t count[4];
  int32_t nf, nleaf, nalways, top;
  double near_lo[3], near_hi[3];
} EposMeshRec;
int epos_project_rows_to_mesh_f64(double* coord_3d, const int64_t* slot_base,
                                  const EposCorrSlot* slots, int S, int64_t capacity,
                                  const EposMeshRec* recs, int num_objs, const double* geom,
                                  const int32_t* face_ids, int32_t* face_idx,
                                  int32_t* visited, void* stream);

int epos_fragmentation_fps(const double* vertices, int64_t V, int num_frags,
                           double* nn_dist, double* centers, int32_t* center_idx,
                           int32_t* vertex_frag_ids, void* stream);

typedef struct EposFitParams {
  double threshold;
  double neighborhood_ball_radius;
  double spatial_coherence_weight;
  double scaling_from_millimeters;
  double max_tanimoto_similarity;
  double conf;
  double proposal_engine_conf;
  double min_coverage;
  double min_triangle_area;
  int32_t max_iters;
  int32_t min_point_number;
  int32_t max_model_number;
  int32_t max_model_number_for_optimization;
  int32_t use_prosac;
  int32_t lo_iters;
  int32_t gc_sweeps;
  int32_t pearl_iters;
} EposFitParams;
void epos_fit_params_default(EposFitParams* p);

int epos_find6d_poses(const double* xy, const double* xyz, int64_t n,
                      const double* K, const EposFitParams* p, uint64_t seed,
                      double* poses_out, int32_t* labels_out, double* scores_out,
                      int32_t max_k);

int64_t epos_fit_workspace_bytes(int S, int64_t n_capacity, const EposFitParams* p,
                                 int32_t max_k);
// ... 374 lines not shown
```

Baseline: 397.2.

## Add per-family cache store policies with write-through for GEMM outputs feeding depthwise

Adds a store-policy selector (plain, nontemporal stream, or write-through via sc1 / buffer store bit) threaded through depthwise, pointwise/heads GEMM, conv3x3, im2col, resize, u8 conversion and softmax kernels, configured per producer family from an environment table. By default, GEMM outputs consumed by a depthwise conv use write-through stores, while heads and softmax stores are streamed. The aim is to reduce cache pollution and coherence or writeback cost between producer and consumer kernels. It adds template instantiations and inline asm stores, and the benefit depends on how MI355X cache behaviour treats these hints.

```diff
diff --git a/epos_amd/_lib.py b/epos_amd/_lib.py
--- a/epos_amd/_lib.py
+++ b/epos_amd/_lib.py
@@ -45,9 +45,12 @@
       ('Ho', ctypes.c_int32), ('Wo', ctypes.c_int32), ('C', ctypes.c_int32),
       ('stride', ctypes.c_int32), ('rate', ctypes.c_int32),
       ('relu_in', ctypes.c_int32), ('relu_out', ctypes.c_int32),
-      ('y_h2', ctypes.c_int32), ('x_amax', vp), ('x_amax2', vp),
+      ('y_h2', ctypes.c_int32), ('y_store', ctypes.c_int32), ('x_amax', vp), ('x_amax2', vp),
       ('gain', ctypes.c_float), ('bias0', ctypes.c_float),
   ]
+
+
+STORE_PLAIN, STORE_STREAM, STORE_WT = 0, 1, 2
 
 
 class SepConvArgs(ctypes.Structure):
@@ -273,6 +276,17 @@
 
 SYMBOLS = {
     'epos_abi_version': (ctypes.c_int, []),
+    'epos_store_policy_layout': (None, [c_i64p]),
+    'epos_conv3x3_policy_f32': (ctypes.c_int, [ctypes.POINTER(Conv3x3Args), ctypes.c_int, vp]),
+    'epos_im2col3x3_policy_f32': (ctypes.c_int, [ctypes.POINTER(Im2colArgs), ctypes.c_int, vp]),
+    'epos_resize_bilinear_policy_f32': (ctypes.c_int, [
+        vp, ctypes.c_int64, vp, ctypes.c_int64, ctypes.c_int, ctypes.c_int,
+        ctypes.c_int, ctypes.c_int, ctypes.c_int, ctypes.c_int, ctypes.c_int, vp]),
+    'epos_u8_to_f32_policy': (ctypes.c_int, [vp, vp, ctypes.c_int64, ctypes.c_int, vp]),
+    'epos_softmax_groups_policy_f32': (ctypes.c_int, [
+        vp, ctypes.c_int64, ctypes.c_int, ctypes.c_int, vp]),
+    'epos_softmax_slots_policy_f32': (ctypes.c_int, [
+        vp, vp, ctypes.c_int, ctypes.c_int, ctypes.c_int, ctypes.c_int, ctypes.c_int, vp]),
     'epos_last_error': (ctypes.c_char_p, []),
     'epos_device_count': (ctypes.c_int, []),
     'epos_clock_probe': (ctypes.c_int, [ctypes.c_void_p, ctypes.c_int, ctypes.c_void_p]),
diff --git a/epos_amd/csrc/common.h b/epos_amd/csrc/common.h
--- a/epos_amd/csrc/common.h
+++ b/epos_amd/csrc/common.h
@@ -2,6 +2,8 @@
 #include <hip/hip_runtime.h>
 #include <stdint.h>
 #include <stdio.h>
+
+#include <type_traits>
 
 #include "../../include/epos_hip.h"
 
@@ -31,6 +33,26 @@
                      fmaxf(v.w, 0.f));
 }
 
+typedef float st16_f32x4 __attribute__((ext_vector_type(4)));
+__device__ __forceinline__ void st16_wt(float* p, float4 v) {
+  const st16_f32x4 x = {v.x, v.y, v.z, v.w};
+  asm volatile("global_store_dwordx4 %0, %1, off sc1\n\ts_nop 1" : : "v"(p), "v"(x) : "memory");
+}
+__device__ __forceinline__ void st16_cached(float* p, float4 v, bool stream) {
+  const st16_f32x4 x = {v.x, v.y, v.z, v.w};
+  if (stream) __builtin_nontemporal_store(x, reinterpret_cast<st16_f32x4*>(p));
+  else *reinterpret_cast<st16_f32x4*>(p) = x;
+}
+__device__ __forceinline__ void st16_policy(float* p, float4 v, int policy) {
+  if (policy == EPOS_STORE_WT) st16_wt(p, v);
+  else st16_cached(p, v, policy == EPOS_STORE_STREAM);
+}
+template <class Body>
+__device__ __forceinline__ void st16_runs(int policy, Body body) {
+  if (policy == EPOS_STORE_WT) body(std::true_type{});
+  else body(std::false_type{});
+}
+
 constexpr int DW_PRIO = 3;
 #define EPOS_SET_PRIO(p) do { if ((p) > 0) __builtin_amdgcn_s_setprio(p); } while (0)
 
diff --git a/epos_amd/csrc/glue.hip b/epos_amd/csrc/glue.hip
--- a/epos_amd/csrc/glue.hip
+++ b/epos_amd/csrc/glue.hip
@@ -6,7 +6,7 @@
 template <class SP, class DP>
 __global__ __launch_bounds__(256) void resize_bilinear_kernel(
     const typename SP::elem* X, int64_t ldx, typename DP::elem* Y, int64_t ldy, int Hi, int Wi,
-    int Ho, int Wo, int cn, float sy, float sx, int64_t total) {
+    int Ho, int Wo, int cn, float sy, float sx, int64_t total, int policy) {
   static_assert(SP::n == DP::n, "one thread reads the channels it writes");
   const int64_t id = static_cast<int64_t>(blockIdx.x) * blockDim.x + threadIdx.x;
   if (id >= total) return;
@@ -14,7 +14,10 @@
   const BilinearSrc<typename SP::elem> src = {X, ldx, Hi, Wi, sy, sx};
   float o[DP::n];
   bilinear_sample<SP>(src, p.b, p.yo, p.xo, p.c, o);
-  DP::store(Y + pixel_offset(p, Ho, Wo, ldy), o);
+  if constexpr (std::is_same<DP, F32Pack<4>>::value)
+    st16_policy(Y + pixel_offset(p, Ho, Wo, ldy), make_float4(o[0], o[1], o[2], o[3]), policy);
+  else
+    DP::store(Y + pixel_offset(p, Ho, Wo, ldy), o);
 }
 
 template <class P>
@@ -93,12 +96,12 @@
 
 template <class SP, class DP>
 int resize(const typename SP::elem* X, int64_t ldx, typename DP::elem* Y, int64_t ldy, int B,
-           int Hi, int Wi, int Ho, int Wo, int C, void* stream) {
+           int Hi, int Wi, int Ho, int Wo, int C, void* stream, int policy = EPOS_STORE_PLAIN) {
   const int cn = C / DP::n;
   const int64_t total = static_cast<int64_t>(B) * Ho * Wo * cn;
   hipLaunchKernelGGL((resize_bilinear_kernel<SP, DP>), dim3(blocks_for(total, 256)), dim3(256),
                      0, static_cast<hipStream_t>(stream), X, ldx, Y, ldy, Hi, Wi, Ho, Wo, cn,
-                     align_corners_scale(Hi, Ho), align_corners_scale(Wi, Wo), total);
+                     align_corners_scale(Hi, Ho), align_corners_scale(Wi, Wo), total, policy);
   return launch_status("resize_bilinear_kernel");
 }
 
@@ -150,11 +153,24 @@
 
 using namespace epos;
 
+static int resize_f32(const char* fn, const float* X, int64_t ldx, float* Y, int64_t ldy, int B,
+                      int Hi, int Wi, int Ho, int Wo, int C, int policy, void* stream) {
+  EPOS_REQUIRE_FN(fn, Ho >= 1 && Wo >= 1, "empty map");
+  EPOS_REQUIRE_FN(fn, policy >= EPOS_STORE_PLAIN && policy <= EPOS_STORE_WT,
+                  "policy must be an EPOS_STORE_* policy");
+  if (int rc = check_maps(fn, X, ldx, Y, ldy, B, Hi, Wi, C, 4)) return rc;
+  return resize<F32, F32>(X, ldx, Y, ldy, B, Hi, Wi, Ho, Wo, C, stream, policy);
+}
+
+extern "C" int epos_resize_bilinear_policy_f32(const float* X, int64_t ldx, float* Y, int64_t ldy,
+                                               int B, int Hi, int Wi, int Ho, int Wo, int C,
+                                               int policy, void* stream) {
+  return resize_f32(__func__, X, ldx, Y, ldy, B, Hi, Wi, Ho, Wo, C, policy, stream);
+}
+
 extern "C" int epos_resize_bilinear_f32(const float* X, int64_t ldx, float* Y, int64_t ldy, int B,
                                         int Hi, int Wi, int Ho, int Wo, int C, void* stream) {
-  EPOS_REQUIRE(Ho >= 1 && Wo >= 1, "empty map");
-  if (int rc = check_maps(__func__, X, ldx, Y, ldy, B, Hi, Wi, C, 4)) return rc;
-  return resize<F32, F32>(X, ldx, Y, ldy, B, Hi, Wi, Ho, Wo, C, stream);
+  return resize_f32(__func__, X, ldx, Y, ldy, B, Hi, Wi, Ho, Wo, C, EPOS_STORE_PLAIN, stream);
 }
 
 extern "C" int epos_resize_bilinear_bf16(const void* X, int64_t ldx, int x_f32, uint16_t* Y,
diff --git a/epos_amd/csrc/heads_gemm_h2.hip b/epos_amd/csrc/heads_gemm_h2.hip
--- a/epos_amd/csrc/heads_gemm_h2.hip
+++ b/epos_amd/csrc/heads_gemm_h2.hip
@@ -257,14 +257,23 @@
     if (vec) {
       const unsigned oob = n < cur.N ? 0u : HD_OOB;
       const unsigned nb4 = static_cast<unsigned>(n) * 4u;
-#pragma unroll
-      for (int i = 0; i < 8; ++i) {
-        const int off = static_cast<int>(
-            opaque(((row0 + 4 * i) * static_cast<unsigned>(ldc) * 4u + nb4) | oob));
-        if (q.c_stream)
-          __builtin_amdgcn_raw_buffer_store_b128(__builtin_bit_cast(hd_u32x4, v[i]), rsrc, off, 0, 2);
-        else
-          __builtin_amdgcn_raw_buffer_store_b128(__builtin_bit_cast(hd_u32x4, v[i]), rsrc, off, 0, 0);
+      if (q.c_stream == EPOS_STORE_WT) {
+#pragma unroll
+        for (int i = 0; i < 8; ++i) {
+          const int off = static_cast<int>(
+              opaque(((row0 + 4 * i) * static_cast<unsigned>(ldc) * 4u + nb4) | oob));
+          __builtin_amdgcn_raw_buffer_store_b128(__builtin_bit_cast(hd_u32x4, v[i]), rsrc, off, 0, 16);
+        }
+      } else {
+#pragma unroll
+        for (int i = 0; i < 8; ++i) {
+          const int off = static_cast<int>(
+              opaque(((row0 + 4 * i) * static_cast<unsigned>(ldc) * 4u + nb4) | oob));
+          if (q.c_stream == EPOS_STORE_STREAM)
+            __builtin_amdgcn_raw_buffer_store_b128(__builtin_bit_cast(hd_u32x4, v[i]), rsrc, off, 0, 2);
+          else
+            __builtin_amdgcn_raw_buffer_store_b128(__builtin_bit_cast(hd_u32x4, v[i]), rsrc, off, 0, 0);
+        }
       }
     } else {
 #pragma unroll
diff --git a/epos_amd/csrc/layers.hip b/epos_amd/csrc/layers.hip
--- a/epos_amd/csrc/layers.hip
+++ b/epos_amd/csrc/layers.hip
@@ -6,17 +6,19 @@
 namespace epos {
 namespace {
 
-typedef unsigned dw_u32x4 __attribute__((ext_vector_type(4)));
-__device__ __forceinline__ void st4_h2(float* p, float4 v, float s) {
-  dw_u32x4 o;
+__device__ __forceinline__ float4 pack4_h2(float4 v, float s) {
   unsigned h0, h1, m0, m1;
   h2_split_pair(v.x, v.y, s, h0, m0);
   h2_split_pair(v.z, v.w, s, h1, m1);
-  o[0] = h0; o[1] = h1; o[2] = m0; o[3] = m1;
-  *reinterpret_cast<dw_u32x4*>(p) = o;
-}
+  return make_float4(__uint_as_float(h0), __uint_as_float(h1), __uint_as_float(m0),
+                     __uint_as_float(m1));
+}
+__device__ __forceinline__ void st4_any(float* p, float4 v, bool h2, float s, int policy) {
+  if (h2) st16_policy(p, pack4_h2(v, s), policy); else st16_policy(p, v, policy);
+}
+template <int ST>
 __device__ __forceinline__ void st4_any(float* p, float4 v, bool h2, float s) {
-  if (h2) st4_h2(p, v, s); else st4(p, v);
+  st4_any(p, v, h2, s, ST);
 }
 __device__ __forceinline__ float4 fma4(float4 a, float4 b, float4 c) {
   return make_float4(fmaf(a.x, b.x, c.x), fmaf(a.y, b.y, c.y),
@@ -63,7 +65,7 @@
     float hinv;
     h2_scale_finish(am_raw, am_raw2, p.gain, p.bias0, hs, hinv);
   }
-  if (live) st4_any(p.Y + pixel_offset(o, p.Ho, p.Wo, p.ldy), acc, h2, hs);
+  if (live) st4_any(p.Y + pixel_offset(o, p.Ho, p.Wo, p.ldy), acc, h2, hs, p.y_store);
 }
 
 constexpr int DW_REP = 1;
@@ -95,7 +97,7 @@
   return make_float4(relu_1op(v.x), relu_1op(v.y), relu_1op(v.z), relu_1op(v.w));
 }
 
-template <int L, bool RELU_IN, bool RELU_OUT, int ROWS>
+template <int L, bool RELU_IN, bool RELU_OUT, int ROWS, int ST>
 __global__ __launch_bounds__(256, (ROWS == 2 ? DW_MIN_BLOCKS2 : DW_MIN_BLOCKS)) void depthwise3x3_s1_kernel(
     EposDepthwiseArgs p, int c4n, int nres, int nchunk, int nrows, DwPartition part) {
   constexpr int NR = ROWS + 2;
@@ -233,7 +235,7 @@
           acc = fma4(col[j + 2][ky + rr], w[ky * 3 + 2], acc);
         }
         if (RELU_OUT) acc = relu4_1op(acc);
-        st4_any(yb + (static_cast<unsigned>((x0 + j * r) * ldy) + (rr ? yrow1 : 0u)), acc, h2, hs);
+        st4_any<ST>(yb + (static_cast<unsigned>((x0 + j * r) * ldy) + (rr ? yrow1 : 0u)), acc, h2, hs);
       }
     }
     continue;
@@ -282,7 +284,7 @@
         acc = fma4(col[j + 2][ky + rr], w[ky * 3 + 2], acc);
       }
       if (RELU_OUT) acc = relu4_1op(acc);
-      if (x < p.Wo && live) st4_any(yb + (static_cast<unsigned>(x * ldy) + (rr ? yrow1 : 0u)), acc, h2, hs);
+      if (x < p.Wo && live) st4_any<ST>(yb + (static_cast<unsigned>(x * ldy) + (rr ? yrow1 : 0u)), acc, h2, hs);
     }
   }
   }
@@ -422,17 +424,23 @@
 }
 
 __global__ __launch_bounds__(256) void u8_to_f32_kernel(const uint8_t* __restrict__ X,
-                                                        float* __restrict__ Y, int64_t n) {
+                                                        float* __restrict__ Y, int64_t n,
+                                                        int policy) {
   const int64_t i = (static_cast<int64_t>(blockIdx.x) * blockDim.x + threadIdx.x) * 16;
   if (i >= n) return;
   if (i + 16 <= n) {
     const uint4 v = *reinterpret_cast<const uint4*>(X + i);
     const unsigned w[4] = {v.x, v.y, v.z, v.w};
-#pragma unroll
-    for (int q = 0; q < 4; ++q)
-      reinterpret_cast<float4*>(Y + i)[q] = make_float4(
-          static_cast<float>(w[q] & 0xffu), static_cast<float>((w[q] >> 8) & 0xffu),
-          static_cast<float>((w[q] >> 16) & 0xffu), static_cast<float>(w[q] >> 24));
+    st16_runs(policy, [&](auto wt) {
+#pragma unroll
+      for (int q = 0; q < 4; ++q) {
+        const float4 f = make_float4(
+            static_cast<float>(w[q] & 0xffu), static_cast<float>((w[q] >> 8) & 0xffu),
+            static_cast<float>((w[q] >> 16) & 0xffu), static_cast<float>(w[q] >> 24));
+        if constexpr (decltype(wt)::value) st16_wt(Y + i + 4 * q, f);
+        else st16_cached(Y + i + 4 * q, f, policy == EPOS_STORE_STREAM);
+      }
+    });
   } else {
     for (int64_t j = i; j < n; ++j) Y[j] = static_cast<float>(X[j]);
   }
@@ -451,6 +459,8 @@
   EPOS_REQUIRE(a->stride == 1 || (a->stride == 2 && a->rate == 1),
                "stride 2 requires rate 1");
   EPOS_REQUIRE(!a->y_h2 || a->x_amax, "y_h2 needs the absmax slot of X (x_amax)");
+  EPOS_REQUIRE(a->y_store >= EPOS_STORE_PLAIN && a->y_store <= EPOS_STORE_WT,
+               "y_store must be an EPOS_STORE_* policy");
   const int c4n = a->C / 4;
   hipStream_t st = static_cast<hipStream_t>(stream);
   if (a->stride == 1 && a->Hi == a->Ho && a->Wi == a->Wo) {
@@ -527,9 +537,15 @@
       const char* e = getenv("EPOS_DW_LDS_KB");
       return e ? static_cast<unsigned>(atoi(e)) * 1024u : 0u;
     }();
+#define EPOS_DW_LAUNCH_ST(RI, RO, RW, ST)                                                   \
+    hipLaunchKernelGGL((depthwise3x3_s1_kernel<L, RI, RO, RW, ST>), dim3(grid), dim3(threads), \
+                       lds_pad, st, *a, c4n, nres, nchunk, nrows, part)
 #define EPOS_DW_LAUNCH(RI, RO, RW)                                                          \
-    hipLaunchKernelGGL((depthwise3x3_s1_kernel<L, RI, RO, RW>), dim3(grid), dim3(threads),   \
-                       lds_pad, st, *a, c4n, nres, nchunk, nrows, part)
+    do {                                                                                     \
+      if (a->y_store == EPOS_STORE_WT) EPOS_DW_LAUNCH_ST(RI, RO, RW, EPOS_STORE_WT);         \
+      else if (a->y_store == EPOS_STORE_STREAM) EPOS_DW_LAUNCH_ST(RI, RO, RW, EPOS_STORE_STREAM); \
+      else EPOS_DW_LAUNCH_ST(RI, RO, RW, EPOS_STORE_PLAIN);                                  \
+    } while (0)
     if (ROWS == 2) {
       if (v == 0) EPOS_DW_LAUNCH(false, false, 2);
       else if (v == 1) EPOS_DW_LAUNCH(false, true, 2);
@@ -541,6 +557,7 @@
       else if (v == 2) EPOS_DW_LAUNCH(true, false, 1);
       else EPOS_DW_LAUNCH(true, true, 1);
     }
+#undef EPOS_DW_LAUNCH_ST
 #undef EPOS_DW_LAUNCH
     return launch_status("depthwise3x3_s1_kernel");
   }
@@ -551,16 +568,26 @@
   return launch_status("depthwise3x3_kernel");
 }
 
-extern "C" int epos_im2col3x3_f32(const EposIm2colArgs* a, void* stream) {
-  EPOS_REQUIRE(a && a->X && a->col, "null pointer");
-  EPOS_REQUIRE(a->ldcol >= 9 * a->C, "ldcol too small");
+static int im2col3x3(const char* fn, const EposIm2colArgs* a, int policy, void* stream) {
+  EPOS_REQUIRE_FN(fn, a && a->X && a->col, "null pointer");
+  EPOS_REQUIRE_FN(fn, policy >= EPOS_STORE_PLAIN && policy <= EPOS_STORE_WT,
+                  "policy must be an EPOS_STORE_* policy");
+  EPOS_REQUIRE_FN(fn, a->ldcol >= 9 * a->C, "ldcol too small");
   const int64_t total = static_cast<int64_t>(a->B) * a->Ho * a->Wo * a->ldcol;
-  EPOS_REQUIRE(!a->amax_clear || (a->amax_words >= 0 && a->amax_words <= total),
-               "amax_words exceeds the launch's thread count");
+  EPOS_REQUIRE_FN(fn, !a->amax_clear || (a->amax_words >= 0 && a->amax_words <= total),
+                  "amax_words exceeds the launch's thread count");
   if (total == 0) return EPOS_OK;
   hipLaunchKernelGGL(im2col3x3_kernel, dim3(blocks_for(total, 256)), dim3(256), 0,
                      static_cast<hipStream_t>(stream), *a, total);
   return launch_status("im2col3x3_kernel");
+}
+
+extern "C" int epos_im2col3x3_policy_f32(const EposIm2colArgs* a, int policy, void* stream) {
+  return im2col3x3(__func__, a, policy, stream);
+}
+
+extern "C" int epos_im2col3x3_f32(const EposIm2colArgs* a, void* stream) {
+  return im2col3x3(__func__, a, EPOS_STORE_PLAIN, stream);
 }
 
 extern "C" int epos_im2col_f32(const EposIm2colKArgs* a, void* stream) {
@@ -666,12 +693,24 @@
   return launch_status("scatter_blocks_kernel");
 }
 
-extern "C" int epos_u8_to_f32(const uint8_t* X, float* Y, int64_t n, void* stream) {
-  EPOS_REQUIRE(X && Y, "null pointer");
-  EPOS_REQUIRE(reinterpret_cast<uintptr_t>(X) % 16 == 0 &&
-               reinterpret_cast<uintptr_t>(Y) % 16 == 0, "16-byte aligned buffers");
+static int u8_to_f32(const char* fn, const uint8_t* X, float* Y, int64_t n, int policy,
+                     void* stream) {
+  EPOS_REQUIRE_FN(fn, X && Y, "null pointer");
+  EPOS_REQUIRE_FN(fn, reinterpret_cast<uintptr_t>(X) % 16 == 0 &&
+                  reinterpret_cast<uintptr_t>(Y) % 16 == 0, "16-byte aligned buffers");
+  EPOS_REQUIRE_FN(fn, policy >= EPOS_STORE_PLAIN && policy <= EPOS_STORE_WT,
+                  "policy must be an EPOS_STORE_* policy");
   if (n == 0) return EPOS_OK;
   hipLaunchKernelGGL(u8_to_f32_kernel, dim3(blocks_for((n + 15) / 16, 256)), dim3(256), 0,
-                     static_cast<hipStream_t>(stream), X, Y, n);
+                     static_cast<hipStream_t>(stream), X, Y, n, policy);
   return launch_status("u8_to_f32_kernel");
 }
+
+extern "C" int epos_u8_to_f32_policy(const uint8_t* X, float* Y, int64_t n, int policy,
+                                     void* stream) {
+  return u8_to_f32(__func__, X, Y, n, policy, stream);
+}
+
+extern "C" int epos_u8_to_f32(const uint8_t* X, float* Y, int64_t n, void* stream) {
+  return u8_to_f32(__func__, X, Y, n, EPOS_STORE_PLAIN, stream);
+}
diff --git a/epos_amd/csrc/pointwise_gemm.h b/epos_amd/csrc/pointwise_gemm.h
--- a/epos_amd/csrc/pointwise_gemm.h
+++ b/epos_amd/csrc/pointwise_gemm.h
@@ -161,20 +161,25 @@
   __builtin_amdgcn_fence(__ATOMIC_RELEASE, "wavefront");
   const bool relu = p.relu != 0;
   float amax = 0.f;
+  const bool nt = p.c_stream == EPOS_STORE_STREAM;
+  st16_runs(p.c_stream, [&](auto wt) {
 #pragma unroll
-  for (int i = 0; i < NI; ++i) {
-    const int row = r0 + i * RPI;
-    const int m = m0w + row;
-    float4 v = *reinterpret_cast<const float4*>(ws + row * EPR + c4 * 4);
-    if (HAS_RES) {
-      v.x += rv[i].x; v.y += rv[i].y; v.z += rv[i].z; v.w += rv[i].w;
+    for (int i = 0; i < NI; ++i) {
+      const int row = r0 + i * RPI;
+      const int m = m0w + row;
+      float4 v = *reinterpret_cast<const float4*>(ws + row * EPR + c4 * 4);
+      if (HAS_RES) {
+        v.x += rv[i].x; v.y += rv[i].y; v.z += rv[i].z; v.w += rv[i].w;
+      }
+      if (relu) v = relu4(v);
+      if (m < M && n < N) {
+        float* dst = p.C + static_cast<int64_t>(m) * p.ldc + n;
+        if constexpr (decltype(wt)::value) st16_wt(dst, v);
+        else st16_cached(dst, v, nt);
+        amax = fmaxf(fmaxf(amax, fmaxf(fabsf(v.x), fabsf(v.y))), fmaxf(fabsf(v.z), fabsf(v.w)));
+      }
     }
-    if (relu) v = relu4(v);
-    if (m < M && n < N) {
-      *reinterpret_cast<float4*>(p.C + static_cast<int64_t>(m) * p.ldc + n) = v;
-      amax = fmaxf(fmaxf(amax, fmaxf(fabsf(v.x), fabsf(v.y))), fmaxf(fabsf(v.z), fabsf(v.w)));
-    }
-  }
+  });
   if (p.c_amax) amax_publish(p.c_amax, amax, lane, static_cast<int>(blockIdx.x) * 4 + (m0w >> 5));
 }
 
diff --git a/epos_amd/csrc/pointwise_gemm.hip b/epos_amd/csrc/pointwise_gemm.hip
--- a/epos_amd/csrc/pointwise_gemm.hip
+++ b/epos_amd/csrc/pointwise_gemm.hip
@@ -118,6 +118,8 @@
   for (int i = 0; i < count; ++i) {
     const EposPointwiseArgs& a = args[i];
     EPOS_REQUIRE(a.reserved0 == 0, "EposPointwiseArgs.reserved0 must be 0 (ABI 7)");
+    EPOS_REQUIRE(a.c_stream >= EPOS_STORE_PLAIN && a.c_stream <= EPOS_STORE_WT,
+                 "EposPointwiseArgs.c_stream must be an EPOS_STORE_* policy");
     if (a.col_sums)
       EPOS_REQUIRE(!a.R && a.N % 4 == 0 && a.col_ld % 4 == 0 && a.col_ld >= a.N &&
                        (reinterpret_cast<uintptr_t>(a.col_sums) & 15) == 0 &&
@@ -136,6 +138,8 @@
     return epos_pointwise_conv_grouped_f32(args, count, stream);
   for (int i = 0; i < count; ++i) {
     EPOS_REQUIRE(args[i].reserved0 == 0, "EposPointwiseArgs.reserved0 must be 0 (ABI 7)");
+    EPOS_REQUIRE(args[i].c_stream >= EPOS_STORE_PLAIN && args[i].c_stream <= EPOS_STORE_WT,
+                 "EposPointwiseArgs.c_stream must be an EPOS_STORE_* policy");
     const int rc = validate(&args[i]);
     if (rc) return rc;
   }
@@ -201,16 +205,18 @@
   return no_fp32_mfma("epos_pointwise_conv_grouped_f32");
 }
 
-extern "C" int epos_conv3x3_f32(const EposConv3x3Args* a, void* stream) {
-  using namespace epos;
-  EPOS_REQUIRE(a && a->X && a->Wp && a->Y, "null pointer");
-  EPOS_REQUIRE(a->Cin > 0 && a->Cin % BK == 0, "Cin must be a multiple of 32");
-  EPOS_REQUIRE(a->ldx % 4 == 0 && a->ldx >= a->Cin, "ldx: multiple of 4, >= Cin");
-  EPOS_REQUIRE((reinterpret_cast<uintptr_t>(a->X) & 15) == 0, "X must be 16-byte aligned");
-  EPOS_REQUIRE(a->B > 0 && a->H > 0 && a->W > 0 && a->Cout > 0, "empty problem");
-  EPOS_REQUIRE((a->stride == 1 || a->stride == 2) && a->rate >= 1, "stride 1|2, rate >= 1");
+static int conv3x3(const char* fn, const EposConv3x3Args* a, int policy, void* stream) {
+  using namespace epos;
+  EPOS_REQUIRE_FN(fn, policy >= EPOS_STORE_PLAIN && policy <= EPOS_STORE_WT,
+                  "policy must be an EPOS_STORE_* policy");
+  EPOS_REQUIRE_FN(fn, a && a->X && a->Wp && a->Y, "null pointer");
+  EPOS_REQUIRE_FN(fn, a->Cin > 0 && a->Cin % BK == 0, "Cin must be a multiple of 32");
+  EPOS_REQUIRE_FN(fn, a->ldx % 4 == 0 && a->ldx >= a->Cin, "ldx: multiple of 4, >= Cin");
+  EPOS_REQUIRE_FN(fn, (reinterpret_cast<uintptr_t>(a->X) & 15) == 0, "X must be 16-byte aligned");
+  EPOS_REQUIRE_FN(fn, a->B > 0 && a->H > 0 && a->W > 0 && a->Cout > 0, "empty problem");
+  EPOS_REQUIRE_FN(fn, (a->stride == 1 || a->stride == 2) && a->rate >= 1, "stride 1|2, rate >= 1");
   const int ho = (a->H - 1) / a->stride + 1, wo = (a->W - 1) / a->stride + 1;
-  EPOS_REQUIRE(static_cast<int64_t>(a->B) * a->H * a->W < (1LL << 31), "too many pixels");
+  EPOS_REQUIRE_FN(fn, static_cast<int64_t>(a->B) * a->H * a->W < (1LL << 31), "too many pixels");
   EposPointwiseArgs p = {};
   p.A = a->X; p.lda = a->ldx;
   p.Wp = a->Wp; p.bias = a->bias;
@@ -221,6 +227,7 @@
   p.Ho = ho; p.Wo = wo; p.Hi = a->H; p.Wi = a->W;
   p.Ws = a->Ws;
   p.Wh = a->Wh; p.a_amax = a->x_amax; p.c_amax = a->y_amax;
+  p.c_stream = policy;
   {
     const int rc = validate(&p);
     if (rc) return rc;
@@ -232,7 +239,15 @@
     return launch_grouped_split(&p, 1, static_cast<hipStream_t>(stream), &cin, &rate);
   if (fp32_mfma_ref().dma)
     return fp32_mfma_ref().dma(&p, 1, static_cast<hipStream_t>(stream), &cin, &rate);
-  return no_fp32_mfma("epos_conv3x3_f32");
+  return no_fp32_mfma(fn);
+}
+
+extern "C" int epos_conv3x3_f32(const EposConv3x3Args* a, void* stream) {
+  return conv3x3(__func__, a, EPOS_STORE_PLAIN, stream);
+}
+
+extern "C" int epos_conv3x3_policy_f32(const EposConv3x3Args* a, int policy, void* stream) {
+  return conv3x3(__func__, a, policy, stream);
 }
 
 extern "C" int epos_separable_conv_f32(const EposSepConvArgs* a, void* stream) {
diff --git a/epos_amd/csrc/pointwise_gemm_h2.hip b/epos_amd/csrc/pointwise_gemm_h2.hip
--- a/epos_amd/csrc/pointwise_gemm_h2.hip
+++ b/epos_amd/csrc/pointwise_gemm_h2.hip
@@ -157,21 +157,20 @@
   float* crow = p.C + (static_cast<int64_t>(m0w + r0) * p.ldc + n);
   const int64_t cstep = static_cast<int64_t>(RPI) * p.ldc;
   const bool nok = n < N;
-  const bool nt = p.c_stream != 0;
-#pragma unroll
-  for (int i = 0; i < NI; ++i) {
-    const int m = m0w + r0 + i * RPI;
-    if (m < M && nok) {
-      if (nt) {
-        const h2_f32x4 nv = {v[i].x, v[i].y, v[i].z, v[i].w};
-        __builtin_nontemporal_store(nv, reinterpret_cast<h2_f32x4*>(crow));
+  const bool nt = p.c_stream == EPOS_STORE_STREAM;
+  st16_runs(p.c_stream, [&](auto wt) {
+#pragma unroll
+    for (int i = 0; i < NI; ++i) {
+      const int m = m0w + r0 + i * RPI;
+      if (m < M && nok) {
+        if constexpr (decltype(wt)::value) st16_wt(crow, v[i]);
+        else st16_cached(crow, v[i], nt);
+        amax = fmaxf(fmaxf(amax, fmaxf(fabsf(v[i].x), fabsf(v[i].y))),
+                     fmaxf(fabsf(v[i].z), fabsf(v[i].w)));
       }
-      else *reinterpret_cast<float4*>(crow) = v[i];
-      amax = fmaxf(fmaxf(amax, fmaxf(fabsf(v[i].x), fabsf(v[i].y))),
-                   fmaxf(fabsf(v[i].z), fabsf(v[i].w)));
-    }
-    crow += cstep;
-  }
+      crow += cstep;
+    }
+  });
 #ifdef EPOS_GEMM_TRACE
   if (g_h2_trace && threadIdx.x == 0) g_h2_trace[8 * static_cast<uint64_t>(blockIdx.x) + 7] = wall_clock64();
 #endif
diff --git a/epos_amd/csrc/runtime.hip b/epos_amd/csrc/runtime.hip
--- a/epos_amd/csrc/runtime.hip
+++ b/epos_amd/csrc/runtime.hip
@@ -1,3 +1,4 @@
+#include <stddef.h>
 #include <stdarg.h>
 #include <string.h>
 
@@ -39,6 +40,13 @@
 
 extern "C" int epos_abi_version(void) { return EPOS_ABI_VERSION; }
 
+extern "C" void epos_store_policy_layout(int64_t* out4) {
+  out4[0] = sizeof(EposPointwiseArgs);
+  out4[1] = offsetof(EposPointwiseArgs, c_stream);
+  out4[2] = sizeof(EposDepthwiseArgs);
+  out4[3] = offsetof(EposDepthwiseArgs, y_store);
+}
+
 extern "C" const char* epos_last_error(void) { return epos::g_error; }
 
 extern "C" int epos_device_count(void) {
diff --git a/epos_amd/csrc/softmax.hip b/epos_amd/csrc/softmax.hip
--- a/epos_amd/csrc/softmax.hip
+++ b/epos_amd/csrc/softmax.hip
@@ -65,7 +65,7 @@
 };
 
 template <int VEC, int NV, typename Rows>
-__global__ __launch_bounds__(256) void softmax_kernel(float* X, Rows rows, int G) {
+__global__ __launch_bounds__(256) void softmax_kernel(float* X, Rows rows, int G, int policy) {
   constexpr int ROWS_PER_WAVE = VEC ? 64 / VEC : 1;
   const int lane = threadIdx.x & 63;
   typedef typename Rows::Index Index;
@@ -76,25 +76,25 @@
   if constexpr (VEC != 0) {
     float* x = rows.at(X, on ? r : 0, 4 * VEC) + (lane & (VEC - 1)) * 4;
     const float4 y = softmax_vec4<VEC>(ld4<Rows::STREAM>(x));
-    if (on) st4<Rows::STREAM>(x, y);
+    if (on) st16_policy(x, y, policy);
   } else {
     softmax_strided<NV>(rows.at(X, r, G), G, lane);
   }
 }
 
 template <int VEC, int NV, typename Rows>
-int launch_form(float* X, const Rows& rows, unsigned grid_y, int G, void* stream,
+int launch_form(float* X, const Rows& rows, unsigned grid_y, int G, int policy, void* stream,
                 const char* name) {
   const unsigned grid_x = static_cast<unsigned>(ceil_div(rows.n, VEC == 16 ? 16 : 4));
   hipLaunchKernelGGL((softmax_kernel<VEC, NV, Rows>), dim3(grid_x, grid_y), dim3(256), 0,
-                     static_cast<hipStream_t>(stream), X, rows, G);
+                     static_cast<hipStream_t>(stream), X, rows, G, policy);
   return launch_status(name);
 }
 
 template <typename Rows>
-int softmax_launch(float* X, const Rows& rows, unsigned grid_y, int G, void* stream) {
+int softmax_launch(float* X, const Rows& rows, unsigned grid_y, int G, int policy, void* stream) {
 #define EPOS_SM_LAUNCH(VEC, NV)                                                          \
-  launch_form<VEC, NV>(X, rows, grid_y, G, stream,                                       \
+  launch_form<VEC, NV>(X, rows, grid_y, G, policy, stream,                                    \
                        std::is_same<Rows, DenseRows>::value                              \
                            ? "softmax_kernel<" #VEC ", " #NV ", DenseRows>"              \
                            : "softmax_kernel<" #VEC ", " #NV ", SlotRows>")
@@ -109,18 +109,42 @@
 
 using namespace epos;
 
+static int softmax_groups(const char* fn, float* X, int64_t n_groups, int G, int policy,
+                          void* stream) {
+  EPOS_REQUIRE_FN(fn, X, "null pointer");
+  EPOS_REQUIRE_FN(fn, G >= 1 && G <= 256, "G must be in [1, 256]");
+  EPOS_REQUIRE_FN(fn, policy >= EPOS_STORE_PLAIN && policy <= EPOS_STORE_WT,
+                  "policy must be an EPOS_STORE_* policy");
+  if (n_groups == 0) return EPOS_OK;
+  return softmax_launch(X, DenseRows{n_groups}, 1, G, policy, stream);
+}
+
+static int softmax_slots(const char* fn, float* X, const EposCorrSlot* slots, int S, int P, int O,
+                         int F, int policy, void* stream) {
+  EPOS_REQUIRE_FN(fn, X && slots, "null pointer");
+  EPOS_REQUIRE_FN(fn, F >= 1 && F <= 256, "F must be in [1, 256]");
+  EPOS_REQUIRE_FN(fn, policy >= EPOS_STORE_PLAIN && policy <= EPOS_STORE_WT,
+                  "policy must be an EPOS_STORE_* policy");
+  if (S == 0 || P == 0) return EPOS_OK;
+  return softmax_launch(X, SlotRows{P, slots, O}, S, F, policy, stream);
+}
+
+extern "C" int epos_softmax_groups_policy_f32(float* X, int64_t n_groups, int G, int policy,
+                                              void* stream) {
+  return softmax_groups(__func__, X, n_groups, G, policy, stream);
+}
+
 extern "C" int epos_softmax_groups_f32(float* X, int64_t n_groups, int G,
                                        void* stream) {
-  EPOS_REQUIRE(X, "null pointer");
-  EPOS_REQUIRE(G >= 1 && G <= 256, "G must be in [1, 256]");
-  if (n_groups == 0) return EPOS_OK;
-  return softmax_launch(X, DenseRows{n_groups}, 1, G, stream);
+  return softmax_groups(__func__, X, n_groups, G, EPOS_STORE_STREAM, stream);
+}
+
+extern "C" int epos_softmax_slots_policy_f32(float* X, const EposCorrSlot* slots, int S, int P,
+                                             int O, int F, int policy, void* stream) {
+  return softmax_slots(__func__, X, slots, S, P, O, F, policy, stream);
 }
 
 extern "C" int epos_softmax_slots_f32(float* X, const EposCorrSlot* slots, int S,
                                       int P, int O, int F, void* stream) {
-  EPOS_REQUIRE(X && slots, "null pointer");
-  EPOS_REQUIRE(F >= 1 && F <= 256, "F must be in [1, 256]");
-  if (S == 0 || P == 0) return EPOS_OK;
-  return softmax_launch(X, SlotRows{P, slots, O}, S, F, stream);
+  return softmax_slots(__func__, X, slots, S, P, O, F, EPOS_STORE_PLAIN, stream);
 }
diff --git a/epos_amd/net.py b/epos_amd/net.py
--- a/epos_amd/net.py
+++ b/epos_amd/net.py
@@ -6,6 +6,7 @@
 
 from epos_amd import _call as C
 from epos_amd import _lib
+from epos_amd import store_policy
 from epos_amd import weights as W
 from epos_amd._call import ptr as _ptr
 from epos_amd.net_modes import Bf16Mode, Fp32Mode
@@ -177,6 +178,9 @@
     bias0 = float(np.abs(np.asarray(bias, np.float64)).max())
     return self._dev(w9c), self._dev(bias), gain, bias0
 
+  def _store_policy(self, family, default):
+    return getattr(self.mode, 'store_policy', {}).get(family, default)
+
   def _fn(self, name):
     return None if self.lib is None else getattr(self.lib, name)
 
@@ -493,9 +497,12 @@
       self._conv1x1('logits/' + name, None, x, 0, 256, m_dec, 256, buf, 0, ch, relu=False,
                     group=grp, track_out=False)
       self.logits[name] = buf
-    if os.environ.get('EPOS_HEAD_NT_STORES', '1') == '1':
-      for g in grp:
-        g[1].c_stream = 1
+    heads_policy = self._store_policy('heads', _lib.STORE_STREAM)
+    if os.environ.get('EPOS_HEAD_NT_STORES', '1') != '1' and \
+        'heads' not in store_policy.named(os.environ.get(store_policy.ENV)):
+      heads_policy = _lib.STORE_PLAIN
+    for g in grp:
+      g[1].c_stream = heads_policy
     oname, oargs, oflops = [g for g in grp if g[0].endswith(W.PRED_OBJ_CONF)][0][:3]
     self.heads_group = None
     mode.flush(grp, heads=os.environ.get('EPOS_HEADS_KERNEL', '1') == '1')
@@ -507,10 +514,12 @@
     frag = self.logits[W.PRED_FRAG_CONF]
     self.obj_label = self._empty(B, dh, dw_, dtype=torch.int64)
     O, F = self.num_objs, self.num_frags
-    softmax = self._fn('epos_softmax_groups_f32')
+    softmax = self._fn('epos_softmax_groups_policy_f32')
+    sm_policy = self._store_policy('softmax', _lib.STORE_STREAM)
     self.post_ops = [
-        ('softmax_obj', self._call('softmax_obj', softmax, (_ptr(obj), m_dec, O + 1))),
-        ('softmax_frag', self._call('softmax_frag', softmax, (_ptr(frag), m_dec * O, F))),
+        ('softmax_obj', self._call('softmax_obj', softmax, (_ptr(obj), m_dec, O + 1, sm_policy))),
+        ('softmax_frag', self._call('softmax_frag', softmax,
+                                    (_ptr(frag), m_dec * O, F, sm_policy))),
         ('argmax', self._call('argmax', self._fn('epos_argmax_i64'),
                               (_ptr(obj), O + 1, _ptr(self.obj_label), m_dec, O + 1)))]
     eo = self._expr_of(self.logits[W.PRED_OBJ_CONF])
@@ -806,8 +815,9 @@
           self._images_u8 = torch.empty(n, dtype=torch.uint8, device=self.dev)
         self._images_u8.copy_(t, non_blocking=True)
         src = self._images_u8
-      _lib.check(self.lib.epos_u8_to_f32(_ptr(src), _ptr(self.images), n, self._stream()),
-                 'u8_to_f32')
+      _lib.check(self.lib.epos_u8_to_f32_policy(
+          _ptr(src), _ptr(self.images), n, self._store_policy('glue', _lib.STORE_PLAIN),
+          self._stream()), 'u8_to_f32')
       return
     if t.dtype != torch.float32:
       if t.is_cuda:
diff --git a/epos_amd/net_modes.py b/epos_amd/net_modes.py
--- a/epos_amd/net_modes.py
+++ b/epos_amd/net_modes.py
@@ -5,6 +5,7 @@
 import torch
 
 from epos_amd import _lib
+from epos_amd import store_policy
 from epos_amd._call import ptr as _ptr
 from epos_amd import weights as W
 
@@ -46,14 +47,14 @@
     self.gemm1 = fn('epos_pointwise_conv_f32')
     self.heads = fn('epos_heads_gemm_f32')
     self.dw = fn('epos_depthwise3x3_f32')
-    self.conv3x3 = fn('epos_conv3x3_f32')
-    self.im2col3x3 = fn('epos_im2col3x3_f32')
+    self.conv3x3 = fn('epos_conv3x3_policy_f32')
+    self.im2col3x3 = fn('epos_im2col3x3_policy_f32')
     self.im2col_k = fn('epos_im2col_f32')
     self.absmax = fn('epos_absmax_f32')
     self.amax_clear = fn('epos_amax_clear')
     self.avg_pool = fn('epos_global_avg_pool_f32')
     self.avg_pool_partial = fn('epos_global_avg_pool_partial_f32')
-    self.resize_fn = fn('epos_resize_bilinear_f32')
+    self.resize_fn = fn('epos_resize_bilinear_policy_f32')
     self.subsample = fn('epos_subsample_f32')
     self.add_relu = fn('epos_add_relu_f32')
     self.maxpool = fn('epos_maxpool3x3_s2_f32')
@@ -72,6 +73,10 @@
     self.packs = {}
     self.layer_operands = {}
     self.pack_device = fn('epos_pack_weights_device_f32')
+    self.store_policy = store_policy.from_env()
+    self._c_writers = {}
+    self._writer_of = {}
+    self.dw_launches = []
     self._last_pw = None
     self._first_im2col = None
 
@@ -174,7 +179,12 @@
         a_amax=self._slot_ptr(ab[0]) if h else None,
         a_amax2=self._slot_ptr(ab[1]) if h else None,
         a_gain=ab[2] if h else 0.0, a_bias=ab[3] if h else 0.0,
-        a_presplit=int(presplit), c_amax=self._slot_ptr(cslot))
+        a_presplit=int(presplit), c_amax=self._slot_ptr(cslot),
+        c_stream=self.store_policy['gemm_gemm'])
+    writer = [args]
+    self._c_writers.setdefault(id(c), []).append(writer)
+    if group is not None:
+      self._writer_of[id(args)] = writer
     if (name in W.TRAINABLE_LAYERS and name not in W.LOGITS_LAYERS) or \
         name in W.POINTWISE_CHAIN_LAYERS or name in net._aspp_pw:
       assert a_off == 0 and sub == 1 and res is None, name
@@ -191,6 +201,10 @@
     for kind in sorted({g[1].a_presplit for g in group}):
       part = [g for g in group if g[1].a_presplit == kind]
       arr = (_lib.PointwiseArgs * len(part))(*[g[1] for g in part])
+      for i, g in enumerate(part):
+        writer = self._writer_of.pop(id(g[1]), None)
+        if writer is not None:
+          writer[0] = arr[i]
       fn = self.heads if heads and not kind else self.gemm
       if fn is self.heads:
         self.net.heads_group = (arr, len(part))
@@ -198,11 +212,17 @@
                        sum(g[2] for g in part), sum(g[3] for g in part))
     del group[:]
 
+  def gemm_launches(self):
+    return [writer[0] for writers in self._c_writers.values() for writer in writers]
+
   def depthwise(self, name, x, y, gain, bias0, flops, nbytes, **fields):
     xb = self._bounds.get(id(x))
     if xb is not None:
       self._set_bound(y, xb[0], xb[1], gain * (xb[2] if xb[2] else 1.0), gain * xb[3] + bias0)
-    args = _lib.DepthwiseArgs(**fields)
+    args = _lib.DepthwiseArgs(y_store=self.store_policy['dw'], **fields)
+    for writer in self._c_writers.get(id(x), ()):
+      writer[0].c_stream = self.store_policy['gemm_dw']
+    self.dw_launches.append(args)
     yb = self._bounds.get(id(y))
     if yb is not None and self.use_presplit:
       args.y_h2 = 1
@@ -227,7 +247,8 @@
                               Wh=_ptr(wh) if wh is not None else None,
                               x_amax=self._slot_ptr(xb[0]) if wh is not None else None,
                               y_amax=self._slot_ptr(yslot))
-      net._launch(name, self.conv3x3, (args,), 'gemm', 2 * B * ho * wo * cout * k,
+      net._launch(name, self.conv3x3, (args, self.store_policy['conv']), 'gemm',
+                  2 * B * ho * wo * cout * k,
                   4 * (B * hi * wi * cin + k * cout + B * ho * wo * cout))
       net.op_io[name] = (4 * B * hi * wi * cin, 4 * (k * cout + B * ho * wo * cout), id(x))
       return
@@ -239,12 +260,14 @@
                 C=cin, stride=stride, rate=rate, pad=pad, preprocess=preprocess)
     if kk == 3:
       args, fn, words = _lib.Im2colArgs(**geom), self.im2col3x3, m * ldcol
+      extra = (self.store_policy['glue'],)
     else:
       args = _lib.Im2colKArgs(k=kk, mean_rgb=(ctypes.c_float * 3)(*W.MEAN_RGB), **geom)
       fn, words = self.im2col_k, wo * ldcol // 4 * min(B * ho, 65535)
+      extra = ()
     if self._first_im2col is None:
       self._first_im2col = (name + '/im2col', args, words)
-    net._launch(name + '/im2col', fn, (args,), 'im2col')
+    net._launch(name + '/im2col', fn, (args,) + extra, 'im2col')
     self.pointwise(name, col, 0, ldcol, m, k, conv, y, 0, cout, relu=True)
     net.op_io[name] = (x.element_size() * B * hi * wi * cin, net.op_io[name][1], id(x))
 
@@ -265,7 +288,8 @@
 
   def resize(self, name, x, ldx, y, ldy, hi, wi, ho, wo, c):
     self.net._launch(name, self.resize_fn,
-                     (_ptr(x), ldx, _ptr(y), ldy, self.net.B, hi, wi, ho, wo, c))
+                     (_ptr(x), ldx, _ptr(y), ldy, self.net.B, hi, wi, ho, wo, c,
+                      self.store_policy['glue']))
 
   def obj_head(self, name, args):
     return self.net._call(name, self.gemm1, (args,))
diff --git a/epos_amd/store_policy.py b/epos_amd/store_policy.py
--- /dev/null
+++ b/epos_amd/store_policy.py
@@ -0,0 +1,51 @@
+import os
+
+from epos_amd import _lib
+
+POLICIES = {'plain': _lib.STORE_PLAIN, 'stream': _lib.STORE_STREAM, 'wt': _lib.STORE_WT}
+FAMILIES = ('gemm_dw', 'gemm_gemm', 'dw', 'heads', 'conv', 'glue', 'softmax')
+ALIASES = {'gemm': ('gemm_dw', 'gemm_gemm')}
+ENV = 'EPOS_STORE_POLICY'
+
+DEFAULT = {'gemm_dw': 'wt', 'gemm_gemm': 'plain', 'dw': 'plain', 'heads': 'stream',
+           'conv': 'plain', 'glue': 'plain', 'softmax': 'stream'}
+
+
+def parse(text):
+  table = dict(DEFAULT)
+  text = (text or '').strip()
+  if not text:
+    return table
+  if ':' not in text and ',' not in text:
+    if text not in POLICIES:
+      raise ValueError('%s=%r: expected one of %s or family:policy,...' % (
+          ENV, text, '|'.join(sorted(POLICIES))))
+    return dict.fromkeys(FAMILIES, text)
+  seen = set()
+  for item in text.split(','):
+    family, sep, policy = item.strip().partition(':')
+    families = ALIASES.get(family, (family,))
+    if not sep or any(f not in FAMILIES for f in families) or policy not in POLICIES:
+      raise ValueError('%s: %r is not family:policy with a family of %s and a policy of %s' % (
+          ENV, item, '|'.join(FAMILIES), '|'.join(sorted(POLICIES))))
+    if seen.intersection(families):
+      raise ValueError('%s: family %r is set twice' % (ENV, family))
+    seen.update(families)
+    table.update(dict.fromkeys(families, policy))
+  return table
+
+
+def named(text):
+  text = (text or '').strip()
+  if not text:
+    return set()
+  parse(text)
+  if ':' not in text:
+    return set(FAMILIES)
+  return {f for item in text.split(',')
+          for f in ALIASES.get(item.strip().partition(':')[0], (item.strip().partition(':')[0],))}
+
+
+def from_env(environ=None):
+  table = parse((os.environ if environ is None else environ).get(ENV))
+  return {family: POLICIES[name] for family, name in table.items()}
diff --git a/include/epos_hip.h b/include/epos_hip.h
--- a/include/epos_hip.h
+++ b/include/epos_hip.h
@@ -15,6 +15,11 @@
 #define EPOS_E_HIP_BASE (-1000)
 
 #define EPOS_ABI_VERSION 7
+
+#define EPOS_STORE_PLAIN 0
+#define EPOS_STORE_STREAM 1
+#define EPOS_STORE_WT 2
+void epos_store_policy_layout(int64_t* out4);
 
 int epos_abi_version(void);
 const char* epos_last_error(void);
@@ -77,6 +82,7 @@
   uint32_t* y_amax;
 } EposConv3x3Args;
 int epos_conv3x3_f32(const EposConv3x3Args* args, void* stream);
+int epos_conv3x3_policy_f32(const EposConv3x3Args* args, int policy, void* stream);
 
 typedef struct EposDepthwiseArgs {
   const float* X; int64_t ldx;
@@ -86,6 +92,7 @@
   int32_t stride, rate;
   int32_t relu_in, relu_out;
   int32_t y_h2;
+  int32_t y_store;
   const uint32_t* x_amax;
   const uint32_t* x_amax2;
   float gain, bias0;
@@ -109,6 +116,7 @@
   int64_t amax_words;
 } EposIm2colArgs;
 int epos_im2col3x3_f32(const EposIm2colArgs* args, void* stream);
+int epos_im2col3x3_policy_f32(const EposIm2colArgs* args, int policy, void* stream);
 
 #define EPOS_PREPROCESS_NONE 0
 #define EPOS_PREPROCESS_UNIT_RANGE 1
@@ -134,6 +142,9 @@
 int epos_resize_bilinear_f32(const float* X, int64_t ldx, float* Y, int64_t ldy,
                              int B, int Hi, int Wi, int Ho, int Wo, int C,
                              void* stream);
+int epos_resize_bilinear_policy_f32(const float* X, int64_t ldx, float* Y, int64_t ldy,
+                                    int B, int Hi, int Wi, int Ho, int Wo, int C, int policy,
+                                    void* stream);
 
 int epos_maxpool3x3_s2_f32(const float* X, int64_t ldx, float* Y, int64_t ldy,
                            int B, int Hi, int Wi, int C, void* stream);
@@ -146,8 +157,10 @@
                             int64_t n_blocks, int width, void* stream);
 
 int epos_u8_to_f32(const uint8_t* X, float* Y, int64_t n, void* stream);
+int epos_u8_to_f32_policy(const uint8_t* X, float* Y, int64_t n, int policy, void* stream);
 
 int epos_softmax_groups_f32(float* X, int64_t n_groups, int G, void* stream);
+int epos_softmax_groups_policy_f32(float* X, int64_t n_groups, int G, int policy, void* stream);
 
 int epos_argmax_i64(const float* X, int64_t ldx, int64_t* labels, int64_t P,
                     int C, void* stream);
@@ -159,6 +172,8 @@
 
 int epos_softmax_slots_f32(float* X, const EposCorrSlot* slots, int S, int P,
                            int O, int F, void* stream);
+int epos_softmax_slots_policy_f32(float* X, const EposCorrSlot* slots, int S, int P, int O, int F,
+                                  int policy, void* stream);
 
 int epos_corr_count(const float* obj_confs, const float* frag_confs,
                     const EposCorrSlot* slots , int S, int B, int P,
```

New measurement: 400.6, median of 6. No clear change (+0.8%).
